# declare-lab/Emma-X

Hardware: AMD Instinct MI355X
Metric: actions/sec (higher is better)
Workload: dtype bf16; 1 GPU; BASELINE configs[1]: Emma-X-7B bf16, 1 frame(s)/GPU 224x224, 512-token prompt, greedy, 512 new tokens (EOS disabled), random-init weights; uint8 frames and prompt ids are resident in HBM when the timed region starts; the 7-vector is de-tokenised from the generated ids by the ids-level stand-in `actions_from_ids` (no LLaMA tokenizer offline: decode -> Solver text parse is host work of microseconds,; batch_per_gpu=1, global_batch=1, context=1280, parallelism=dp1, hipgraph=False, exact_numerics=False

## Files before the change

emma-x_amd/csrc/decode_ks.hip:

```cpp
#include <cstdlib>

#include "common.h"
#include "kernels.h"
#include "decode_epilogue.h"

#ifndef KS_W_AUX
#define KS_W_AUX 2
#endif
namespace {

constexpr int KS_WAVES = 8;
constexpr int KS_NT = KS_WAVES * 64;
constexpr int PSTRIDE = EMMAX_PSTRIDE;

__device__ __forceinline__ void ks_fold32(float& a, float& b) {
    asm volatile("s_nop 1\n\tv_permlane32_swap_b32 %0, %1" : "+v"(a), "+v"(b));
    a += b;
}
__device__ __forceinline__ void ks_fold16(float& a, float& b) {
    asm volatile("s_nop 1\n\tv_permlane16_swap_b32 %0, %1" : "+v"(a), "+v"(b));
    a += b;
}
template <int RB>
__device__ __forceinline__ float ks_reduce_rows(float (&v)[RB], int lane) {
    static_assert(RB == 1 || RB == 2 || RB == 4 || RB == 8 || RB == 16, "batch of rows");
    if constexpr (RB == 16) {
#pragma unroll
        for (int j = 0; j < 8; ++j) ks_fold32(v[j], v[j + 8]);
    }
    if constexpr (RB >= 8) {
        constexpr int H = 4;
#pragma unroll
        for (int j = 0; j < H; ++j) ks_fold16(v[j], v[j + H]);
    }
    if constexpr (RB >= 4) {
        const bool hi = (lane & 8) != 0;
#pragma unroll
        for (int j = 0; j < 2; ++j) {
            const float keep = hi ? v[j + 2] : v[j], give = hi ? v[j] : v[j + 2];
            v[j] = keep + dpp_move<0x128>(give);
        }
    }
    if constexpr (RB >= 2) {
        const bool hi = (lane & 4) != 0;
        const float keep = hi ? v[1] : v[0], give = hi ? v[0] : v[1];
        v[0] = keep + dpp_move<0x141>(give);
    }
    float t = v[0];
    t += dpp_move<0xB1>(t);
    t += dpp_move<0x4E>(t);
    if constexpr (RB < 2) t += dpp_move<0x141>(t);
    if constexpr (RB < 4) t += dpp_move<0x128>(t);
    if constexpr (RB < 8) { float a = t, b = t; ks_fold16(a, b); t = a; }
    if constexpr (RB < 16) { float a = t, b = t; ks_fold32(a, b); t = a; }
    return t;
}
template <int RB>
__device__ __forceinline__ int ks_row_of_lane(int lane) {
    int r = 0, bit = RB >> 1;
    if constexpr (RB == 16) { r += (lane >> 5) * bit; bit >>= 1; }
    if constexpr (RB >= 8) { r += ((lane >> 4) & 1) * bit; bit >>= 1; }
    if constexpr (RB >= 4) { r += ((lane >> 3) & 1) * bit; bit >>= 1; }
    if constexpr (RB >= 2) { r += ((lane >> 2) & 1) * bit; }
    return r;
}
template <int RB>
__device__ __forceinline__ bool ks_lane_stores(int lane) {
    int mask = 3;
    if constexpr (RB < 2) mask |= 4;
    if constexpr (RB < 4) mask |= 8;
    if constexpr (RB < 8) mask |= 16;
    if constexpr (RB < 16) mask |= 32;
    return (lane & mask) == 0;
}

template <int B, int CPL> struct KsShape { static constexpr int RB = (B == 1 ? 16 : 8) / (CPL == 1 ? 1 : CPL == 2 ? 2 : 4); };

template <int B> struct KsRegs { static constexpr int N = B == 1 ? 16 : 8; };

enum { XS_GLOBAL = 0, XS_ATTN = 1, XS_EMBED = 2 };
#ifdef DECODE_LAB_TRACE
__device__ unsigned long long g_ks_trace[512 * 2 * 4 * 6];
#define KS_STAMP(op, k, v) do { if ((threadIdx.x == 0 || threadIdx.x == 448) && blockIdx.x < 512 && (op) >= 0) \
    g_ks_trace[((blockIdx.x * 2 + (threadIdx.x ? 1 : 0)) * 4 + (op)) * 6 + (k)] = (v); } while (0)
#else
#define KS_STAMP(op, k, v) do { } while (0)
#endif
template <int MODE>
__device__ __forceinline__ void ks_pair_rows(const GemvParams& p, int g, int& r0, int& r1) {
    if (MODE == GEMV_QKV) {
        const int half = p.head_dim >> 1;
        const int hb = g >> p.ks_shift, d = g - hb * half;
        r0 = hb * p.head_dim + d;
        r1 = r0 + half;
    } else if (MODE == GEMV_GATEUP) {
        r0 = (g >> 4) * 32 + (g & 15);
        r1 = r0 + 16;
    } else {
        r0 = 2 * g;
        r1 = min(2 * g + 1, p.n_rows - 1);
    }
}
__device__ __forceinline__ void ks_share(const GemvParams& p, int& g_lo, int& npairs) {
    const int G = gridDim.x, bid = blockIdx.x;
    const int q = p.n_groups / G, r = p.n_groups % G;
    g_lo = bid * q + min(bid, r);
    npairs = min(q + (bid < r ? 1 : 0), max(p.n_groups - g_lo, 0));
}

template <int B, int MODE, int CPL>
__device__ __forceinline__ void ks_issue(const GemvParams& p, int g_lo, int nrows, int bb, const unsigned (&voff)[CPL], u32x4_t (&wr)[KsRegs<B>::N]) {
    constexpr int RB = KsShape<B, CPL>::RB;
    const __amdgpu_buffer_rsrc_t wrsrc = __builtin_amdgcn_make_buffer_rsrc((void*)p.W, 0, (int)((unsigned)p.n_rows * (unsigned)p.ldw * 2u), 0x00020000);
#pragma unroll
    for (int jj = 0; jj < RB; ++jj) {
        const int i = bb * RB + jj;
        int r0, r1;
        ks_pair_rows<MODE>(p, g_lo + (i >> 1), r0, r1);
        const int m = (i - nrows) >> 31;
        const int r = (((i & 1) ? r1 : r0) & m) | (p.n_rows & ~m);
        const unsigned so = (unsigned)r * (unsigned)p.ldw * 2u;
#pragma unroll
        for (int j = 0; j < CPL; ++j)
            wr[jj * CPL + j] = __builtin_bit_cast(u32x4_t, __builtin_amdgcn_raw_buffer_load_b128(wrsrc, voff[j], so, KS_W_AUX));
    }
}

template <int CPL>
__device__ __forceinline__ void ks_chunks(int K, int wave, int lane, int (&coff)[CPL], bool (&cok)[CPL], unsigned (&voff)[CPL]) {
    const int NCW = K >> 6;
#pragma unroll
    for (int j = 0; j < CPL; ++j) {
        const int c = j * 64 + lane;
        cok[j] = c < NCW;
        coff[j] = wave * NCW + min(c, NCW - 1);
        voff[j] = (unsigned)coff[j] * 16u;
    }
}

template <int B, int MODE, bool NORM, int XS, int CPL, bool R32, bool EX = false>
__device__ __forceinline__ void ks_run_op(const GemvParams& p, u32x4_t (&wr)[KsRegs<B>::N], float* part, float* sumsq, int rows_cap,
                                          int trace_op = -1) {
    constexpr int RB = KsShape<B, CPL>::RB;
    KS_STAMP(trace_op, 0, wall_clock64());
    const int tid = threadIdx.x, lane = tid & 63, wave = __builtin_amdgcn_readfirstlane(tid >> 6);
    const int K = p.K, bid = blockIdx.x;
    int g_lo, npairs;
    ks_share(p, g_lo, npairs);
    const int nrows = 2 * npairs;

    const bool epi = wave < B && lane < npairs;
    const int eb = wave < B ? wave : 0, epair = g_lo + min(lane, max(npairs - 1, 0));
    int er0, er1;
    ks_pair_rows<MODE>(p, epair, er0, er1);
    float pre_a = 0.f, pre_b = 0.f;
    int pre_pos = 0, pre_pg = 0;
    if (epi) {
        if (MODE == GEMV_RESID) {
            pre_a = resid_fetch(p, eb, er0, R32);
            pre_b = resid_fetch(p, eb, er1, R32);
        } else if (MODE == GEMV_QKV) {
            qkv_row_pos(p, eb, pre_pos, pre_pg);
            const int hb = epair >> p.ks_shift;
            qkv_rope_fetch(p, pre_pos, hb, epair - hb * (p.head_dim >> 1), pre_a, pre_b);
        }
    }

    int coff[CPL];
    bool cok[CPL];
    unsigned voff[CPL];
    ks_chunks<CPL>(K, wave, lane, coff, cok, voff);

    u32x4_t xr[B][CPL];
    u32x4_t xl[EX ? B : 1][EX ? CPL : 1];
    if constexpr (EX && XS == XS_GLOBAL && !NORM) {
        f32x8_t xq[B][CPL];
#pragma unroll
        for (int b = 0; b < B; ++b)
#pragma unroll
            for (int j = 0; j < CPL; ++j) xq[b][j] = ld_f32x8((const float*)p.x + (size_t)b * p.ldx + (size_t)coff[j] * 8);
        ks_issue<B, MODE, CPL>(p, g_lo, nrows, 0, voff, wr);
#pragma unroll
        for (int b = 0; b < B; ++b)
#pragma unroll
            for (int j = 0; j < CPL; ++j)
#pragma unroll
                for (int e = 0; e < 4; ++e) {
                    const hl2_t t = split_hl2(cok[j] ? f32x8_at(xq[b][j], 2 * e) : 0.f, cok[j] ? f32x8_at(xq[b][j], 2 * e + 1) : 0.f);
                    xr[b][j][e] = t.hi;
                    xl[b][j][e] = t.lo;
                }
    } else if constexpr (XS == XS_ATTN) {
#pragma unroll
        for (int b = 0; b < B; ++b)
#pragma unroll
            for (int j = 0; j < CPL; ++j) {
                const int cg = coff[j];
                const float* pp = p.attn_part + (size_t)(b * p.Hq + (cg >> 4)) * p.nsplit * PSTRIDE;
                if constexpr (EX) {
                    float m8[8];
                    (void)(p.nsplit == 8 ? attn_merge_chunk<8, 4>(pp, (cg & 15) * 8, m8) : attn_merge_chunk_loop(pp, (cg & 15) * 8, p.nsplit, m8));
#pragma unroll
                    for (int e = 0; e < 4; ++e) {
                        const hl2_t t = split_hl2(cok[j] ? m8[2 * e] : 0.f, cok[j] ? m8[2 * e + 1] : 0.f);
                        xr[b][j][e] = t.hi;
                        xl[b][j][e] = t.lo;
                    }
                } else {
                    const u32x4_t v = p.nsplit == 8 ? attn_merge_chunk<8, 4>(pp, (cg & 15) * 8) : attn_merge_chunk_loop(pp, (cg & 15) * 8, p.nsplit);
#pragma unroll
                    for (int e = 0; e < 4; ++e) xr[b][j][e] = cok[j] ? v[e] : 0u;
                }
            }
        __builtin_amdgcn_sched_barrier(0);
        ks_issue<B, MODE, CPL>(p, g_lo, nrows, 0, voff, wr);
    } else {
        u32x4_t nw[CPL];
        if constexpr (NORM) {
#pragma unroll
            for (int j = 0; j < CPL; ++j) nw[j] = *((const u32x4_t*)p.norm_w + coff[j]);
        }
        float ss[B];
        if constexpr (R32 && NORM && XS != XS_EMBED) {
            f32x8_t xq[B][CPL];
#pragma unroll
            for (int b = 0; b < B; ++b)
#pragma unroll
                for (int j = 0; j < CPL; ++j) xq[b][j] = ld_f32x8(p.h32 + (size_t)b * p.ldh + (size_t)coff[j] * 8);
            ks_issue<B, MODE, CPL>(p, g_lo, nrows, 0, voff, wr);
#pragma unroll
            for (int b = 0; b < B; ++b) {
                ss[b] = 0.f;
#pragma unroll
                for (int j = 0; j < CPL; ++j)
#pragma unroll
                    for (int e = 0; e < 4; ++e) {
                        const float a = cok[j] ? f32x8_at(xq[b][j], 2 * e) : 0.f, c = cok[j] ? f32x8_at(xq[b][j], 2 * e + 1) : 0.f;
                        ss[b] += a * a + c * c;
                        if constexpr (EX) {
                            const hl2_t t = split_hl2(a * bf_lo(nw[j][e]), c * bf_hi(nw[j][e]));
                            xr[b][j][e] = t.hi;
                            xl[b][j][e] = t.lo;
                        } else {
                            xr[b][j][e] = pack_bf16x2(a * bf_lo(nw[j][e]), c * bf_hi(nw[j][e]));
                        }
                    }
            }
        } else {
#pragma unroll
            for (int b = 0; b < B; ++b) {
                size_t row = (size_t)b;
                if constexpr (XS == XS_EMBED) row = (size_t)min(max(p.x_tok[b], 0), p.x_vocab - 1);
#pragma unroll
                for (int j = 0; j < CPL; ++j) {
                    xr[b][j] = *((const u32x4_t*)((const bf16_t*)p.x + row * p.ldx) + coff[j]);
                    if constexpr (XS == XS_EMBED) {
                        if (blockIdx.x == 0 && cok[j]) {
                            *((u32x4_t*)((bf16_t*)p.x_copy + (size_t)b * p.ldx) + coff[j]) = xr[b][j];
                            if constexpr (R32) {
                                const f32x8_t f = bf16x8_to_f32(xr[b][j]);
                                float* hp = p.h32 + (size_t)b * p.ldh + (size_t)coff[j] * 8;
                                *(f32x4_t*)hp = f.lo;
                                *(f32x4_t*)(hp + 4) = f.hi;
                            }
                        }
                    }
                }
            }
            ks_issue<B, MODE, CPL>(p, g_lo, nrows, 0, voff, wr);
#pragma unroll
            for (int b = 0; b < B; ++b) {
                ss[b] = 0.f;
#pragma unroll
                for (int j = 0; j < CPL; ++j)
#pragma unroll
                    for (int e = 0; e < 4; ++e) {
                        uint32_t v = cok[j] ? xr[b][j][e] : 0u;
                        if constexpr (NORM) {
                            const float a = bf_lo(v), c = bf_hi(v);
                            ss[b] += a * a + c * c;
                            if constexpr (EX) {
                                const hl2_t t = split_hl2(a * bf_lo(nw[j][e]), c * bf_hi(nw[j][e]));
                                v = t.hi;
                                xl[b][j][e] = t.lo;
                            } else {
                                v = pack_bf16x2(a * bf_lo(nw[j][e]), c * bf_hi(nw[j][e]));
                            }
                        }
                        xr[b][j][e] = v;
                    }
            }
        }
        if constexpr (NORM) {
#pragma unroll
            for (int b = 0; b < B; ++b) {
                const float t = wave_sum(ss[b]);
                if (lane == 0) sumsq[wave * B + b] = t;
            }
        }
    }

    KS_STAMP(trace_op, 1, wall_clock64());
    const int nbatch = (nrows + RB - 1) / RB;
    for (int bb = 0; bb < nbatch; ++bb) {
        float acc[B][RB];
#pragma unroll
        for (int jj = 0; jj < RB; ++jj)
#pragma unroll
            for (int b = 0; b < B; ++b) {
                float a = 0.f;
#pragma unroll
                for (int j = 0; j < CPL; ++j) {
                    a = dot2_bf16(wr[jj * CPL + j][0], xr[b][j][0], a);
                    a = dot2_bf16(wr[jj * CPL + j][1], xr[b][j][1], a);
                    a = dot2_bf16(wr[jj * CPL + j][2], xr[b][j][2], a);
                    a = dot2_bf16(wr[jj * CPL + j][3], xr[b][j][3], a);
                    if constexpr (EX) {
                        a = dot2_bf16(wr[jj * CPL + j][0], xl[b][j][0], a);
                        a = dot2_bf16(wr[jj * CPL + j][1], xl[b][j][1], a);
                        a = dot2_bf16(wr[jj * CPL + j][2], xl[b][j][2], a);
                        a = dot2_bf16(wr[jj * CPL + j][3], xl[b][j][3], a);
                    }
                }
                acc[b][jj] = a;
            }
        __builtin_amdgcn_sched_barrier(0);
        ks_issue<B, MODE, CPL>(p, g_lo, nrows, bb + 1, voff, wr);
        __builtin_amdgcn_sched_barrier(0);
#pragma unroll
        for (int b = 0; b < B; ++b) {
            const float t = ks_reduce_rows<RB>(acc[b], lane);
            if (ks_lane_stores<RB>(lane)) part[(wave * B + b) * rows_cap + bb * RB + ks_row_of_lane<RB>(lane)] = t;
        }
    }
    KS_STAMP(trace_op, 3, wall_clock64());
    __syncthreads();
    KS_STAMP(trace_op, 4, wall_clock64());

    float red0 = 0.f, red1 = 0.f;
    if (epi) {
#pragma unroll
        for (int w = 0; w < KS_WAVES; ++w) {
            red0 += part[(w * B + eb) * rows_cap + 2 * lane];
            red1 += part[(w * B + eb) * rows_cap + 2 * lane + 1];
        }
        if constexpr (NORM) {
            float t = 0.f;
#pragma unroll
            for (int w = 0; w < KS_WAVES; ++w) t += sumsq[w * B + eb];
            const float rstd = rsqrtf(t / (float)K + p.eps);
            red0 *= rstd;
            red1 *= rstd;
        }
    }
    const bool has1 = MODE == GEMV_QKV || MODE == GEMV_GATEUP || 2 * epair + 1 < p.n_rows;
    if (MODE == GEMV_PLAIN) {
        if (epi) {
            bf16_t* yp = (bf16_t*)p.y + (size_t)eb * p.ldy;
            yp[er0] = f2bf(red0);
            if (has1) yp[er1] = f2bf(red1);
        }
    } else if (MODE == GEMV_RESID) {
        if (epi) {
            if constexpr (R32) {
                float* hq = p.h32 + (size_t)eb * p.ldh;
                hq[er0] = pre_a + red0;
                if (has1) hq[er1] = pre_b + red1;
            }
            const uint32_t hv = pack_bf16x2(pre_a + red0, pre_b + red1);
            bf16_t* hp = (bf16_t*)p.y + (size_t)eb * p.ldy;
            hp[er0] = (bf16_t)(hv & 0xffffu);
            if (has1) hp[er1] = (bf16_t)(hv >> 16);
        }
    } else if (MODE == GEMV_GATEUP) {
        if (epi) swiglu_finish<EX>(p, eb, epair, red0, red1);
    } else if (MODE == GEMV_QKV && EX) {
        if (epi) {
            const int hd = p.head_dim, half = hd >> 1;
            const int hb = epair >> p.ks_shift, d = epair - hb * half;
            if (hb < p.Hq + p.Hkv) {
                const float y0 = __fadd_rn(__fmul_rn(red0, pre_a), -__fmul_rn(red1, pre_b)), y1 = __fadd_rn(__fmul_rn(red1, pre_a), __fmul_rn(red0, pre_b));
                if (hb < p.Hq) {
                    float* dst = (float*)p.y + (size_t)eb * p.ldy + hb * hd;
                    dst[d] = y0;
                    dst[d + half] = y1;
                } else {
                    gemv_kv_store_x(p, false, pre_pg, pre_pos, hb - p.Hq, d, y0);
                    gemv_kv_store_x(p, false, pre_pg, pre_pos, hb - p.Hq, d + half, y1);
                }
            } else {
                gemv_kv_store_x(p, true, pre_pg, pre_pos, hb - p.Hq - p.Hkv, d, red0);
                gemv_kv_store_x(p, true, pre_pg, pre_pos, hb - p.Hq - p.Hkv, d + half, red1);
            }
        }
    } else if (MODE == GEMV_QKV) {
        if (epi) {
            const int hd = p.head_dim, half = hd >> 1;
            const int hb = epair >> p.ks_shift, d = epair - hb * half;
            const float x0 = bf2f(f2bf(red0)), x1 = bf2f(f2bf(red1));
            if (hb < p.Hq + p.Hkv) {
                const bf16_t y0 = f2bf(x0 * pre_a - x1 * pre_b), y1 = f2bf(x1 * pre_a + x0 * pre_b);
                if (hb < p.Hq) {
                    bf16_t* q = (bf16_t*)p.y + (size_t)eb * p.ldy + hb * hd;
                    q[d] = y0;
                    q[d + half] = y1;
                } else {
                    bf16_t* kc = gemv_kv_row(p, false, eb, pre_pg, pre_pos, hb - p.Hq);
                    kc[d] = y0;
                    kc[d + half] = y1;
                }
            } else {
                bf16_t* vc = gemv_kv_row(p, true, eb, pre_pg, pre_pos, hb - p.Hq - p.Hkv);
                vc[d] = f2bf(x0);
                vc[d + half] = f2bf(x1);
            }
        }
    } else if (MODE == GEMV_LMHEAD) {
        if (wave < B) {
            float bv = -INFINITY;
            int bi = 0x7fffffff;
            if (epi) {
                bv = red0;
                bi = er0;
                if (has1) lmhead_take(red1, er1, bv, bi);
                if (p.logits_out) {
                    p.logits_out[(size_t)eb * p.n_rows + er0] = red0;
                    if (has1) p.logits_out[(size_t)eb * p.n_rows + er1] = red1;
                }
            }
            const float m = wave_max(bv);
            const float mi = wave_max((epi && bv == m) ? -(float)bi : -INFINITY);
            if (lane == 0) {
                p.part_val[(size_t)bid * B + eb] = m;
                p.part_idx[(size_t)bid * B + eb] = mi == -INFINITY ? 0x7fffffff : (int)(-mi);
            }
        }
    }
    KS_STAMP(trace_op, 5, wall_clock64());
}

template <int B, int MODE, bool NORM, int XS, int CPL, bool R32, bool EX = false>
__global__ __launch_bounds__(KS_NT, 4) void emmax_decode_ks_kernel(GemvParams p) {
    extern __shared__ __attribute__((aligned(16))) unsigned char ks_smem[];
    const int tid = threadIdx.x, lane = tid & 63, wave = __builtin_amdgcn_readfirstlane(tid >> 6);
    const int rows_cap = p.kc;
    float* part = (float*)ks_smem;
    float* sumsq = part + KS_WAVES * B * rows_cap;
    u32x4_t wr[KsRegs<B>::N];
    ks_run_op<B, MODE, NORM, XS, CPL, R32, EX>(p, wr, part, sumsq, rows_cap, 0);
}

template <int B, int MODE, bool NORM, int XS, int CPL, bool R32, bool EX = false>
int ks_launch_r(const GemvParams& p, const ProjGeom& g, hipStream_t stream) {
    hipLaunchKernelGGL((emmax_decode_ks_kernel<B, MODE, NORM, XS, CPL, R32, EX>), dim3(g.grid), dim3(KS_NT), g.smem, stream, p);
    return hipGetLastError() == hipSuccess ? 0 : -4;
}
template <int B, int MODE, bool NORM, bool XATTN, int CPL>
int ks_launch_t(const GemvParams& p, const ProjGeom& g, hipStream_t stream) {
    constexpr bool touches_h = NORM || MODE == GEMV_RESID;
    if (p.exact) {
        if constexpr (MODE == GEMV_PLAIN) return -2;
        else {
            if constexpr (MODE == GEMV_QKV) {
                if (p.x_tok) return ks_launch_r<B, MODE, NORM, XS_EMBED, CPL, true, true>(p, g, stream);
            }
            return ks_launch_r<B, MODE, NORM, XATTN ? XS_ATTN : XS_GLOBAL, CPL, true, true>(p, g, stream);
        }
    }
    if constexpr (MODE == GEMV_QKV) {
        if (p.x_tok) return p.h32 ? ks_launch_r<B, MODE, NORM, XS_EMBED, CPL, true>(p, g, stream) : ks_launch_r<B, MODE, NORM, XS_EMBED, CPL, false>(p, g, stream);
    }
    if constexpr (touches_h) {
        if (p.h32) return ks_launch_r<B, MODE, NORM, XATTN ? XS_ATTN : XS_GLOBAL, CPL, true>(p, g, stream);
    }
    return ks_launch_r<B, MODE, NORM, XATTN ? XS_ATTN : XS_GLOBAL, CPL, false>(p, g, stream);
}

template <int MODE, bool NORM, bool XATTN>
int ks_launch_mode(const GemvParams& p, int B, const ProjGeom& g, hipStream_t stream) {
#define KS_CASE(BB, CC) if (B == BB && g.cpl == CC) return ks_launch_t<BB, MODE, NORM, XATTN, CC>(p, g, stream)
    KS_CASE(1, 1); KS_CASE(1, 2); KS_CASE(1, 3); KS_CASE(2, 1); KS_CASE(2, 2); KS_CASE(2, 3);
#undef KS_CASE
    return -2;
}

}

bool decode_ks_enabled() { return emmax_tune().ks != 0; }

bool decode_ks_takes(const ProjShape& s, int B, ProjGeom* out) {
    if (B < 1 || B > 2 || s.wfmt != PW_BF16) return false;
    if (s.K % 64 || s.K > 64 * 64 * 3 || !s.ld_ok || s.K < 64) return false;
    if (s.mode < GEMV_QKV || s.mode > GEMV_PLAIN) return false;
    ProjGeom g = {};
    int max_grid = s.max_grid;
    if (s.mode == GEMV_RESID && s.attn_part) {
        if (s.K != s.Hq * 128) return false;
        if (!emmax_tune().ks_oproj) return false;
        max_grid = emmax_tune().ks_oproj_grid;
    }
    if (s.x_tok && s.mode != GEMV_QKV) return false;
    if (s.exact ? (s.mode == GEMV_PLAIN || !s.h32) : (s.mode == GEMV_PLAIN && s.h32)) return false;
    g.n_groups = (s.mode == GEMV_QKV || s.mode == GEMV_GATEUP) ? s.n_rows / 2 : (s.n_rows + 1) / 2;
    if (s.mode == GEMV_QKV) {
        while ((2 << g.shift) < s.head_dim) ++g.shift;
        if ((2 << g.shift) != s.head_dim) return false;
    }
    g.cpl = cdiv(s.K >> 6, 64);
    const int rb = B == 1 ? (g.cpl == 1 ? KsShape<1, 1>::RB : g.cpl == 2 ? KsShape<1, 2>::RB : KsShape<1, 3>::RB)
                          : (g.cpl == 1 ? KsShape<2, 1>::RB : g.cpl == 2 ? KsShape<2, 2>::RB : KsShape<2, 3>::RB);
    g.grid = min(512, g.n_groups);
    if (max_grid > 0) g.grid = min(g.grid, max_grid);
    if (s.mode == GEMV_LMHEAD) g.grid = min(g.grid, s.max_parts);
    if (g.grid < 1) return false;
    const int pairs_max = cdiv(g.n_groups, g.grid);
    if (pairs_max > 64) return false;
    g.kc = cdiv(2 * pairs_max, rb) * rb;
    g.smem = (size_t)(KS_WAVES * B * g.kc + KS_WAVES * B) * sizeof(float);
    if (out) *out = g;
    return true;
}

int launch_decode_ks(int mode, const GemvParams& p_in, int B, hipStream_t stream, int* grid_out, const ProjGeom* geom) {
    ProjGeom g;
    if (geom) g = *geom;
    else if (!decode_ks_takes(proj_shape(mode, p_in), B, &g)) return -2;
    GemvParams p = p_in;
    p.n_groups = p.n_pairs = g.n_groups; p.ks_shift = g.shift; p.kc = g.kc;
    if (grid_out) *grid_out = g.grid;
    switch (mode) {
        case GEMV_QKV: return ks_launch_mode<GEMV_QKV, true, false>(p, B, g, stream);
        case GEMV_RESID:
            return p.attn_part ? ks_launch_mode<GEMV_RESID, false, true>(p, B, g, stream) : ks_launch_mode<GEMV_RESID, false, false>(p, B, g, stream);
        case GEMV_GATEUP: return ks_launch_mode<GEMV_GATEUP, true, false>(p, B, g, stream);
        case GEMV_LMHEAD: return ks_launch_mode<GEMV_LMHEAD, true, false>(p, B, g, stream);
        default: return ks_launch_mode<GEMV_PLAIN, false, false>(p, B, g, stream);
    }
}

#ifdef DECODE_LAB_TRACE
extern "C" int emmax_debug_ks_trace(unsigned long long* host_out, int n_words) {
    return hipMemcpyFromSymbol(host_out, HIP_SYMBOL(g_ks_trace), (size_t)n_words * 8) == hipSuccess ? 0 : -1;
}
#endif
```

emma-x_amd/csrc/kernels.h:

```cpp
#pragma once

#include <hip/hip_runtime.h>
#include <stdint.h>

#include "common.h"

struct GemmParams {
    const void* A;
    const void* W;
    void* C;
    const void* bias;
    const void* scale;
    const void* residual;
    int M, N, K;
    int lda, ldw, ldc, ldr;
    int res_f32;
    int N_store;
    int act;
    int out_f32;
    float* ws;
    long long ws_bytes;
    int ksplit;
    const float* ln_stats;
    const float* ln_s;
// ... 63 lines not shown
};
int launch_prefill_state(const PrefillState& st, int32_t* cu, int32_t* ctx_len, int32_t* done, int32_t* n_out, int32_t* max_new,
                         int32_t* stop_m, int32_t* stop_after, hipStream_t stream);
struct CommitParams {
    int n, max_pages, max_out;
    int slot[EMMAX_MAX_DECODE_BATCH], src[EMMAX_MAX_DECODE_BATCH];
    int32_t *cur_tok, *ctx_len, *done, *n_out, *max_new, *stop_m, *stop_after, *out_ids, *page_table;
    float *temperature, *top_p, *logprob;
    int32_t* top_k;
    uint64_t* seed;
    uint32_t* subseq;
    float* penalty;
    int32_t *ngram, *min_new, *hist, *hist_len;
    int max_prompt;
    float* warp[4];
    uint32_t* rule_en;
};
int launch_slots_commit(const CommitParams& c, hipStream_t stream);
struct SlotForkParams {
    int n, rows, src, S, max_pages, max_prompt;
    int dst[EMMAX_MAX_DECODE_BATCH];
    int32_t *page_table, *hidden, *ctx_len, *done, *n_out, *max_new, *stop_m, *stop_after, *copy_src, *copy_dst, *copy_ntok;
    const float *in_t, *in_p;
    const int32_t* in_k;
    const uint64_t* in_seed;
    const uint32_t* in_sub;
    float *temperature, *top_p;
    int32_t* top_k;
    uint64_t* seed;
    uint32_t* subseq;
    float* penalty;
    int32_t *ngram, *min_new, *hist, *hist_len;
    float* warp[4];
    uint32_t* rule_en;
};
int launch_slots_fork(const SlotForkParams& p, hipStream_t stream);
int launch_slots_unhide(int32_t* table, int32_t* hidden, int n, hipStream_t stream);
int launch_set_int(int32_t* p, int32_t v, hipStream_t stream);
int launch_set_ints(int32_t* p, int n, int32_t v, hipStream_t stream);
int launch_slots_idle(int n, int32_t* cur_tok, int32_t* ctx_len, int32_t* done, int32_t* n_out, int32_t pad_id, hipStream_t stream);
int launch_embed_splice(const int32_t* ids, int P_max, const int32_t* cu, const void* E, const void* patches, void* h, int B,
                        int max_seqlen, int n_patches, int hidden, int vocab, hipStream_t stream, float* h32 = nullptr);
int launch_rope_kv_write(void* qkv, int ld, int q_off, int k_off, int v_off, const int32_t* cu, int B, int total_rows,
                         const float* cos_t, const float* sin_t, void* kcache, void* vcache, const int32_t* page_table,
                         int max_pages, int Hq, int Hkv, int hd, int page, hipStream_t stream);
int launch_kv_quant_rows(void* qkv , int ld, int k_off, int v_off, const int32_t* cu, int B, int total_rows, void* k8, void* v8, float* kscale,
                         float* vscale, const int32_t* page_table, int max_pages, int Hkv, int hd, int page, hipStream_t stream);
int launch_resize_bicubic_u8(const uint8_t* src, int B, int H, int W, uint8_t* dst, int OH, int OW, uint8_t* tmp, const int32_t* bounds_h,
                             const int32_t* kk_h, int ksize_h, const int32_t* bounds_v, const int32_t* kk_v, int ksize_v, hipStream_t stream);
int launch_gather_last_rows(const void* in, void* out, const int32_t* cu, int B, int D, hipStream_t stream, float* out32 = nullptr, const float* in32 = nullptr);

struct EmmaxTune {
    int graph;
    int ks;
    int ks_oproj;
    int ks_oproj_grid;
    int km;
    int km_down;
    int km_roll;
    int attn_deep;
    int attn_ksplit;
    int attn_lazy;
    int vis_streams;
    int attn_nw;
    int streamk;
    int fp8_gemv;
    int attn_group;
    int attn_nsplit;
    int attn_direct;
    int fold_embed;
    int mfma_xbar;
    int gemm_big;
    int gemm_splitk;
    int gemm_sk_big;
    int gemm_hybrid;
    int gemm_normfuse;
    int gemm_deep;
    int gemm_dbg;
    int gemm_lnfuse;
    int attn_resident;
    int kv_fp8;
    int resid32;
    int mx4_wide;
    int exact;
    int epoch;
};
const EmmaxTune& emmax_tune();

enum { GEMV_QKV = 0, GEMV_RESID = 1, GEMV_GATEUP = 2, GEMV_LMHEAD = 3, GEMV_PLAIN = 4 };
struct GemvParams {
    const void* x;
    const void* W;
    void* y;
    const void* norm_w;
    int K, ldw, ldx, ldy;
    int n_rows;
    int n_groups;
    int max_parts;
    int kc;
    int batch;
    float eps;
    int head_dim, Hq, Hkv, page, max_pages;
    const int32_t* ctx_len;
    const int32_t* page_table;
    const float* cos_t;
    const float* sin_t;
    void* kcache;
    void* vcache;
    float* part_val;
    int32_t* part_idx;
    float* logits_out;
    const float* attn_part;
    int nsplit;
    void* kv_stage;
    const float* wscale;
    int n_pairs;
    unsigned long long* sk_ws;
    int sk_kt8, sk_q, sk_r;
    unsigned int sk_magic;
    int qk_shift;
    int x_bar;
    int max_grid;
    int ks_shift;
    const int32_t* x_tok;
    void* x_copy;
    int x_vocab;
    float* h32;
    int ldh;
    int exact;
    long long kv24;
    const void* w4_scales;
};

enum { PW_BF16 = 0, PW_FP8 = 1, PW_MX4 = 2 };
struct ProjShape {
    int mode, K, n_rows, head_dim, Hq;
    int wfmt;
    bool exact, h32, attn_part, x_tok;
    int nsplit, max_parts, max_grid;
    bool ld_ok;
    bool mx4_wide;
};
static inline ProjShape proj_shape(int mode, const GemvParams& p) {
    return {mode, p.K, p.n_rows, p.head_dim, p.Hq, p.w4_scales ? PW_MX4 : p.wscale ? PW_FP8 : PW_BF16, p.exact != 0, p.h32 != nullptr,
            p.attn_part != nullptr, p.x_tok != nullptr, p.nsplit, p.max_parts, p.max_grid, p.ldw % 8 == 0 && p.ldx % 8 == 0};
}
struct ProjGeom {
    int grid, n_groups;
    int kc;
    size_t smem;
    int shift;
    int cpl, f8;
    int nb, phased, roll;
    int tmax, nph, nh;
};
bool decode_ks_takes(const ProjShape& s, int B, ProjGeom* g = nullptr);
bool decode_gemv_takes(const ProjShape& s, int B, ProjGeom* g = nullptr);
bool decode_km_takes(const ProjShape& s, int B, ProjGeom* g = nullptr);
bool decode_kmp_takes(const ProjShape& s, int B, ProjGeom* g = nullptr);
bool decode_mfma_takes(const ProjShape& s, int B, ProjGeom* g = nullptr);
int launch_decode_gemv(int mode, const GemvParams& p, int B, hipStream_t stream, int* grid_out = nullptr, int* staged_out = nullptr);
int launch_decode_gemv_staged(int mode, const GemvParams& p, int B, const ProjGeom& g, hipStream_t stream, int* grid_out = nullptr);
int launch_decode_ks(int mode, const GemvParams& p, int B, hipStream_t stream, int* grid_out = nullptr, const ProjGeom* geom = nullptr);
bool decode_ks_enabled();
int decode_gemv_init();
int launch_decode_embed(const int32_t* cur_tok, const void* E, void* h, int B, int hidden, int vocab, hipStream_t stream, float* h32 = nullptr);

struct DecodeAttnParams {
    const void* q;
    const void* kcache;
    const void* vcache;
    const int32_t* page_table;
    const int32_t* ctx_len;
    const int32_t* done;
    float* part;
    void* o_out;
    const void* kv_stage;
    float* kscale;
    float* vscale;
    int ldq, Hkv, page, max_pages;
    int page_shift;
    float scale;
    long long kv24;
    const int32_t* grp_shared;
    int grp_N, grp_nsplit, grp_Hq;
};
int decode_attn_nsplit(int B, int Hkv);
int launch_decode_attn(const DecodeAttnParams& p, int B, int Hq, int head_dim, int nsplit, hipStream_t stream);
enum { EMMAX_GROUP_ATTN_MAX_SPLITS = 8 };
bool group_attn_takes(int B, int N, int Hq, int Hkv);
int group_attn_nsplit(int B, int N, int Hq, int Hkv);
int launch_group_attn(const DecodeAttnParams& p, int B, int N, int Hq, int head_dim, hipStream_t stream);
int launch_x_decode_attn(const DecodeAttnParams& p, int B, int Hq, int head_dim, int nsplit, hipStream_t stream);

struct FinishParams {
    const float* part_val;
    const int32_t* part_idx;
    int n_part, B;
    int32_t* cur_tok;
    int32_t* ctx_len;
    int32_t* done;
    int32_t* n_out;
    int32_t* out_ids;
    const int32_t* max_new_p;
    const int32_t* stop_ids;
    const int32_t* stop_cfg;
    int32_t* stop_m;
    int32_t* stop_after;
    int max_out, max_ctx;
    int eos_id, pad_id;
    int is_prefill;
};
int launch_decode_finish(const FinishParams& p, hipStream_t stream);
__device__ __forceinline__ void emmax_finish_row(const FinishParams& p, int b, int tok, float* lp_row, float lp, bool stop_row) {
    int was_done = p.done[b];
    int n = p.n_out[b];
    const int budget_n = p.max_new_p[b];
    if (!p.is_prefill && !was_done && n >= budget_n) {
        was_done = 1;
        p.done[b] = 1;
    }
    if (!p.is_prefill && !was_done) p.ctx_len[b] += 1;
    if (p.is_prefill)
        for (int i = 0; i < p.max_out; ++i) {
            p.out_ids[(size_t)b * p.max_out + i] = p.pad_id;
            if (lp_row) lp_row[i] = 0.f;
        }
    if (was_done) {
        tok = p.pad_id;
    } else {
        if (n < p.max_out) {
            p.out_ids[(size_t)b * p.max_out + n] = tok;
            if (lp_row) lp_row[n] = lp;
        }
        n += 1;
        p.n_out[b] = n;
        const bool budget = !p.is_prefill && n >= budget_n;
        bool stop = false;
        const int n_trig = p.stop_cfg[0];
        if (n_trig > 0) {
            int aft = p.stop_after[b];
            if (aft >= 0) {
                aft += 1;
            } else {
                int mp = p.stop_m[b];
                mp = (tok == p.stop_ids[mp]) ? mp + 1 : ((tok == p.stop_ids[0]) ? 1 : 0);
                if (mp == n_trig) {
// ... 162 lines not shown
```

emma-x_amd/csrc/model.hip:

```cpp
#include <array>
#include <cctype>
#include <cstdarg>
#include <cstdlib>
#include <mutex>

#include "session.h"

thread_local std::string g_err;
int fail(int code, const char* fmt, ...) {
    char buf[1024];
    va_list ap;
    va_start(ap, fmt);
    vsnprintf(buf, sizeof(buf), fmt, ap);
    va_end(ap);
    g_err = buf;
    return code;
}

namespace {
struct TuneEntry { const char* name; int EmmaxTune::*field; int def; };
const TuneEntry kTune[] = {
    {"graph", &EmmaxTune::graph, 0},           {"ks", &EmmaxTune::ks, 1},
    {"ks_oproj", &EmmaxTune::ks_oproj, 1},     {"ks_oproj_grid", &EmmaxTune::ks_oproj_grid, 256},
    {"km", &EmmaxTune::km, 1},                 {"km_down", &EmmaxTune::km_down, 1},
    {"km_roll", &EmmaxTune::km_roll, 0},       {"attn_nw", &EmmaxTune::attn_nw, 4},
    {"attn_deep", &EmmaxTune::attn_deep, -1},  {"attn_ksplit", &EmmaxTune::attn_ksplit, -1},
    {"attn_lazy", &EmmaxTune::attn_lazy, 1},      {"vis_streams", &EmmaxTune::vis_streams, 1},
    {"streamk", &EmmaxTune::streamk, 1},       {"fp8_gemv", &EmmaxTune::fp8_gemv, -1},
    {"attn_nsplit", &EmmaxTune::attn_nsplit, 0}, {"attn_direct", &EmmaxTune::attn_direct, 1},
    {"fold_embed", &EmmaxTune::fold_embed, 1}, {"mfma_xbar", &EmmaxTune::mfma_xbar, 1},
    {"gemm_big", &EmmaxTune::gemm_big, -1},    {"gemm_splitk", &EmmaxTune::gemm_splitk, 1},
    {"gemm_sk_big", &EmmaxTune::gemm_sk_big, -1},
    {"gemm_deep", &EmmaxTune::gemm_deep, -1},       {"gemm_dbg", &EmmaxTune::gemm_dbg, 0},
    {"gemm_lnfuse", &EmmaxTune::gemm_lnfuse, 1}, {"attn_resident", &EmmaxTune::attn_resident, -1},
    {"gemm_hybrid", &EmmaxTune::gemm_hybrid, 1}, {"gemm_normfuse", &EmmaxTune::gemm_normfuse, 1},
    {"resid32", &EmmaxTune::resid32, 1},       {"kv_fp8", &EmmaxTune::kv_fp8, 0},
    {"exact", &EmmaxTune::exact, 0},           {"attn_group", &EmmaxTune::attn_group, -1},
    {"mx4_wide", &EmmaxTune::mx4_wide, 0},
};
EmmaxTune g_tune;
std::once_flag g_tune_once;
void tune_init() {
    g_tune.epoch = 0;
    for (const TuneEntry& e : kTune) {
        g_tune.*(e.field) = e.def;
        std::string env = "EMMAX_";
        for (const char* c = e.name; *c; ++c) env += (char)toupper((unsigned char)*c);
        if (const char* v = getenv(env.c_str())) g_tune.*(e.field) = atoi(v);
    }
}
}
const EmmaxTune& emmax_tune() {
    std::call_once(g_tune_once, tune_init);
    return g_tune;
}

__attribute__((constructor)) static void emmax_export_runtime_switches() { setenv("DEBUG_CLR_GRAPH_PACKET_CAPTURE", "0", 0); }

static int check_config(const emmax_config& c, bool format_rules = true) {
    for (int t = 0; t < 2; ++t) {
        const auto& w = c.tower[t];
        if (w.embed_dim <= 0 || w.num_heads <= 0 || w.embed_dim % w.num_heads) return fail(EMMAX_ERR_INVALID, "tower %d: bad embed_dim/num_heads", t);
        const int hd = w.embed_dim / w.num_heads;
        if (hd != 64 && hd != 72) return fail(EMMAX_ERR_INVALID, "tower %d: head_dim %d outside the hot path (64 or 72)", t, hd);
        if (w.embed_dim % 8 || w.mlp_hidden % 8) return fail(EMMAX_ERR_INVALID, "tower %d: dims must be multiples of 8", t);
        if (w.take_index < 0 || w.take_index >= w.depth) return fail(EMMAX_ERR_INVALID, "tower %d: take_index out of range", t);
        if (w.image_size % w.patch) return fail(EMMAX_ERR_INVALID, "tower %d: image_size %% patch != 0", t);
    }
    if (c.tower[0].image_size != c.tower[1].image_size || c.tower[0].patch != c.tower[1].patch)
        return fail(EMMAX_ERR_INVALID, "towers must share image size and patch size");
    if (c.head_dim != 128) return fail(EMMAX_ERR_INVALID, "LLM head_dim %d outside the hot path (128)", c.head_dim);
    if (c.hidden % 128) return fail(EMMAX_ERR_INVALID, "LLM hidden must be a multiple of 128");
    if (c.n_heads % c.n_kv_heads) return fail(EMMAX_ERR_INVALID, "n_heads %% n_kv_heads != 0");
    const int G = c.n_heads / c.n_kv_heads;
    if (G != 1 && G != 2 && G != 4 && G != 8) return fail(EMMAX_ERR_INVALID, "GQA group %d unsupported (1,2,4,8)", G);
    if (c.inter % 16) return fail(EMMAX_ERR_INVALID, "LLM intermediate size must be a multiple of 16");
    if (c.vocab % 8) return fail(EMMAX_ERR_INVALID, "vocab must be a multiple of 8");
    if (c.decode_fp8 < 0 || c.decode_fp8 > 2) return fail(EMMAX_ERR_INVALID, "decode_fp8 %d: 0 (bf16), 1 (fp8-e4m3) or 2 (MXFP4)", c.decode_fp8);
    if (c.decode_fp8 == 1 && (c.hidden % 64 || (c.n_heads * c.head_dim) % 64)) return fail(EMMAX_ERR_INVALID, "fp8 decode needs K % 64 == 0");
    if (c.decode_fp8 == 2 && format_rules) {
        const int q_dim = c.n_heads * c.head_dim, qkv_dim = (c.n_heads + 2 * c.n_kv_heads) * c.head_dim;
        if (c.hidden % 1024 || c.hidden > 4096 || q_dim % 1024 || q_dim > 4096)
            return fail(EMMAX_ERR_INVALID, "MXFP4 decode weights need hidden (%d) and n_heads * head_dim (%d) in multiples of 1024 up to 4096", c.hidden, q_dim);
        if (c.inter % 128 || c.inter <= 4096 || c.inter > 12288)
            return fail(EMMAX_ERR_INVALID, "MXFP4 decode weights need an intermediate size (%d) that is a multiple of 128, above 4096 and at most 12288", c.inter);
        if (qkv_dim > 32768 || 2 * c.inter > 32768 || pad_to(c.vocab, 128) > 32768)
            return fail(EMMAX_ERR_INVALID, "MXFP4 decode weights need at most 32768 rows per projection (qkv %d, gate/up %d, vocab %d)", qkv_dim, 2 * c.inter, c.vocab);
    }
    return 0;
}

struct ProjDim { int stage; int64_t N, K; int perm, perm_hd, gemv_mode, f8bit; };
static std::array<ProjDim, 4> layer_projs(const emmax_model* m) {
    return {{{STAGE_QKV, m->qkv_dim, m->H, 1, m->cfg.head_dim, GEMV_QKV, F8_QKV}, {STAGE_OPROJ, m->H, m->q_dim, 0, 0, GEMV_RESID, F8_OPROJ},
             {STAGE_GATEUP, 2 * (int64_t)m->inter_p, m->H, 2, 0, GEMV_GATEUP, F8_GATEUP}, {STAGE_DOWN, m->H, m->inter_p, 0, 0, GEMV_RESID, F8_DOWN}}};
}

static void derive(emmax_model* m) {
    const auto& c = m->cfg;
    m->H = c.hidden;
    m->inter = c.inter;
    m->inter_p = pad_to(c.inter, 64);
    m->q_dim = c.n_heads * c.head_dim;
    m->kv_dim = c.n_kv_heads * c.head_dim;
    m->qkv_dim = m->q_dim + 2 * m->kv_dim;
    m->vocab = c.vocab;
    m->vocab_p = pad_to(c.vocab, 128);
    m->V = c.tower[0].embed_dim + c.tower[1].embed_dim;
    m->Vp = pad_to(m->V, 128);
    m->P1 = 4 * m->V;
    m->P1p = pad_to(m->P1, 128);
    for (int t = 0; t < 2; ++t) {
        const auto& w = c.tower[t];
        TowerW& T = m->tw[t];
        T.D = w.embed_dim;
        T.Dp = pad_to(T.D, 128);
        T.D3p = pad_to(3 * T.D, 128);
        T.M = w.mlp_hidden;
        T.Mp = pad_to(T.M, 128);
        T.n_prefix = (w.has_cls ? 1 : 0) + w.n_reg;
        T.n_patches = (w.image_size / w.patch) * (w.image_size / w.patch);
        T.N = T.n_prefix + T.n_patches;
        T.hd = T.D / w.num_heads;
        T.Kpe = pad_to(3 * w.patch * w.patch, 64);
        T.n_blocks = w.take_index + 1;
        T.blk.resize(T.n_blocks);
    }
    m->layers.resize(c.n_layers);
    for (auto& L : m->layers) {
        memset(&L, 0, sizeof(L));
        for (const ProjDim& d : layer_projs(m)) { L.proj[d.stage].gemv_mode = d.gemv_mode; L.proj[d.stage].f8bit = d.f8bit; }
    }
    m->lm_head_w = ProjW{};
    m->lm_head_w.gemv_mode = GEMV_LMHEAD; m->lm_head_w.f8bit = F8_LMHEAD;
    m->fp8 = c.decode_fp8 == 1;
    m->mx4 = c.decode_fp8 == 2;
    m->mx4_wide = m->mx4 && emmax_tune().mx4_wide != 0;
    for (auto& L : m->layers)
        for (const ProjDim& d : layer_projs(m)) L.proj[d.stage].q4w = m->mx4_wide;
    m->lm_head_w.q4w = m->mx4_wide;
}

static void plan_arena(emmax_model* m, Bump& b) {
    for (int t = 0; t < 2; ++t) {
        TowerW& T = m->tw[t];
        T.patch_w = b.take((int64_t)T.Dp * T.Kpe);
        T.patch_b = b.take(T.Dp);
        T.pos = b.take((int64_t)T.n_patches * T.D);
        T.cls = b.take(T.D);
        T.reg = b.take((int64_t)std::max(1, m->cfg.tower[t].n_reg) * T.D);
        for (auto& k : T.blk) {
            k.n1w = b.take(T.D); k.n1b = b.take(T.D);
            k.qkv_w = b.take((int64_t)T.D3p * T.Dp); k.qkv_b = b.take(T.D3p);
            k.proj_w = b.take((int64_t)T.Dp * T.Dp); k.proj_b = b.take(T.Dp);
            k.ls1 = b.take(T.Dp);
            k.n2w = b.take(T.D); k.n2b = b.take(T.D);
            k.fc1_w = b.take((int64_t)T.Mp * T.Dp); k.fc1_b = b.take(T.Mp);
            k.fc2_w = b.take((int64_t)T.Dp * T.Mp); k.fc2_b = b.take(T.Dp);
            k.ls2 = b.take(T.Dp);
            k.ln1_s = (float*)b.take(2 * (int64_t)T.D3p); k.ln1_c = (float*)b.take(2 * (int64_t)T.D3p);
            k.ln2_s = (float*)b.take(2 * (int64_t)T.Mp); k.ln2_c = (float*)b.take(2 * (int64_t)T.Mp);
        }
    }
    m->pj1_w = b.take((int64_t)m->P1p * m->Vp); m->pj1_b = b.take(m->P1p);
    m->pj2_w = b.take((int64_t)m->H * m->P1p); m->pj2_b = b.take(m->H);
    m->pj3_w = b.take((int64_t)m->H * m->H); m->pj3_b = b.take(m->H);
    m->embed = b.take((int64_t)m->vocab * m->H);
    for (auto& L : m->layers) {
        const auto dims = layer_projs(m);
        ProjW *const q = &L.proj[STAGE_QKV], *const o = &L.proj[STAGE_OPROJ], *const g = &L.proj[STAGE_GATEUP], *const d = &L.proj[STAGE_DOWN];
        L.ln1 = b.take(m->H);
        q->rm = b.take(dims[0].N * dims[0].K);
        o->rm = b.take(dims[1].N * dims[1].K);
        L.ln2 = b.take(m->H);
        g->rm = b.take(dims[2].N * dims[2].K);
        d->rm = b.take(dims[3].N * dims[3].K);
        for (const ProjDim& p : dims) { ProjW& w = L.proj[p.stage]; w.r8 = nullptr; w.sc = w.km_sc = nullptr; w.q4 = w.q4s = nullptr; }
        if (m->mx4)
            for (const ProjDim& p : dims) { ProjW& w = L.proj[p.stage]; w.q4 = b.bytes(p.N * p.K / 2); w.q4s = b.bytes(p.N * p.K / 32); }
        if (m->fp8) {
            for (const ProjDim& p : dims) L.proj[p.stage].fm = b.take(p.N * p.K / 2);
            q->km = b.take(dims[0].N * dims[0].K / 2);
            g->km = b.take(dims[2].N * dims[2].K / 2);
            for (const ProjDim& p : dims) L.proj[p.stage].r8 = b.take(p.N * p.K / 2);
            for (const ProjDim& p : dims) L.proj[p.stage].sc = (float*)b.take(2 * p.N);
            q->km_sc = (float*)b.take(2 * dims[0].N);
            g->km_sc = (float*)b.take(2 * dims[2].N);
            o->km = o->fm; o->km_sc = o->sc;
            d->km = d->fm; d->km_sc = d->sc;
        }
    }
    m->final_norm = b.take(m->H);
    ProjW& lm = m->lm_head_w;
    lm.rm = b.take((int64_t)m->vocab_p * m->H);
    if (m->fp8) {
        lm.km = lm.fm = b.take((int64_t)m->vocab_p * m->H / 2);
        lm.km_sc = lm.sc = (float*)b.take(2 * (int64_t)m->vocab_p);
        lm.r8 = b.take((int64_t)m->vocab_p * m->H / 2);
    }
    if (m->mx4) { lm.q4 = b.bytes((int64_t)m->vocab_p * m->H / 2); lm.q4s = b.bytes((int64_t)m->vocab_p * m->H / 32); }
}

static void plan_aux(emmax_model* m, Bump& b, bool with_ab_partner) {
    for (auto& L : m->layers) {
        const auto dims = layer_projs(m);
        ProjW *const q = &L.proj[STAGE_QKV], *const o = &L.proj[STAGE_OPROJ], *const g = &L.proj[STAGE_GATEUP], *const d = &L.proj[STAGE_DOWN];
        q->km = b.take(dims[0].N * dims[0].K);
        g->km = b.take(dims[2].N * dims[2].K);
        o->km = o->fm = b.take(dims[1].N * dims[1].K);
        d->km = d->fm = b.take(dims[3].N * dims[3].K);
        q->fm = with_ab_partner ? b.take(dims[0].N * dims[0].K) : nullptr;
        g->fm = with_ab_partner ? b.take(dims[2].N * dims[2].K) : nullptr;
    }
    m->lm_head_w.km = m->lm_head_w.fm = b.take((int64_t)m->vocab_p * m->H);
}

static int put2d(emmax_model* m, const std::string& key, int rows, int cols, bf16* dst, int dst_ld, int row0, hipStream_t st) {
    auto it = m->bound.find(key);
    if (it == m->bound.end()) return fail(EMMAX_ERR_MISSING, "finalize: weight `%s` was never bound", key.c_str());
    const Bound& w = it->second;
    if (w.dtype != EMMAX_BF16) return fail(EMMAX_ERR_INVALID, "weight `%s` must be bf16", key.c_str());
    if (w.numel() != (int64_t)rows * cols)
        return fail(EMMAX_ERR_INVALID, "weight `%s`: expected %d x %d = %lld elements, got %lld", key.c_str(), rows, cols,
// ... 81 lines not shown
        TowerW& T = m->tw[t];
        const emmax_tower_config& tc = m->cfg.tower[t];
        const std::string P = pre[t];
        PUT2(P + "patch_embed.proj.weight", T.D, 3 * tc.patch * tc.patch, T.patch_w, T.Kpe, 0);
        PUT1(P + "patch_embed.proj.bias", T.D, T.patch_b);
        PUT1(P + "pos_embed", T.n_patches * T.D, T.pos);
        if (tc.has_cls) PUT1(P + "cls_token", T.D, T.cls);
        if (tc.n_reg) PUT1(P + "reg_token", tc.n_reg * T.D, T.reg);
        for (int i = 0; i < T.n_blocks; ++i) {
            BlockW& k = T.blk[i];
            const std::string Bp = P + "blocks." + std::to_string(i) + ".";
            PUT1(Bp + "norm1.weight", T.D, k.n1w); PUT1(Bp + "norm1.bias", T.D, k.n1b);
            PUT2(Bp + "attn.qkv.weight", 3 * T.D, T.D, k.qkv_w, T.Dp, 0); PUT1(Bp + "attn.qkv.bias", 3 * T.D, k.qkv_b);
            PUT2(Bp + "attn.proj.weight", T.D, T.D, k.proj_w, T.Dp, 0); PUT1(Bp + "attn.proj.bias", T.D, k.proj_b);
            PUT1(Bp + "norm2.weight", T.D, k.n2w); PUT1(Bp + "norm2.bias", T.D, k.n2b);
            PUT2(Bp + "mlp.fc1.weight", T.M, T.D, k.fc1_w, T.Dp, 0); PUT1(Bp + "mlp.fc1.bias", T.M, k.fc1_b);
            PUT2(Bp + "mlp.fc2.weight", T.D, T.M, k.fc2_w, T.Mp, 0); PUT1(Bp + "mlp.fc2.bias", T.D, k.fc2_b);
            if (tc.layerscale) { PUT1(Bp + "ls1.scale_factor", T.D, k.ls1); PUT1(Bp + "ls2.scale_factor", T.D, k.ls2); }
            if (fold_ln) {
                KCHK(launch_ln_fold(k.qkv_w, T.Dp, 3 * T.D, T.D, k.n1w, k.n1b, k.qkv_b, k.ln1_s, k.ln1_c, st));
                KCHK(launch_ln_fold(k.fc1_w, T.Dp, T.M, T.D, k.n2w, k.n2b, k.fc1_b, k.ln2_s, k.ln2_c, st));
            }
        }
    }
    PUT2("projector.fc1.weight", m->P1, m->V, m->pj1_w, m->Vp, 0); PUT1("projector.fc1.bias", m->P1, m->pj1_b);
    PUT2("projector.fc2.weight", m->H, m->P1, m->pj2_w, m->P1p, 0); PUT1("projector.fc2.bias", m->H, m->pj2_b);
    PUT2("projector.fc3.weight", m->H, m->H, m->pj3_w, m->H, 0); PUT1("projector.fc3.bias", m->H, m->pj3_b);
    PUT2("language_model.model.embed_tokens.weight", m->vocab, m->H, m->embed, m->H, 0);
    for (int li = 0; li < m->cfg.n_layers; ++li) {
        LayerW& L = m->layers[li];
        const std::string P = "language_model.model.layers." + std::to_string(li) + ".";
        PUT1(P + "input_layernorm.weight", m->H, L.ln1);
        PUT2(P + "self_attn.q_proj.weight", m->q_dim, m->H, L.proj[STAGE_QKV].rm, m->H, 0);
        PUT2(P + "self_attn.k_proj.weight", m->kv_dim, m->H, L.proj[STAGE_QKV].rm, m->H, m->q_dim);
        PUT2(P + "self_attn.v_proj.weight", m->kv_dim, m->H, L.proj[STAGE_QKV].rm, m->H, m->q_dim + m->kv_dim);
        PUT2(P + "self_attn.o_proj.weight", m->H, m->q_dim, L.proj[STAGE_OPROJ].rm, m->q_dim, 0);
        PUT1(P + "post_attention_layernorm.weight", m->H, L.ln2);
        {
            auto ig = m->bound.find(P + "mlp.gate_proj.weight");
            auto iu = m->bound.find(P + "mlp.up_proj.weight");
            if (ig == m->bound.end() || iu == m->bound.end()) return fail(EMMAX_ERR_MISSING, "finalize: gate/up of layer %d not bound", li);
            if (ig->second.numel() != (int64_t)m->inter * m->H || iu->second.numel() != (int64_t)m->inter * m->H)
                return fail(EMMAX_ERR_INVALID, "gate/up of layer %d have the wrong size", li);
            const size_t grp = (size_t)16 * m->H * 2;
            HIPCHK(hipMemcpy2DAsync(L.proj[STAGE_GATEUP].rm, 2 * grp, ig->second.ptr, grp, grp, m->inter / 16, hipMemcpyDeviceToDevice, st));
            HIPCHK(hipMemcpy2DAsync((char*)L.proj[STAGE_GATEUP].rm + grp, 2 * grp, iu->second.ptr, grp, grp, m->inter / 16, hipMemcpyDeviceToDevice, st));
        }
        PUT2(P + "mlp.down_proj.weight", m->H, m->inter, L.proj[STAGE_DOWN].rm, m->inter_p, 0);
        if (m->fp8) {
            const auto dims = layer_projs(m);
            for (const ProjDim& d : dims) KCHK(launch_quant_fm8(L.proj[d.stage].rm, (int)d.K, L.proj[d.stage].fm, L.proj[d.stage].sc, (int)d.N, (int)d.K, st));
            for (const ProjDim& d : dims)
                KCHK(launch_quant_rm8(L.proj[d.stage].rm, (int)d.K, L.proj[d.stage].r8, L.proj[d.stage].sc, (int)d.N, (int)d.K, st));
            for (const ProjDim& d : dims)
                if (d.perm) KCHK(launch_quant_fm8(L.proj[d.stage].rm, (int)d.K, L.proj[d.stage].km, L.proj[d.stage].km_sc, (int)d.N, (int)d.K, st, d.perm, d.perm_hd));
        }
        if (m->mx4)
            for (const ProjDim& d : layer_projs(m)) {
                ProjW& w = L.proj[d.stage];
                KCHK(launch_quant_mx4(w.rm, (int)d.K, w.q4, w.q4s, (int)d.N, (int)d.K, d.perm, d.perm_hd, st));
                KCHK(launch_dequant_mx4(w.q4, w.q4s, w.rm, (int)d.K, (int)d.N, (int)d.K, d.perm, d.perm_hd, st));
            }
    }
    PUT1("language_model.model.norm.weight", m->H, m->final_norm);
    PUT2("language_model.lm_head.weight", m->vocab, m->H, m->lm_head_w.rm, m->H, 0);
    if (m->fp8) {
        KCHK(launch_quant_fm8(m->lm_head_w.rm, m->H, m->lm_head_w.fm, m->lm_head_w.sc, m->vocab_p, m->H, st));
        KCHK(launch_quant_rm8(m->lm_head_w.rm, m->H, m->lm_head_w.r8, m->lm_head_w.sc, m->vocab_p, m->H, st));
    }
    if (m->mx4) {
        KCHK(launch_quant_mx4(m->lm_head_w.rm, m->H, m->lm_head_w.q4, m->lm_head_w.q4s, m->vocab_p, m->H, 0, 0, st));
        KCHK(launch_dequant_mx4(m->lm_head_w.q4, m->lm_head_w.q4s, m->lm_head_w.rm, m->H, m->vocab_p, m->H, 0, 0, st));
    }
#undef PUT2
#undef PUT1
    HIPCHK(hipStreamSynchronize(st));
    m->finalized = true;
    m->ln_folded = fold_ln;
    m->aux_built = m->fp8 || m->mx4;
    m->bound.clear();
    return 0;
}

int emmax_model_max_decode_batch(const emmax_model* m) { return m ? model_max_decode_batch(m) : -1; }
int emmax_model_max_decode_batch_exact(const emmax_model* m) { return m ? model_max_decode_batch(m, true) : -1; }
int emmax_model_mxfp4_wide(const emmax_model* m) { return m ? (m->mx4_wide ? 1 : 0) : -1; }
int emmax_config_max_decode_batch(const emmax_config* cfg, int exact) {
    if (!cfg) return fail(EMMAX_ERR_INVALID, "null argument");
    if (int r = check_config(*cfg, false)) return r;
    emmax_model tmp;
    tmp.cfg = *cfg;
    derive(&tmp);
    return model_max_decode_batch(&tmp, exact != 0);
}

int64_t emmax_model_aux_bytes(const emmax_model* m) {
    if (!m) return -1;
    if (m->fp8 || m->mx4) return 0;
    emmax_model tmp = *m;
    Bump b{nullptr};
    plan_aux(&tmp, b, emmax_tune().km == 0);
    return b.off + 256;
}

int emmax_model_build_aux(emmax_model* m, void* aux, int64_t aux_bytes, emmax_stream stream) {
    if (!m) return fail(EMMAX_ERR_INVALID, "null argument");
    if (!m->finalized) return fail(EMMAX_ERR_STATE, "emmax_model_build_aux before emmax_model_finalize");
    if (m->fp8 || m->mx4) return 0;
    if (!aux) return fail(EMMAX_ERR_INVALID, "null argument");
    hipStream_t st = (hipStream_t)stream;
    const bool ab = emmax_tune().km == 0;
    const int64_t need = emmax_model_aux_bytes(m);
    if (aux_bytes < need) return fail(EMMAX_ERR_NOMEM, "aux arena too small: %lld < %lld", (long long)aux_bytes, (long long)need);
    if ((uintptr_t)aux % 256) return fail(EMMAX_ERR_INVALID, "aux arena must be 256-byte aligned");
    Bump b{(char*)aux};
    plan_aux(m, b, ab);
    for (auto& L : m->layers) {
        const auto dims = layer_projs(m);
        for (const ProjDim& d : dims)
            if (d.perm) KCHK(launch_repack_km(L.proj[d.stage].rm, (int)d.K, L.proj[d.stage].km, (int)d.N, (int)d.K, d.perm, d.perm_hd, st));
        for (const ProjDim& d : dims)
            if (!d.perm) KCHK(launch_repack_fm(L.proj[d.stage].rm, (int)d.K, L.proj[d.stage].fm, (int)d.N, (int)d.K, st));
        for (const ProjDim& d : dims)
            if (d.perm && ab) KCHK(launch_repack_fm(L.proj[d.stage].rm, (int)d.K, L.proj[d.stage].fm, (int)d.N, (int)d.K, st));
    }
    KCHK(launch_repack_fm(m->lm_head_w.rm, m->H, m->lm_head_w.fm, m->vocab_p, m->H, st));
    HIPCHK(hipStreamSynchronize(st));
    m->aux_built = true;
    m->aux_ab = ab;
    return 0;
}

}
```

emma-x_amd/csrc/ops.hip:

```cpp
#include "session.h"

static GemvParams plain_gemv(const void* x, const void* W, void* y, int N, int K, const float* wscale = nullptr) {
    GemvParams p;
    memset(&p, 0, sizeof(p));
    p.x = x; p.ldx = K; p.W = W; p.ldw = K; p.K = K; p.y = y; p.ldy = N; p.n_rows = N; p.wscale = wscale;
    return p;
}

extern "C" {

int emmax_profile_decode_stage(emmax_session* s, int stage, int reps, float* avg_us, emmax_stream stream) {
    if (!s || !avg_us || reps < 1) return fail(EMMAX_ERR_INVALID, "bad argument");
    if (!s->prefilled) return fail(EMMAX_ERR_STATE, "profile needs an active (prefilled) session");
    hipStream_t st = (hipStream_t)stream;
    emmax_model* m = s->m;
    const int B = s->cur_B, nl = m->cfg.n_layers;
    hipEvent_t e0, e1;
    HIPCHK(hipEventCreate(&e0));
    HIPCHK(hipEventCreate(&e1));
    int launches = 0, r = 0;
    for (int pass = 0; pass < 2 && r == 0; ++pass) {
        if (pass == 1) HIPCHK(hipEventRecord(e0, st));
        const int n = pass == 0 ? 1 : reps;
        for (int i = 0; i < n && r == 0; ++i) {
// ... 590 lines not shown
    if (ksplit != 0 && (ksplit < 2 || ksplit > K / 64)) return fail(EMMAX_ERR_INVALID, "emmax_op_gemm_stream: ksplit %d (0 = the launch plan, else 2..K / 64 = %d)", ksplit, K / 64);
    if (ws && (ws_bytes < 0 || ((uintptr_t)ws & 15))) return fail(EMMAX_ERR_INVALID, "emmax_op_gemm_stream: the workspace must be 16-byte aligned");
    if (ksplit >= 2 && (!ws || (long long)ksplit * M * N * 4 > ws_bytes))
        return fail(EMMAX_ERR_NOMEM, "emmax_op_gemm_stream: %d slices need a workspace of %lld bytes (%lld given)", ksplit, (long long)ksplit * M * N * 4, (long long)(ws ? ws_bytes : 0));
    if ((norm_w == nullptr) != (norm_out == nullptr)) return fail(EMMAX_ERR_INVALID, "emmax_op_gemm_stream: norm_w and norm_out go together");
    GemmParams p = gp(A, lda, W, ldw, C32, ldc, M, N, K);
    p.bias = bias; p.act = act; p.scale = scale; p.out_f32 = 1; p.res_f32 = 1; p.N_store = n_store;
    p.residual = residual32 ? residual32 : C32;
    p.ldr = residual32 ? ldr : ldc;
    if (ws) { p.ws = (float*)ws; p.ws_bytes = ws_bytes; }
    if (norm_out) {
        p.norm_w = norm_w; p.norm_out = norm_out; p.ld_norm = ld_norm; p.norm_eps = eps;
        if (ld_norm < N) return fail(EMMAX_ERR_INVALID, "emmax_op_gemm_stream: ld_norm %d < N %d", ld_norm, N);
        if (ksplit == 0 ? !gemm_fuses_norm(p) : !gemm_splitk_fuses_norm(p))
            return fail(EMMAX_ERR_INVALID, "emmax_op_gemm_stream: this path does not fuse the RMSNorm (act 0, N = 4096 whole rows, 16-byte aligned rows of ld %% 8, %s)",
                        ksplit == 0 ? "and a launch plan that splits K with the given workspace" : "explicit slices");
    }
    const int r = ksplit == 0 ? launch_gemm(p, (hipStream_t)stream) : launch_gemm_splitk(p, ksplit, (hipStream_t)stream, emmax_tune().gemm_sk_big > 0 ? 1 : 0);
    if (r) return fail(r == -4 ? EMMAX_ERR_HIP : EMMAX_ERR_INVALID, "emmax_op_gemm_stream: unsupported shape or launch failure");
    return 0;
}
int emmax_op_rmsnorm_f32(const float* x, int ldx, void* y, int ldy, const void* w, int rows, int D, float eps, emmax_stream stream) {
    if (!x || !y || !w) return fail(EMMAX_ERR_INVALID, "emmax_op_rmsnorm_f32: null argument");
    if (rows < 1 || D < 8 || ldx < D || ldy < D || (((uintptr_t)x | (uintptr_t)y | (uintptr_t)w) & 15))
        return fail(EMMAX_ERR_INVALID, "emmax_op_rmsnorm_f32: rows %d, D %d, ldx %d / ldy %d (>= D), 16-byte aligned pointers", rows, D, ldx, ldy);
    const int r = launch_rmsnorm_f32(x, y, w, rows, D, ldx, ldy, eps, (hipStream_t)stream);
    if (r) return fail(r == -4 ? EMMAX_ERR_HIP : EMMAX_ERR_INVALID, "emmax_op_rmsnorm_f32: unsupported shape (D %% 8, D <= 8192, ldx %% 4, ldy %% 8)");
    return 0;
}
int emmax_op_rope_kv_write(void* qkv, int ld, int q_off, int k_off, int v_off, const int32_t* cu, int B, int total_rows, const float* cos_t, const float* sin_t,
                           void* kcache, void* vcache, const int32_t* page_table, int max_pages, int Hq, int Hkv, int head_dim, int page, emmax_stream stream) {
    if (!qkv || !cu || !cos_t || !sin_t || !page_table) return fail(EMMAX_ERR_INVALID, "emmax_op_rope_kv_write: null argument");
    if ((kcache == nullptr) != (vcache == nullptr)) return fail(EMMAX_ERR_INVALID, "emmax_op_rope_kv_write: kcache and vcache go together (both null: rotate only)");
    if (B < 1 || B > EMMAX_MAX_DECODE_BATCH || total_rows < 1 || Hq < 1 || Hkv < 1 || page < 1 || max_pages < 1)
        return fail(EMMAX_ERR_INVALID, "emmax_op_rope_kv_write: B %d (1..%d), total_rows %d, heads %d / %d, page %d, max_pages %d", B, EMMAX_MAX_DECODE_BATCH, total_rows, Hq, Hkv, page, max_pages);
    if (head_dim < 8 || head_dim % 8 || (ld | q_off | k_off | v_off) % 8 || q_off < 0 || k_off < 0 || v_off < 0 || q_off + Hq * head_dim > ld || k_off + Hkv * head_dim > ld ||
        v_off + Hkv * head_dim > ld)
        return fail(EMMAX_ERR_INVALID, "emmax_op_rope_kv_write: head_dim %d, ld %d and the offsets %d / %d / %d in multiples of 8, the heads inside a row", head_dim, ld, q_off, k_off, v_off);
    if ((((uintptr_t)qkv | (uintptr_t)kcache | (uintptr_t)vcache) & 15) || (((uintptr_t)cos_t | (uintptr_t)sin_t | (uintptr_t)cu | (uintptr_t)page_table) & 3))
        return fail(EMMAX_ERR_INVALID, "emmax_op_rope_kv_write: qkv and the caches must be 16-byte aligned, the tables 4-byte aligned");
    const int r = launch_rope_kv_write(qkv, ld, q_off, k_off, v_off, cu, B, total_rows, cos_t, sin_t, kcache, vcache, page_table, max_pages, Hq, Hkv, head_dim, page,
                                       (hipStream_t)stream);
    if (r) return fail(r == -4 ? EMMAX_ERR_HIP : EMMAX_ERR_INVALID, "emmax_op_rope_kv_write: launch failure");
    return 0;
}
int emmax_op_kv_quant_rows(void* qkv, int ld, int k_off, int v_off, const int32_t* cu, int B, int total_rows, void* k8, void* v8, float* kscale, float* vscale,
                           const int32_t* page_table, int max_pages, int Hkv, int head_dim, int page, emmax_stream stream) {
    if (!qkv || !cu || !k8 || !v8 || !kscale || !vscale || !page_table) return fail(EMMAX_ERR_INVALID, "emmax_op_kv_quant_rows: null argument");
    if (head_dim != 128) return fail(EMMAX_ERR_INVALID, "emmax_op_kv_quant_rows: head_dim %d (the fp8 KV cache holds rows of 128)", head_dim);
    if (B < 1 || B > EMMAX_MAX_DECODE_BATCH || total_rows < 1 || Hkv < 1 || page < 1 || max_pages < 1)
        return fail(EMMAX_ERR_INVALID, "emmax_op_kv_quant_rows: B %d (1..%d), total_rows %d, Hkv %d, page %d, max_pages %d", B, EMMAX_MAX_DECODE_BATCH, total_rows, Hkv, page, max_pages);
    if ((ld | k_off | v_off) % 8 || k_off < 0 || v_off < 0 || k_off + Hkv * 128 > ld || v_off + Hkv * 128 > ld)
        return fail(EMMAX_ERR_INVALID, "emmax_op_kv_quant_rows: ld %d and the offsets %d / %d in multiples of 8, the heads inside a row", ld, k_off, v_off);
    if (((uintptr_t)qkv & 15) || (((uintptr_t)k8 | (uintptr_t)v8) & 7) || (((uintptr_t)kscale | (uintptr_t)vscale | (uintptr_t)cu | (uintptr_t)page_table) & 3))
        return fail(EMMAX_ERR_INVALID, "emmax_op_kv_quant_rows: qkv must be 16-byte aligned, the e4m3 pages 8-byte, scales and tables 4-byte");
    const int r = launch_kv_quant_rows(qkv, ld, k_off, v_off, cu, B, total_rows, k8, v8, kscale, vscale, page_table, max_pages, Hkv, head_dim, page, (hipStream_t)stream);
    if (r) return fail(r == -4 ? EMMAX_ERR_HIP : EMMAX_ERR_INVALID, "emmax_op_kv_quant_rows: launch failure");
    return 0;
}
int emmax_op_embed_splice(const int32_t* ids, int P_max, const int32_t* cu, const void* E, const void* patches, void* h, float* h32, int B, int max_seqlen,
                          int n_patches, int hidden, int vocab, emmax_stream stream) {
    if (!ids || !cu || !E || !h) return fail(EMMAX_ERR_INVALID, "emmax_op_embed_splice: null argument");
    if (n_patches < 0 || (n_patches > 0 && !patches)) return fail(EMMAX_ERR_INVALID, "emmax_op_embed_splice: n_patches %d needs the patch rows (0: text only)", n_patches);
    if (B < 1 || B > EMMAX_MAX_DECODE_BATCH || P_max < 1 || max_seqlen < 1 || max_seqlen > n_patches + P_max || vocab < 1 || hidden < 8 || hidden % 8)
        return fail(EMMAX_ERR_INVALID, "emmax_op_embed_splice: B %d (1..%d), P_max %d, max_seqlen %d (1..n_patches + P_max), vocab %d, hidden %d (%% 8)", B, EMMAX_MAX_DECODE_BATCH, P_max,
                    max_seqlen, vocab, hidden);
    if ((((uintptr_t)E | (uintptr_t)patches | (uintptr_t)h | (uintptr_t)h32) & 15) || (((uintptr_t)ids | (uintptr_t)cu) & 3))
        return fail(EMMAX_ERR_INVALID, "emmax_op_embed_splice: rows must be 16-byte aligned, ids and cu 4-byte aligned");
    const int r = launch_embed_splice(ids, P_max, cu, E, patches, h, B, max_seqlen, n_patches, hidden, vocab, (hipStream_t)stream, h32);
    if (r) return fail(r == -4 ? EMMAX_ERR_HIP : EMMAX_ERR_INVALID, "emmax_op_embed_splice: launch failure");
    return 0;
}
int emmax_op_gather_last_rows(const void* in, const float* in32, void* out, float* out32, const int32_t* cu, int B, int D, emmax_stream stream) {
    if ((!in && !in32) || !out || !cu) return fail(EMMAX_ERR_INVALID, "emmax_op_gather_last_rows: null argument (source rows as bf16 or as fp32, bf16 out, cu)");
    if (in && in32) return fail(EMMAX_ERR_INVALID, "emmax_op_gather_last_rows: one source, bf16 or fp32");
    if (B < 1 || B > EMMAX_MAX_DECODE_BATCH || D < 8 || D % 8) return fail(EMMAX_ERR_INVALID, "emmax_op_gather_last_rows: B %d (1..%d), D %d (%% 8)", B, EMMAX_MAX_DECODE_BATCH, D);
    if ((((uintptr_t)in | (uintptr_t)in32 | (uintptr_t)out | (uintptr_t)out32) & 15) || ((uintptr_t)cu & 3))
        return fail(EMMAX_ERR_INVALID, "emmax_op_gather_last_rows: rows must be 16-byte aligned, cu 4-byte aligned");
    const int r = launch_gather_last_rows(in, out, cu, B, D, (hipStream_t)stream, out32, in32);
    if (r) return fail(r == -4 ? EMMAX_ERR_HIP : EMMAX_ERR_INVALID, "emmax_op_gather_last_rows: launch failure");
    return 0;
}


}
```

emma-x_amd/csrc/session.h:

```cpp
#pragma once
#include <hip/hip_runtime.h>

#include <algorithm>
#include <cmath>
#include <cstdio>
#include <cstring>
#include <string>
#include <unordered_map>
#include <vector>

#include "../../include/emmax.h"
#include "common.h"
#include "kernels.h"

#pragma GCC visibility push(hidden)
extern thread_local std::string g_err;
int fail(int code, const char* fmt, ...);
#pragma GCC visibility pop
#define HIPCHK(x)                                                                                                   \
    do {                                                                                                            \
        hipError_t e_ = (x);                                                                                        \
        if (e_ != hipSuccess) return fail(EMMAX_ERR_HIP, "%s failed: %s (%s:%d)", #x, hipGetErrorString(e_), __FILE__, __LINE__); \
    } while (0)
#define KCHK(x)                                                                                                     \
    do {                                                                                                            \
        int r_ = (x);                                                                                               \
        if (r_ != 0) return fail(r_ == -4 ? EMMAX_ERR_HIP : EMMAX_ERR_INVALID, "%s failed (%d) (%s:%d)", #x, r_, __FILE__, __LINE__); \
    } while (0)

static inline int pad_to(int x, int m) { return (x + m - 1) / m * m; }
static const int PAGE = 64;
static const int EMMAX_LM_BLOCKS = 512;

typedef uint16_t bf16;

struct Bump {
    char* base;
    int64_t off = 0;
    void* bytes(int64_t n) {
        off = (off + 255) / 256 * 256;
        void* p = base ? (void*)(base + off) : nullptr;
        off += n;
        return p;
    }
    bf16* take(int64_t elems) { return (bf16*)bytes(elems * 2); }
};

struct Bound {
    const void* ptr;
    int dtype;
    std::vector<int64_t> shape;
    int64_t numel() const {
        int64_t n = 1;
        for (auto s : shape) n *= s;
        return n;
    }
};

struct BlockW {
    bf16 *n1w, *n1b, *qkv_w, *qkv_b, *proj_w, *proj_b, *ls1, *n2w, *n2b, *fc1_w, *fc1_b, *fc2_w, *fc2_b, *ls2;
    float *ln1_s, *ln1_c, *ln2_s, *ln2_c;
};
struct TowerW {
    int D, Dp, D3p, M, Mp, N, n_prefix, n_patches, hd, Kpe, n_blocks;
    bf16 *patch_w, *patch_b, *pos, *cls, *reg;
    std::vector<BlockW> blk;
};

enum { STAGE_QKV = 0, STAGE_ATTN = 1, STAGE_OPROJ = 2, STAGE_GATEUP = 3, STAGE_DOWN = 4, STAGE_LMHEAD = 5 };
enum { F8_QKV = 1, F8_OPROJ = 2, F8_GATEUP = 4, F8_DOWN = 8, F8_LMHEAD = 16 };

struct ProjW {
    bf16 *rm, *fm;
    bf16* km;
    bf16* r8;
    float *sc, *km_sc;
    void *q4, *q4s;
    int gemv_mode, f8bit;
    bool q4w;
};
struct LayerW {
    bf16 *ln1, *ln2;
    ProjW proj[STAGE_DOWN + 1];
};

struct emmax_model {
    emmax_config cfg;
    std::unordered_map<std::string, Bound> bound;
    bool finalized = false;
    int H, inter, inter_p, q_dim, kv_dim, qkv_dim, vocab, vocab_p, V, Vp, P1, P1p;
    TowerW tw[2];
    bf16 *pj1_w, *pj1_b, *pj2_w, *pj2_b, *pj3_w, *pj3_b;
    bf16 *embed, *final_norm;
    ProjW lm_head_w = {};
    bool fp8 = false;
    bool mx4 = false;
    bool mx4_wide = false;
    bool ln_folded = false;
    bool aux_built = false;
    bool aux_ab = false;
    std::vector<LayerW> layers;
};

enum { UPLOAD_ROWS = 256, PINNED_BYTES = 4096 * 4 };
struct Pinned {
    int32_t done[EMMAX_MAX_DECODE_BATCH];
    alignas(8) char upload[UPLOAD_ROWS * (4 * 4 + 8)];
};
static_assert(sizeof(Pinned) <= PINNED_BYTES, "the pinned buffer's layout outgrew its allocation");

struct Sampling {
    bool on = false;
    float *t, *p, *logprob ;
    int32_t* k;
    uint64_t* seed;
    uint32_t* sub;
};
struct Processing {
    bool on = false;
    float* pen;
    int32_t *ng, *mn, *hist , *hist_len;
};
struct Warpers {
    bool on = false;
    float *minp, *typ, *eps, *eta;
};
struct TokenRules {
    bool on = false;
    bool implied_proc = false;
    int32_t *n , *off , *ids , *flags;
    float* bias;
    uint32_t* en;
};
struct Scores {
    bool on = false, has_scores = false;
    int rows = 0;
    uint64_t* words;
};
struct Beams {
    int K = 0, G = 0, es = 0, lp_pos = 0, eos = -1, max_new = 0;
    bool forked = false, ready = false;
    float *cand_acc, *row_lse, *run, *fin_score, *pw, *tr_score, *tr_lse, *tc_acc, *res_score;
    int32_t *cand_tok, *fin_flag, *fin_t, *fin_par, *fin_tok, *grp, *spare, *csrc, *cdst, *cntok, *tr_tok, *tr_par, *tc_idx, *res_bidx, *res_len;
};

struct emmax_session {
    emmax_model* m;
    int max_batch, max_prompt, max_ctx, max_pages, max_rows , max_out;
    int rows_total, stg0, n_stg;
    bf16 *vA, *vpe, *vtok, *vln, *vqkv, *vatt, *vmlp, *feats, *pj1, *pj2, *patch_embeds;
    float* vstats;
    int32_t* cu_vit[2];
    bf16 *v2A, *v2pe, *v2tok, *v2ln, *v2qkv, *v2att, *v2mlp;
    float *v2stats, *v2splitk_ws;
    int64_t v2splitk_bytes;
    int vis2_B = 0;
    hipStream_t vis_stream = nullptr;
    hipEvent_t ev_vfork = nullptr, ev_vjoin = nullptr;
    bf16 *ph, *pxn, *pqkv, *patt, *pact;
    float* ph32;
    bool p32 = false;
    int32_t* cu;
    bf16 *dh, *dq, *datt, *dact;
    float* dh32;
    float *part, *part_val, *part_val2 ;
    float* logits;
    Sampling samp;
    Processing proc;
    Warpers warp;
    TokenRules rules;
    Scores scores;
    Beams beam;
    int grp_N = 0;
    int32_t* grp_shared = nullptr;
    int32_t* hidden = nullptr;
    float *fork_t = nullptr, *fork_p = nullptr;
    int32_t* fork_k = nullptr;
    uint64_t* fork_seed = nullptr;
    uint32_t* fork_sub = nullptr;
    std::vector<int> sg_gid, sg_own, sg_nfull, slot_fresh, slot_stg_idx, slot_stg_epoch;
// ... 17 lines not shown
    int n_lm_blocks;
    bf16* kv;
    int64_t kv_layer_stride;
    bool kv8 = false;
    bf16* kv_stage = nullptr;
    int cur_B = 0, total_rows = 0, max_seqlen = 0, vision_B = 0;
    int dec_steps = 0;
    bool prefilled = false;
    std::vector<int> S;
    Pinned* pinned = nullptr;
    hipGraph_t graph = nullptr;
    hipGraphExec_t graph_exec = nullptr;
    hipStream_t graph_stream_cap = nullptr;
    int graph_B = 0;
    int graph_failed = 0;
    int last_step_graph = 0;
    int last_via = 0;
    int op_rows = 0;
    int32_t *op_state = nullptr, *op_out = nullptr;
    hipEvent_t ev = nullptr;
    int graph_epoch = -1;
    int graph_grp = 0;
    int graph_mode = 0;
    hipStream_t own_stream = nullptr;
    hipEvent_t ev_in = nullptr, ev_out = nullptr;
    std::string graph_err;
};

enum { KV_BF16 = 0, KV_FP8 = 1, KV_F32 = 2, KV_X24 = 3 };
static inline int kv_elem_bytes(int fmt) { return fmt == KV_F32 ? 4 : fmt == KV_X24 ? 3 : fmt == KV_FP8 ? 1 : 2; }
static inline int64_t kv_rows_per_layer(const emmax_model* m, int rows, int max_pages) { return (int64_t)rows * max_pages * m->cfg.n_kv_heads * PAGE; }
static inline char* kv_layer(emmax_session* s, int layer) { return (char*)s->kv + (size_t)layer * s->kv_layer_stride; }
static inline int64_t kv_rows(emmax_session* s) { return kv_rows_per_layer(s->m, s->rows_total, s->max_pages); }
static inline bf16* kcache_of(emmax_session* s, int layer) { return (bf16*)kv_layer(s, layer); }
static inline bf16* vcache_of(emmax_session* s, int layer) { return (bf16*)(kv_layer(s, layer) + kv_rows(s) * s->m->cfg.head_dim * kv_elem_bytes(s->kv_fmt)); }
static inline float* kscale_of(emmax_session* s, int layer) { return (float*)(kv_layer(s, layer) + 2 * kv_rows(s) * s->m->cfg.head_dim); }
static inline float* vscale_of(emmax_session* s, int layer) { return kscale_of(s, layer) + kv_rows(s); }
static inline float* h32_of(emmax_session* s, int slot0 = 0) { return emmax_tune().resid32 ? s->dh32 + (size_t)slot0 * s->m->H : nullptr; }

#pragma GCC visibility push(hidden)
class StreamScope {
public:
    StreamScope(emmax_session* s, emmax_stream user) : s_(s), user_((hipStream_t)user), st_(user_) { err_ = enter(); }
    StreamScope(const StreamScope&) = delete;
    ~StreamScope() { if (st_ != user_ && hipEventRecord(s_->ev_out, st_) == hipSuccess) (void)hipStreamWaitEvent(user_, s_->ev_out, 0); }
    int error() const { return err_; }
    hipStream_t stream() const { return st_; }
    int leave() {
        const hipStream_t st = st_;
        st_ = user_;
        if (st != user_) {
            HIPCHK(hipEventRecord(s_->ev_out, st));
            HIPCHK(hipStreamWaitEvent(user_, s_->ev_out, 0));
        }
        return 0;
    }

private:
    int enter() {
        if ((uintptr_t)user_ > 2) return 0;
        HIPCHK(hipEventRecord(s_->ev_in, user_));
        HIPCHK(hipStreamWaitEvent(s_->own_stream, s_->ev_in, 0));
        st_ = s_->own_stream;
        return 0;
    }
    emmax_session* s_;
    hipStream_t user_, st_;
    int err_;
};

int check_sampling_values(const emmax_session* s, const int32_t* rows, int n, const float* T, const int32_t* top_k, const float* top_p);
int upload_fork_sampling(emmax_session* s, int n, const float* T, const int32_t* top_k, const float* top_p, const uint64_t* seed, const uint32_t* subseq,
                         hipStream_t st);
int slots_restore_pages(emmax_session* s, hipStream_t st);
GemmParams gp(const void* A, int lda, const void* W, int ldw, void* C, int ldc, int M, int N, int K);
GemmParams gps(emmax_session* s, const void* A, int lda, const void* W, int ldw, void* C, int ldc, int M, int N, int K);
GemmParams gpx(emmax_session* s, const void* A_hl, int Kp, const void* W, int ldw, float* C, int ldc, int M, int N);
int run_prefill(emmax_session* s, const int32_t* ids, const int32_t* lens, int B, int P_max, const void* patches, hipStream_t st, int slot0 = -1);
int model_max_decode_batch(const emmax_model* m, bool exact = false, int* first_stage = nullptr, int* first_B = nullptr);
int session_max_rows(const emmax_session* s);
int decode_stage_route(const emmax_model* m, int stage, int B, bool exact);
bool decode_batch_served(const emmax_model* m, int B, bool exact);
const char* decode_stage_name(int stage);
int stage_chunk(int stage, bool exact);
bool beam_pages_fit(const emmax_session* s, int S, int max_new);
int launch_beam_finish(emmax_session* s, bool is_prefill, hipStream_t st);
int run_group_fork(emmax_session* s, int G, hipStream_t st);
int run_slots_fork(emmax_session* s, int src, int logit_row, const int32_t* dst, int n, hipStream_t st);
int run_lm_head_step(emmax_session* s, int B, bool is_prefill, float* logits_out, bool do_finish, hipStream_t st, int slot0 = 0);
int run_decode_stage(emmax_session* s, int B, int li, int stage, hipStream_t st);
int decode_oproj_form(const emmax_model* m, bool exact, int B, int* nsplit);
int attn_group_rows(const emmax_session* s, int B);
int run_decode_step(emmax_session* s, int B, hipStream_t st);
int ensure_graph(emmax_session* s, int B, hipStream_t st);
int launch_graph_step(emmax_session* s, int B, hipStream_t st);
void drop_graph(emmax_session* s);

#pragma GCC visibility pop
```

emma-x_amd/csrc/step.hip:

```cpp
#include "session.h"

static bool streamk_on() { return emmax_tune().streamk != 0; }

static int fp8_gemv_mask(int B) {
    const int mask = emmax_tune().fp8_gemv;
    if (mask >= 0) return mask & 31;
    return B == 1 ? (F8_OPROJ | F8_LMHEAD) : F8_OPROJ;
}

struct ProjCopies { bool rm, r8, sc, km, fm, q4; int f8bit; bool q4w; };
static ProjCopies copies_of(const ProjW& w) { return {w.rm != nullptr, w.r8 != nullptr, w.sc != nullptr, w.km != nullptr, w.fm != nullptr, w.q4 != nullptr, w.f8bit, w.q4 != nullptr && w.q4w}; }
static ProjCopies copies_planned(const emmax_model* m, int stage) {
    const bool pair = stage == STAGE_QKV || stage == STAGE_GATEUP;
    const bool fm = m->fp8 || (!m->mx4 && (!pair || (m->aux_built ? m->aux_ab : emmax_tune().km == 0)));
    const int bit = stage == STAGE_QKV ? F8_QKV : stage == STAGE_OPROJ ? F8_OPROJ : stage == STAGE_GATEUP ? F8_GATEUP : stage == STAGE_DOWN ? F8_DOWN : F8_LMHEAD;
    return {true, m->fp8, m->fp8, !m->mx4, fm, m->mx4, bit, m->mx4 && m->mx4_wide};
}

enum { ROUTE_NO_FM = -1 };
static int proj_route(const ProjCopies& c, ProjShape s, int B, ProjGeom* g) {
    if (s.exact) {
        s.wfmt = PW_BF16;
        if (c.sc || c.q4) return EMMAX_VIA_NONE;
        if (B < EMMAX_MFMA_MIN_BATCH) return decode_ks_takes(s, B, g) ? EMMAX_VIA_KS : EMMAX_VIA_NONE;
        return c.km && decode_km_enabled() && decode_km_takes(s, B, g) ? EMMAX_VIA_KM : EMMAX_VIA_NONE;
    }
    if (c.q4) {
        s.wfmt = PW_MX4;
        if (c.f8bit == F8_DOWN && s.K <= 4096) return EMMAX_VIA_NONE;
        s.mx4_wide = c.q4w;
        if (!decode_km_takes(s, B, g)) return EMMAX_VIA_NONE;
        return B > 16 ? EMMAX_VIA_KMP : EMMAX_VIA_KM;
    }
    s.wfmt = c.sc ? PW_FP8 : PW_BF16;
    if (B < EMMAX_MFMA_MIN_BATCH && c.sc && c.r8 && (fp8_gemv_mask(B) & c.f8bit) && decode_gemv_takes(s, B, g)) return EMMAX_VIA_GEMV_FP8;
    if (B >= EMMAX_MFMA_MIN_BATCH || c.sc) {
        if (c.km && decode_km_enabled() && decode_km_takes(s, B, g)) return B > 16 ? EMMAX_VIA_KMP : EMMAX_VIA_KM;
        if (!c.fm) return ROUTE_NO_FM;
        return decode_mfma_takes(s, B, g) ? EMMAX_VIA_MFMA : EMMAX_VIA_NONE;
    }
    if (decode_ks_enabled() && decode_ks_takes(s, B, g)) return EMMAX_VIA_KS;
    return decode_gemv_takes(s, B, g) ? EMMAX_VIA_GEMV : EMMAX_VIA_NONE;
}

static int launch_proj(const ProjW& w, GemvParams& p, int B, hipStream_t st, int* grid_out, int* via = nullptr) {
    const int mode = w.gemv_mode;
    ProjGeom g;
    const int route = proj_route(copies_of(w), proj_shape(mode, p), B, &g);
    if (via) *via = route > 0 ? route : EMMAX_VIA_NONE;
    switch (route) {
        case EMMAX_VIA_KS:
            p.W = w.rm;
            return launch_decode_ks(mode, p, B, st, grid_out, &g);
        case EMMAX_VIA_GEMV:
            p.W = w.rm;
            return launch_decode_gemv_staged(mode, p, B, g, st, grid_out);
        case EMMAX_VIA_GEMV_FP8:
            p.W = w.r8; p.wscale = w.sc;
            p.ldw = p.K;
            return launch_decode_gemv_staged(mode, p, B, g, st, grid_out);
        case EMMAX_VIA_KM:
        case EMMAX_VIA_KMP:
            if (w.q4) { p.W = w.q4; p.w4_scales = w.q4s; }
            else { p.W = w.km; p.wscale = w.sc ? w.km_sc : nullptr; }
            return launch_decode_km(mode, p, B, st, grid_out, &g);
        case EMMAX_VIA_MFMA:
            p.W = w.fm; p.wscale = w.sc;
            return launch_decode_mfma(mode, p, B, st, grid_out, &g);
        case ROUTE_NO_FM:
            return fail(EMMAX_ERR_STATE, "decode_mfma.hip's copy of this matrix was not built (tuning switch km was 1 at emmax_model_build_aux)");
        default: break;
    }
    if (p.exact) return fail(EMMAX_ERR_INVALID, "exact numerics: no two-term kernel for this projection (batch %d, K %d)", B, p.K);
    if (w.q4) return fail(EMMAX_ERR_INVALID, "MXFP4 decode weights: no kernel for this projection (batch %d of 1-%d, K %d)", B, w.q4w ? EMMAX_MAX_DECODE_BATCH : 16, p.K);
    return -1;
}

int stage_chunk(int stage, bool exact) {
    return exact ? 8 : (stage == STAGE_DOWN || stage == STAGE_LMHEAD) ? EMMAX_KMP_ROWS : EMMAX_MAX_DECODE_BATCH;
}

static bool attn_direct_on(const emmax_model* m, bool exact, int B) {
    if (exact && B < EMMAX_MFMA_MIN_BATCH) return false;
    return decode_attn_nsplit(B, m->cfg.n_kv_heads) == 1 && emmax_tune().attn_direct != 0;
}
static bool attn_direct_on(const emmax_session* s, int B) { return attn_direct_on(s->m, s->exact, B); }

int attn_group_rows(const emmax_session* s, int B) {
    const int N = s->grp_N > 0 ? s->grp_N : (s->beam.K >= 2 && s->beam.forked) ? s->beam.K : 0;
    const int sw = emmax_tune().attn_group;
    if (N < 2 || s->exact || sw == 0 || !attn_direct_on(s, B)) return 0;
    if (sw < 0 && !(s->grp_N >= 4 && s->grp_N <= 16 && (B == 32 || B == 48 || B == 64))) return 0;
    return group_attn_takes(B, N, s->m->cfg.n_heads, s->m->cfg.n_kv_heads) ? N : 0;
}

int decode_oproj_form(const emmax_model* m, bool exact, int B, int* nsplit) {
    const bool direct = attn_direct_on(m, exact, B);
    if (nsplit) *nsplit = direct ? 1 : decode_attn_nsplit(B, m->cfg.n_kv_heads);
    return !direct ? 1 : (exact ? 2 : 0);
}

static ProjShape stage_shape(const emmax_model* m, int stage, int B, bool exact) {
    ProjShape s = {};
    s.exact = exact; s.h32 = exact || emmax_tune().resid32 != 0; s.ld_ok = true;
    switch (stage) {
        case STAGE_QKV: s.mode = GEMV_QKV; s.K = m->H; s.n_rows = m->qkv_dim; s.head_dim = m->cfg.head_dim; s.Hq = m->cfg.n_heads; break;
        case STAGE_OPROJ:
            s.mode = GEMV_RESID; s.K = m->q_dim; s.n_rows = m->H;
            if (decode_oproj_form(m, exact, B, &s.nsplit) == 1) { s.attn_part = true; s.Hq = m->cfg.n_heads; }
            break;
        case STAGE_GATEUP: s.mode = GEMV_GATEUP; s.K = m->H; s.n_rows = 2 * m->inter_p; break;
        case STAGE_DOWN: s.mode = GEMV_RESID; s.K = m->inter_p; s.n_rows = m->H; break;
        default: s.mode = GEMV_LMHEAD; s.K = m->H; s.n_rows = m->vocab; s.max_parts = EMMAX_LM_BLOCKS;
    }
    return s;
}

bool decode_batch_served(const emmax_model* m, int B, bool exact) {
    if (exact || B <= 8) return true;
    return emmax_tune().attn_direct != 0 && decode_attn_nsplit(9, m->cfg.n_kv_heads) == 1 && m->inter_p > 4096;
}

int decode_stage_route(const emmax_model* m, int stage, int B, bool exact) {
    if (!decode_batch_served(m, B, exact)) return EMMAX_VIA_NONE;
    const ProjShape s = stage_shape(m, stage, B, exact);
    const ProjCopies c = copies_planned(m, stage);
    const int chunk = stage_chunk(stage, exact);
    int via = EMMAX_VIA_NONE, n_prev = 0;
    for (int r = 0; r < B && via >= 0; r += chunk) {
        const int n = std::min(chunk, B - r);
        ProjGeom g;
        if (n != n_prev && (via = proj_route(c, s, n, &g)) == EMMAX_VIA_NONE) break;
        n_prev = n;
    }
    return via;
}

static const int kProjStages[] = {STAGE_QKV, STAGE_OPROJ, STAGE_GATEUP, STAGE_DOWN, STAGE_LMHEAD};
const char* decode_stage_name(int stage) {
    return stage == STAGE_QKV ? "qkv" : stage == STAGE_OPROJ ? "o-proj" : stage == STAGE_GATEUP ? "gate/up" : stage == STAGE_DOWN ? "down" : "lm-head";
}

int model_max_decode_batch(const emmax_model* m, bool exact, int* first_stage, int* first_B) {
    for (int B = 1; B <= EMMAX_MAX_DECODE_BATCH; ++B)
        for (int stage : kProjStages)
            if (decode_stage_route(m, stage, B, exact) <= 0) {
                if (first_stage) *first_stage = stage;
                if (first_B) *first_B = B;
                return B - 1;
            }
    return EMMAX_MAX_DECODE_BATCH;
}
int session_max_rows(const emmax_session* s) { return model_max_decode_batch(s->m, s->exact); }

static void stage_params(emmax_session* s, int B, int li, int stage, GemvParams& p) {
    emmax_model* m = s->m;
    const auto& c = m->cfg;
    const LayerW& L = m->layers[li];
    memset(&p, 0, sizeof(p));
    p.sk_ws = streamk_on() ? s->sk_ws : nullptr;
    if (stage != STAGE_ATTN) { p.h32 = h32_of(s); p.ldh = m->H; }
    if (s->exact) { p.exact = 1; p.h32 = s->dh32; p.ldh = m->H; }
    switch (stage) {
        case STAGE_QKV:
            p.x = s->dh; p.ldx = m->H; p.ldw = m->H; p.K = m->H; p.norm_w = L.ln1; p.eps = c.rms_eps;
            p.y = s->dq; p.ldy = m->q_dim; p.n_rows = m->qkv_dim;
            p.head_dim = c.head_dim; p.Hq = c.n_heads; p.Hkv = c.n_kv_heads; p.page = PAGE; p.max_pages = s->max_pages;
            p.ctx_len = s->ctx_len; p.page_table = s->page_table; p.cos_t = s->cos_t; p.sin_t = s->sin_t;
            p.kcache = kcache_of(s, li); p.vcache = vcache_of(s, li);
            p.kv_stage = s->kv8 ? s->kv_stage : nullptr;
            if (s->exact) { p.y = s->dq32; p.kv24 = s->kv24; }
            break;
        case STAGE_OPROJ:
            p.x = s->datt; p.ldx = m->q_dim; p.ldw = m->q_dim; p.K = m->q_dim; p.y = s->dh; p.ldy = m->H; p.n_rows = m->H;
            if (!attn_direct_on(s, B)) {
                p.attn_part = s->part; p.nsplit = decode_attn_nsplit(B, c.n_kv_heads); p.Hq = c.n_heads;
            } else if (s->exact) {
                p.x = s->dq32;
            }
            break;
        case STAGE_GATEUP:
            p.x = s->dh; p.ldx = m->H; p.ldw = m->H; p.K = m->H; p.norm_w = L.ln2; p.eps = c.rms_eps;
            p.y = s->dact; p.ldy = m->inter_p; p.n_rows = 2 * m->inter_p;
            if (s->exact) p.y = s->dact32;
            break;
        case STAGE_DOWN:
            p.x = s->dact; p.ldx = m->inter_p; p.ldw = m->inter_p; p.K = m->inter_p; p.y = s->dh; p.ldy = m->H; p.n_rows = m->H;
            if (s->exact) p.x = s->dact32;
            break;
        default: break;
    }
}
static void lmhead_params(emmax_session* s, int slot0, float* logits_out, GemvParams& p) {
    emmax_model* m = s->m;
    memset(&p, 0, sizeof(p));
    p.sk_ws = streamk_on() ? (slot0 >= s->stg0 ? s->sk_ws2 : s->sk_ws) : nullptr;
    p.x = s->dh + (size_t)slot0 * m->H; p.ldx = m->H; p.ldw = m->H; p.K = m->H; p.norm_w = m->final_norm; p.eps = m->cfg.rms_eps;
    p.h32 = h32_of(s, slot0); p.ldh = m->H;
    if (s->exact) { p.exact = 1; p.h32 = s->dh32 + (size_t)slot0 * m->H; }
    const bool stg = slot0 >= s->stg0;
    p.n_rows = m->vocab; p.max_parts = s->n_lm_blocks; p.part_val = stg ? s->part_val2 : s->part_val; p.part_idx = stg ? s->part_idx2 : s->part_idx;
    p.logits_out = logits_out;
}

enum { FINISH_WARP = 1 << 13, FINISH_RULES = 1 << 14, FINISH_EXT = FINISH_WARP | FINISH_RULES, FINISH_ROWS = 6 | FINISH_EXT  };
static int finish_mode(const emmax_session* s) {
    return (s->samp.on ? 1 : 0) | (s->proc.on ? 2 : 0) | (s->scores.on ? 4 : 0) |
           (s->beam.K ? (8 | (s->beam.eos >= 0 ? 16 : 0) | (s->beam.K << 5) | (s->beam.es << 10) | (s->beam.lp_pos << 12)) : 0) |
           (s->warp.on ? FINISH_WARP : 0) | (s->rules.on ? FINISH_RULES : 0);
}

static void finish_rows(emmax_session* s, int B, bool is_prefill, int slot0, FinishParams& f) {
    emmax_model* m = s->m;
    f.B = B;
    f.cur_tok = s->cur_tok + slot0; f.ctx_len = s->ctx_len + slot0; f.done = s->done + slot0; f.n_out = s->n_out + slot0;
    f.out_ids = s->out_ids + (size_t)slot0 * s->max_out;
    f.max_new_p = s->max_new_d + slot0; f.max_out = s->max_out; f.max_ctx = s->max_ctx;
    f.stop_ids = s->stop_ids; f.stop_cfg = s->stop_cfg; f.stop_m = s->stop_m + slot0; f.stop_after = s->stop_after + slot0;
// ... 347 lines not shown
```

emma-x_amd/emmax/_lib.py:

```python

from __future__ import annotations

import ctypes as C
import os
from typing import Optional

_HERE = os.path.dirname(os.path.abspath(__file__))
LIB_PATH = os.path.join(_HERE, "libemmax_hip.so")

_c_i32p = C.POINTER(C.c_int32)
_c_i64p = C.POINTER(C.c_int64)
_c_f32p = C.POINTER(C.c_float)
_vp = C.c_void_p


class EmmaxError(RuntimeError):
    pass


class TowerConfigC(C.Structure):
    _fields_ = [
        ("embed_dim", C.c_int32), ("depth", C.c_int32), ("num_heads", C.c_int32), ("mlp_hidden", C.c_int32),
        ("has_cls", C.c_int32), ("n_reg", C.c_int32), ("layerscale", C.c_int32),
        ("patch", C.c_int32), ("image_size", C.c_int32), ("take_index", C.c_int32),
        ("ln_eps", C.c_float), ("mean", C.c_float * 3), ("std", C.c_float * 3),
    ]


class ConfigC(C.Structure):
    _fields_ = [
        ("tower", TowerConfigC * 2),
        ("hidden", C.c_int32), ("inter", C.c_int32), ("n_layers", C.c_int32), ("n_heads", C.c_int32),
        ("n_kv_heads", C.c_int32), ("head_dim", C.c_int32), ("vocab", C.c_int32),
        ("rms_eps", C.c_float), ("rope_theta", C.c_float),
        ("bos_id", C.c_int32), ("eos_id", C.c_int32), ("pad_id", C.c_int32), ("decode_fp8", C.c_int32),
    ]


ABI_VERSION = 12

SIGNATURES = {
    "emmax_version": (C.c_char_p, []),
    "emmax_last_error": (C.c_char_p, []),
    "emmax_abi_version": (C.c_int, []),
    "emmax_config_size": (C.c_int, []),
    "emmax_tuning_set": (C.c_int, [C.c_char_p, C.c_int]),
    "emmax_tuning_get": (C.c_int, [C.c_char_p, C.POINTER(C.c_int)]),
    "emmax_model_create": (C.c_int, [C.POINTER(ConfigC), C.POINTER(_vp)]),
    "emmax_model_destroy": (None, [_vp]),
    "emmax_model_bind_weight": (C.c_int, [_vp, C.c_char_p, _vp, C.c_int, _c_i64p, C.c_int]),
    "emmax_model_arena_bytes": (C.c_int64, [_vp]),
    "emmax_model_max_decode_batch": (C.c_int, [_vp]),
    "emmax_model_max_decode_batch_exact": (C.c_int, [_vp]),
    "emmax_model_mxfp4_wide": (C.c_int, [_vp]),
    "emmax_config_max_decode_batch": (C.c_int, [C.POINTER(ConfigC), C.c_int]),
    "emmax_model_finalize": (C.c_int, [_vp, _vp, C.c_int64, _vp]),
    "emmax_model_aux_bytes": (C.c_int64, [_vp]),
    "emmax_model_build_aux": (C.c_int, [_vp, _vp, C.c_int64, _vp]),
    "emmax_session_bytes": (C.c_int, [_vp, C.c_int, C.c_int, C.c_int, _c_i64p, _c_i64p]),
    "emmax_session_create": (C.c_int, [_vp, C.c_int, C.c_int, C.c_int, _vp, C.c_int64, _vp, C.c_int64, C.POINTER(_vp)]),
    "emmax_session_bytes_ex": (C.c_int, [_vp, C.c_int, C.c_int, C.c_int, C.c_int, _c_i64p, _c_i64p]),
    "emmax_session_create_ex": (C.c_int, [_vp, C.c_int, C.c_int, C.c_int, C.c_int, _vp, C.c_int64, _vp, C.c_int64, C.POINTER(_vp)]),
    "emmax_session_stage_rows": (C.c_int, [_vp]),
    "emmax_session_destroy": (None, [_vp]),
    "emmax_vision_encode": (C.c_int, [_vp, _vp, C.c_int, _vp, _vp]),
    "emmax_vision_encode_pixels": (C.c_int, [_vp, _vp, C.c_int, _vp, _vp]),
    "emmax_vision_features": (C.c_int, [_vp, C.c_int, _vp, _vp]),
    "emmax_prefill": (C.c_int, [_vp, _vp, _c_i32p, C.c_int, C.c_int, _vp, _vp]),
    "emmax_prefill_text": (C.c_int, [_vp, _vp, _c_i32p, C.c_int, C.c_int, _vp]),
    "emmax_prefill_logits": (C.c_int, [_vp, _vp, _vp]),
    "emmax_last_logits": (C.c_int, [_vp, _vp, _vp]),
    "emmax_decode_step": (C.c_int, [_vp, _vp]),
    "emmax_set_current_tokens": (C.c_int, [_vp, _vp, _vp]),
    "emmax_generate": (C.c_int, [_vp, C.c_int, C.c_int, _vp, _vp, _vp]),
    "emmax_session_graph_active": (C.c_int, [_vp]),
    "emmax_profile_decode_stage": (C.c_int, [_vp, C.c_int, C.c_int, _c_f32p, _vp]),
    "emmax_session_set_stop": (C.c_int, [_vp, _vp, C.c_int, C.c_int, _vp]),
    "emmax_slots_open": (C.c_int, [_vp, C.c_int, _vp]),
    "emmax_slot_prefill": (C.c_int, [_vp, C.c_int, _vp, C.c_int, _vp, C.c_int, _vp]),
    "emmax_slots_prefill": (C.c_int, [_vp, C.c_int, C.c_int, _vp, C.c_int, _vp, _vp, _vp, _vp]),
    "emmax_slots_prefill_staged": (C.c_int, [_vp, C.c_int, _vp, C.c_int, _vp, _vp, _vp, _vp]),
    "emmax_slots_commit": (C.c_int, [_vp, _vp, _vp, C.c_int, _vp]),
    "emmax_slots_step": (C.c_int, [_vp, C.c_int, _vp]),
    "emmax_slots_state": (C.c_int, [_vp, _vp, _vp, _vp]),
    "emmax_slot_output": (C.c_int, [_vp, C.c_int, _vp, C.c_int, _vp]),
    "emmax_slot_release": (C.c_int, [_vp, C.c_int, _vp]),
    "emmax_slots_fork": (C.c_int, [_vp, C.c_int, C.c_int, _vp, C.c_int, _vp, _vp, _vp, _vp, _vp, _vp]),
    "emmax_slots_page_state": (C.c_int, [_vp, _vp, _vp, _vp]),
    "emmax_op_gemm": (C.c_int, [_vp, C.c_int, _vp, C.c_int, _vp, C.c_int, C.c_int, C.c_int, C.c_int, _vp, C.c_int, _vp, _vp,
                                C.c_int, C.c_int, _vp]),
    "emmax_op_gemm_splitk": (C.c_int, [_vp, C.c_int, _vp, C.c_int, _vp, C.c_int, C.c_int, C.c_int, C.c_int, _vp, C.c_int, _vp, _vp,
                                       C.c_int, C.c_int, C.c_int, _vp, C.c_int64, _vp]),
    "emmax_gemm_plan": (C.c_int, [C.c_int, C.c_int, C.c_int, C.c_int, C.c_int, C.c_int, C.c_int, C.c_int, C.c_int64, C.c_char_p, C.c_int]),
    "emmax_op_gemm_ln": (C.c_int, [_vp, C.c_int, _vp, C.c_int, _vp, C.c_int, C.c_int, C.c_int, C.c_int, _vp, _vp, _vp, C.c_float, C.c_int, _vp, _vp, _vp, _vp]),
    "emmax_op_layernorm": (C.c_int, [_vp, _vp, _vp, _vp, C.c_int, C.c_int, C.c_float, _vp]),
    "emmax_op_rmsnorm": (C.c_int, [_vp, _vp, _vp, C.c_int, C.c_int, C.c_float, _vp]),
    "emmax_op_attention": (C.c_int, [_vp, C.c_int, C.c_int, C.c_int, C.c_int, _vp, C.c_int, _vp, C.c_int, C.c_int, C.c_int,
                                     C.c_int, C.c_int, C.c_float, C.c_int, _vp]),
    "emmax_op_decode_attention": (C.c_int, [_vp, _vp, _vp, _vp, _vp, _vp, _vp, C.c_int, C.c_int, C.c_int, C.c_int, C.c_int, C.c_int,
                                            C.c_float, C.POINTER(C.c_int), _vp]),
    "emmax_op_decode_attention_direct": (C.c_int, [_vp, _vp, _vp, _vp, _vp, _vp, _vp, C.c_int, C.c_int, C.c_int, C.c_int, C.c_int, C.c_float, _vp]),
    "emmax_op_decode_attention_kv8": (C.c_int, [_vp, _vp, _vp, _vp, _vp, _vp, _vp, _vp, _vp, _vp, _vp, C.c_int, C.c_int, C.c_int, C.c_int, C.c_int, C.c_int,
                                                C.c_float, _vp]),
    "emmax_op_decode_attention_group": (C.c_int, [_vp, _vp, _vp, _vp, _vp, _vp, _vp, C.c_int, C.c_int, C.c_int, C.c_int, C.c_int, C.c_float, C.c_int, _vp, _vp, _vp]),
    "emmax_op_decode_attention_group_kv8": (C.c_int, [_vp, _vp, _vp, _vp, _vp, _vp, _vp, _vp, _vp, _vp, _vp, C.c_int, C.c_int, C.c_int, C.c_int, C.c_int, C.c_int,
                                                      _vp, C.c_float, _vp]),
    "emmax_op_gemv": (C.c_int, [_vp, _vp, _vp, C.c_int, C.c_int, C.c_int, _vp]),
    "emmax_op_resize_bicubic_u8": (C.c_int, [_vp, C.c_int, C.c_int, C.c_int, _vp, C.c_int, C.c_int, _vp, _vp, _vp, C.c_int, _vp, _vp, C.c_int, _vp]),
    "emmax_op_quant_fm8": (C.c_int, [_vp, C.c_int, _vp, _vp, C.c_int, C.c_int, _vp]),
    "emmax_op_quant_mxfp4": (C.c_int, [_vp, C.c_int, _vp, _vp, C.c_int, C.c_int, C.c_int, C.c_int, _vp]),
    "emmax_op_dequant_mxfp4": (C.c_int, [_vp, _vp, _vp, C.c_int, C.c_int, C.c_int, C.c_int, C.c_int, _vp]),
    "emmax_op_gemm_small_mxfp4": (C.c_int, [_vp, _vp, _vp, _vp, C.c_int, C.c_int, C.c_int, _vp]),
    "emmax_op_gemm_wide_mxfp4": (C.c_int, [_vp, _vp, _vp, _vp, C.c_int, C.c_int, C.c_int, _vp]),
    "emmax_op_gemm_small_fp8": (C.c_int, [_vp, _vp, _vp, _vp, C.c_int, C.c_int, C.c_int, _vp]),
    "emmax_op_quant_rm8": (C.c_int, [_vp, C.c_int, _vp, _vp, C.c_int, C.c_int, _vp]),
    "emmax_op_gemv_fp8": (C.c_int, [_vp, _vp, _vp, _vp, C.c_int, C.c_int, C.c_int, _vp]),
    "emmax_op_repack_fm": (C.c_int, [_vp, C.c_int, _vp, C.c_int, C.c_int, _vp]),
    "emmax_op_gemm_small": (C.c_int, [_vp, _vp, _vp, C.c_int, C.c_int, C.c_int, _vp]),
    "emmax_op_repack_km": (C.c_int, [_vp, C.c_int, _vp, C.c_int, C.c_int, C.c_int, C.c_int, _vp]),
    "emmax_op_gemm_small_km": (C.c_int, [_vp, _vp, _vp, C.c_int, C.c_int, C.c_int, _vp]),
    "emmax_session_exact": (C.c_int, [_vp]),
    "emmax_op_x_gemm": (C.c_int, [_vp, C.c_int, _vp, C.c_int, _vp, C.c_int, C.c_int, C.c_int, C.c_int, _vp, C.c_int, _vp, C.c_int, _vp, _vp, C.c_int64, _vp]),
    "emmax_op_x_rownorm": (C.c_int, [C.c_int, _vp, _vp, _vp, _vp, C.c_int, C.c_int, C.c_float, _vp, _vp]),
    "emmax_op_x_attention": (C.c_int, [_vp, C.c_int, C.c_int, C.c_int, C.c_int, _vp, C.c_int, C.c_int, C.c_int, C.c_int, C.c_int, C.c_float, C.c_int, _vp, _vp]),
    "emmax_op_x_join": (C.c_int, [_vp, _vp, C.c_int, C.c_int, _vp]),
    "emmax_op_x_decode_attention": (C.c_int, [_vp, _vp, _vp, C.c_int64, _vp, _vp, _vp, _vp, C.c_int, C.c_int, C.c_int, C.c_int, C.c_int, C.c_int, C.c_float, _vp]),
    "emmax_op_sample": (C.c_int, [_vp, C.c_int, C.c_int, C.c_int, _vp, _vp, _vp, _vp, _vp, _vp, _vp, _vp, _vp]),
    "emmax_session_set_sampling": (C.c_int, [_vp, C.c_int, C.c_int, _vp, _vp, _vp, _vp, _vp, _vp]),
    "emmax_slots_set_sampling_staged": (C.c_int, [_vp, C.c_int, _vp, _vp, _vp, _vp, _vp, _vp]),
    "emmax_session_clear_sampling": (C.c_int, [_vp, _vp]),
    "emmax_session_sampling": (C.c_int, [_vp]),
    "emmax_session_logprobs": (C.c_int, [_vp, C.c_int, _vp, _vp]),
    "emmax_slot_logprobs": (C.c_int, [_vp, C.c_int, _vp, C.c_int, _vp]),
    "emmax_session_set_processing": (C.c_int, [_vp, C.c_int, C.c_int, _vp, _vp, _vp, _vp]),
    "emmax_slots_set_processing_staged": (C.c_int, [_vp, C.c_int, _vp, _vp, _vp, _vp]),
    "emmax_session_clear_processing": (C.c_int, [_vp, _vp]),
    "emmax_session_processing": (C.c_int, [_vp]),
    "emmax_session_set_scores": (C.c_int, [_vp, _vp, _vp, C.c_int, _vp]),
    "emmax_session_set_warpers": (C.c_int, [_vp, C.c_int, C.c_int, _vp, _vp, _vp, _vp, _vp]),
    "emmax_slots_set_warpers_staged": (C.c_int, [_vp, C.c_int, _vp, _vp, _vp, _vp, _vp]),
    "emmax_session_clear_warpers": (C.c_int, [_vp, _vp]),
    "emmax_session_warpers": (C.c_int, [_vp]),
    "emmax_session_set_token_rules": (C.c_int, [_vp, C.c_int, _vp, _vp, _vp, _vp, _vp]),
    "emmax_session_set_rule_enables": (C.c_int, [_vp, C.c_int, C.c_int, _vp, _vp]),
    "emmax_slots_set_rule_enables_staged": (C.c_int, [_vp, C.c_int, _vp, _vp]),
    "emmax_session_clear_token_rules": (C.c_int, [_vp, _vp]),
    "emmax_session_token_rules": (C.c_int, [_vp]),
    "emmax_op_sample_ext": (C.c_int, [_vp, C.c_int, C.c_int, C.c_int, _vp, _vp, _vp, _vp, _vp, _vp, _vp, _vp, _vp, _vp, _vp, _vp, _vp, _vp, _vp, C.c_int, C.c_int,
                                      _vp, _vp, _vp, _vp, _vp, C.c_int, C.c_int, _vp, _vp, _vp, _vp]),
    "emmax_session_set_beams": (C.c_int, [_vp, C.c_int, C.c_double, C.c_int, _vp]),
    "emmax_session_clear_beams": (C.c_int, [_vp, _vp]),
    "emmax_session_beams": (C.c_int, [_vp]),
    "emmax_session_beam_result": (C.c_int, [_vp, C.c_int, _vp, _vp, _vp, _vp, _vp]),
    "emmax_session_beam_trace": (C.c_int, [_vp, C.c_int, _vp, _vp, _vp, _vp, _vp, _vp, _vp]),
    "emmax_session_set_sample_groups": (C.c_int, [_vp, C.c_int, _vp]),
    "emmax_session_clear_sample_groups": (C.c_int, [_vp, _vp]),
    "emmax_session_sample_groups": (C.c_int, [_vp]),
    "emmax_session_attn_grouped": (C.c_int, [_vp, C.c_int]),
    "emmax_op_decode_stage": (C.c_int, [_vp, C.c_int, C.c_int, C.c_int, _vp, _vp, _c_i32p, _c_i32p, _vp, _vp, _vp, _vp, _vp, C.POINTER(C.c_int),
                                        C.POINTER(C.c_int), C.POINTER(C.c_int), _vp]),
    "emmax_op_decode_route": (C.c_int, [_vp, C.c_int, C.c_int, C.c_int, C.POINTER(C.c_int)]),
    "emmax_op_decode_kv_read": (C.c_int, [_vp, C.c_int, C.c_int, C.c_int, C.c_int, _c_i32p, C.c_int, _c_f32p, _c_f32p, _vp]),
    "emmax_op_gemm_stream": (C.c_int, [_vp, C.c_int, _vp, C.c_int, _vp, C.c_int, _vp, C.c_int, C.c_int, C.c_int, C.c_int, _vp, C.c_int, _vp, C.c_int, C.c_int, _vp, C.c_int64,
                                       _vp, _vp, C.c_int, C.c_float, _vp]),
    "emmax_op_rmsnorm_f32": (C.c_int, [_vp, C.c_int, _vp, C.c_int, _vp, C.c_int, C.c_int, C.c_float, _vp]),
    "emmax_op_rope_kv_write": (C.c_int, [_vp, C.c_int, C.c_int, C.c_int, C.c_int, _vp, C.c_int, C.c_int, _vp, _vp, _vp, _vp, _vp, C.c_int, C.c_int, C.c_int, C.c_int,
                                         C.c_int, _vp]),
    "emmax_op_kv_quant_rows": (C.c_int, [_vp, C.c_int, C.c_int, C.c_int, _vp, C.c_int, C.c_int, _vp, _vp, _vp, _vp, _vp, C.c_int, C.c_int, C.c_int, C.c_int, _vp]),
    "emmax_op_embed_splice": (C.c_int, [_vp, C.c_int, _vp, _vp, _vp, _vp, _vp, C.c_int, C.c_int, C.c_int, C.c_int, C.c_int, _vp]),
    "emmax_op_gather_last_rows": (C.c_int, [_vp, _vp, _vp, _vp, _vp, C.c_int, C.c_int, _vp]),
}

_lib: Optional[C.CDLL] = None


def load() -> C.CDLL:
    global _lib
    if _lib is not None:
        return _lib
    if not os.path.isfile(LIB_PATH):
        raise EmmaxError(
            f"{LIB_PATH} not found: the HIP extension is not built. Run `python -c 'import __graft_entry__ as g; g.build()'` "
            "or `make -C emma-x_amd/csrc`. There is no CPU fallback for the product path.")
    lib = C.CDLL(LIB_PATH)
    for name, (res, args) in SIGNATURES.items():
        fn = getattr(lib, name)
        fn.restype = res
        fn.argtypes = args
    if lib.emmax_abi_version() != ABI_VERSION:
        raise EmmaxError(f"ABI mismatch: library reports {lib.emmax_abi_version()}, host expects {ABI_VERSION}")
    if lib.emmax_config_size() != C.sizeof(ConfigC):
        raise EmmaxError(f"emmax_config is {lib.emmax_config_size()} bytes in the library, {C.sizeof(ConfigC)} in this binding")
    _lib = lib
    return lib
# ... 55 lines not shown
```

emma-x_amd/emmax/engine.py:

```python

from __future__ import annotations

import ctypes as C
import os
from typing import Dict, List, Optional, Sequence, Tuple

import torch

from . import _lib
from .config import DECODE_WEIGHT_DTYPES, EmmaXConfig, check_decode_weight_dtype
from .weights import param_shapes, validate_state_dict


def _config_c(cfg: EmmaXConfig) -> _lib.ConfigC:
    c = _lib.ConfigC()
    for i, tw in enumerate(cfg.towers):
        t = c.tower[i]
        t.embed_dim, t.depth, t.num_heads, t.mlp_hidden = tw.embed_dim, tw.depth, tw.num_heads, tw.mlp_hidden
        t.has_cls, t.n_reg, t.layerscale = int(tw.has_cls), tw.n_reg, int(tw.layerscale)
        t.patch, t.image_size, t.take_index = tw.patch, tw.image_size, tw.take_index
        t.ln_eps = tw.ln_eps
        for j in range(3):
            t.mean[j] = tw.mean[j]
            t.std[j] = tw.std[j]
    L = cfg.llm
    c.hidden, c.inter, c.n_layers, c.n_heads, c.n_kv_heads, c.head_dim, c.vocab = (
        L.hidden_size, L.intermediate_size, L.num_layers, L.num_heads, L.num_kv_heads, L.head_dim, L.vocab_size)
    c.rms_eps, c.rope_theta = L.rms_eps, L.rope_theta
    c.bos_id, c.eos_id, c.pad_id = cfg.bos_token_id, cfg.eos_token_id, cfg.pad_token_id
    c.decode_fp8 = DECODE_WEIGHT_DTYPES[check_decode_weight_dtype(getattr(cfg, "decode_weight_dtype", "bf16"))]
    return c


class _Staged:

    def __init__(self, n, event, keep):
        self.n, self.event, self.keep, self.committed = n, event, keep, 0

    def ready(self) -> bool:
        return self.event.query()

    def wait(self) -> None:
        self.event.synchronize()


def _device_bytes(nbytes: int, device, what: str):
    return torch.empty(nbytes, dtype=torch.uint8, device=device)


class EmmaxEngine:

    def __init__(self, cfg: EmmaXConfig, state_dict: Dict[str, torch.Tensor], device: str = "cuda:0",
                 max_batch: int = 1, max_prompt: int = 512, max_ctx: Optional[int] = None, free_state_dict: bool = False,
                 exact: Optional[bool] = None, mxfp4_wide: Optional[bool] = None):
        if mxfp4_wide and cfg.decode_weight_dtype != "mxfp4":
            raise ValueError(f"mxfp4_wide serves MXFP4 decode weights at 17-64 rows: this config has decode_weight_dtype={cfg.decode_weight_dtype!r}")
        self.lib = _lib.load()
        self.exact = int(_lib.tuning_get("exact")) if exact is None else int(exact)
        self.cfg = cfg
        self.device = torch.device(device)
        if self.device.type != "cuda":
            raise _lib.EmmaxError("EmmaxEngine needs a HIP device (cuda:N); the product path has no CPU fallback")
        validate_state_dict(state_dict, cfg)
        torch.cuda.set_device(self.device)
        self._model = C.c_void_p()
        self._session = C.c_void_p()
        cc = _config_c(cfg)
        with _lib.tuning(**({} if mxfp4_wide is None else {"mx4_wide": int(bool(mxfp4_wide))})):
            _lib.check(self.lib.emmax_model_create(C.byref(cc), C.byref(self._model)), "emmax_model_create")
        self.mxfp4_wide = bool(self.lib.emmax_model_mxfp4_wide(self._model) == 1)
        keep: List[torch.Tensor] = []
        for key, shape, _ in param_shapes(cfg):
            t = state_dict[key]
            if t.device != self.device or t.dtype != torch.bfloat16 or not t.is_contiguous():
                t = t.to(device=self.device, dtype=torch.bfloat16).contiguous()
            keep.append(t)
            shp = (C.c_int64 * t.ndim)(*t.shape)
            _lib.check(self.lib.emmax_model_bind_weight(self._model, key.encode(), t.data_ptr(), 0, shp, t.ndim),
                       f"bind {key}")
            if free_state_dict:
                state_dict[key] = None
        nbytes = self.lib.emmax_model_arena_bytes(self._model)
        self.arena = _device_bytes(nbytes, self.device, "ARENA")
        stream = _lib.current_stream()
        import time

        t0 = time.perf_counter()
        with _lib.tuning(exact=int(self.exact)):
            _lib.check(self.lib.emmax_model_finalize(self._model, self.arena.data_ptr(), nbytes, stream), "emmax_model_finalize")
        self.finalize_s = time.perf_counter() - t0
        self.aux_build_s = 0.0
        del keep
        self.aux_arena: Optional[torch.Tensor] = None
        self.max_batch = self.max_prompt = self.max_ctx = 0
        self._resize_tables: Dict[Tuple[int, int, int], tuple] = {}
        self._adm_stream = None
        self._commit_event = None
        self.new_session(max_batch, max_prompt, max_ctx)

    def new_session(self, max_batch: int, max_prompt: int, max_ctx: Optional[int] = None, stage_rows: int = 0) -> None:
        if self._session:
            self.lib.emmax_session_destroy(self._session)
            self._session = C.c_void_p()
        np_ = self.cfg.n_patches
        if max_ctx is None:
            max_ctx = np_ + max_prompt + 512 + 1
        ws, kv = C.c_int64(), C.c_int64()
        with _lib.tuning(exact=int(self.exact)):
            _lib.check(self.lib.emmax_session_bytes_ex(self._model, max_batch, max_prompt, max_ctx, int(stage_rows), C.byref(ws), C.byref(kv)),
                       "emmax_session_bytes_ex")
            self.workspace = torch.empty(ws.value, dtype=torch.uint8, device=self.device)
            self.kv = _device_bytes(kv.value, self.device, "KV")
            _lib.check(self.lib.emmax_session_create_ex(self._model, max_batch, max_prompt, max_ctx, int(stage_rows), self.workspace.data_ptr(),
                                                        ws.value, self.kv.data_ptr(), kv.value, C.byref(self._session)),
                       "emmax_session_create_ex")
        assert bool(self.lib.emmax_session_exact(self._session)) == bool(self.exact)
        self._score_bufs = None
        self._beam_K = 0
        self._group_N = 0
        self.max_batch, self.max_prompt, self.max_ctx, self.stage_rows = max_batch, max_prompt, max_ctx, int(stage_rows)

    def ensure_stage_rows(self, n: int) -> None:
        if n > self.stage_rows:
            self.new_session(max(self.max_batch, int(n)), self.max_prompt, self.max_ctx, stage_rows=int(n))

    def ensure_decode_batch(self, batch: int) -> None:
        if batch < 3 or self.aux_arena is not None:
            return
        n = int(self.lib.emmax_model_aux_bytes(self._model))
        import time

        t0 = time.perf_counter()
        self.aux_arena = _device_bytes(max(n, 256), self.device, "AUX")
        _lib.check(self.lib.emmax_model_build_aux(self._model, self.aux_arena.data_ptr(), n, _lib.current_stream()), "emmax_model_build_aux")
        self.aux_build_s = time.perf_counter() - t0

    @property
    def patch_dtype(self) -> torch.dtype:
        return torch.float32 if self.exact else torch.bfloat16

    def max_decode_batch(self) -> int:
        if self.exact:
            return int(self.lib.emmax_model_max_decode_batch_exact(self._model))
        return int(self.lib.emmax_model_max_decode_batch(self._model))

    def weight_bytes(self) -> int:
        return int(self.arena.numel()) + (int(self.aux_arena.numel()) if self.aux_arena is not None else 0)

    def ensure_capacity(self, batch: int, prompt: int, max_new: int) -> None:
        need_ctx = self.cfg.n_patches + prompt + max_new + 1
        if batch > self.max_batch or prompt > self.max_prompt or need_ctx > self.max_ctx:
            self.new_session(max(batch, self.max_batch), max(prompt, self.max_prompt), max(need_ctx, self.max_ctx),
                             stage_rows=self.stage_rows)

    def close(self) -> None:
        if getattr(self, "_session", None):
            self.lib.emmax_session_destroy(self._session)
            self._session = C.c_void_p()
        if getattr(self, "_model", None):
            self.lib.emmax_model_destroy(self._model)
            self._model = C.c_void_p()

    def __del__(self):
        try:
            self.close()
        except Exception:
            pass

    def vision_encode(self, frames_u8: torch.Tensor) -> torch.Tensor:
        assert frames_u8.dtype == torch.uint8 and frames_u8.is_cuda and frames_u8.is_contiguous()
        frames_u8 = self.resize_frames(frames_u8)
        B = frames_u8.shape[0]
        out = torch.empty(B, self.cfg.n_patches, self.cfg.llm.hidden_size, dtype=self.patch_dtype, device=self.device)
        _lib.check(self.lib.emmax_vision_encode(self._session, frames_u8.data_ptr(), B, out.data_ptr(), _lib.current_stream()),
                   "emmax_vision_encode")
        return out

    def resize_frames(self, frames_u8: torch.Tensor, size: Optional[int] = None) -> torch.Tensor:
        from .resize import bicubic_coeffs

        size = size or self.cfg.towers[0].image_size
        B, H, W, _ = frames_u8.shape
        if H == size and W == size:
            return frames_u8
        assert frames_u8.dtype == torch.uint8 and frames_u8.is_cuda and frames_u8.is_contiguous()
        key = (H, W, size)
        if key not in self._resize_tables:
            bh, kh, nh = bicubic_coeffs(W, size)
            bv, kv, nv = bicubic_coeffs(H, size)
            self._resize_tables[key] = tuple(torch.from_numpy(a.copy()).to(self.device) for a in (bh, kh, bv, kv)) + (nh, nv)
        bh, kh, bv, kv, nh, nv = self._resize_tables[key]
        out = torch.empty(B, size, size, 3, dtype=torch.uint8, device=self.device)
        tmp = torch.empty(B, H, size, 3, dtype=torch.uint8, device=self.device)
        _lib.check(self.lib.emmax_op_resize_bicubic_u8(frames_u8.data_ptr(), B, H, W, out.data_ptr(), size, size, tmp.data_ptr(),
                                                       bh.data_ptr(), kh.data_ptr(), nh, bv.data_ptr(), kv.data_ptr(), nv,
                                                       _lib.current_stream()), "emmax_op_resize_bicubic_u8")
        return out

    def vision_encode_pixels(self, pixel_values: torch.Tensor) -> torch.Tensor:
        pv = pixel_values.to(device=self.device, dtype=torch.bfloat16).contiguous()
        B = pv.shape[0]
        out = torch.empty(B, self.cfg.n_patches, self.cfg.llm.hidden_size, dtype=self.patch_dtype, device=self.device)
        _lib.check(self.lib.emmax_vision_encode_pixels(self._session, pv.data_ptr(), B, out.data_ptr(), _lib.current_stream()),
                   "emmax_vision_encode_pixels")
        return out

    def vision_features(self, B: int) -> torch.Tensor:
        out = torch.empty(B, self.cfg.n_patches, self.cfg.vision_dim, dtype=torch.bfloat16, device=self.device)
        _lib.check(self.lib.emmax_vision_features(self._session, B, out.data_ptr(), _lib.current_stream()), "emmax_vision_features")
        return out

    def _pack_prompts(self, who: str, prompts: Sequence[Sequence[int]], pad: int, patch_embeds: Optional[Sequence[torch.Tensor]] = None):
        lens = [len(p) for p in prompts]
        P_max = max(lens)
        ids = torch.full((len(prompts), P_max), pad, dtype=torch.int32)
        for i, p in enumerate(prompts):
            ids[i, : lens[i]] = torch.as_tensor(list(p), dtype=torch.int32)
        pe = None
        if patch_embeds is not None:
            if len(patch_embeds) != len(prompts):
                raise ValueError(f"{who}: one patch-embedding tensor per prompt")
            pe = torch.stack([t.reshape(self.cfg.n_patches, self.cfg.llm.hidden_size) for t in patch_embeds]).contiguous()
            assert pe.dtype == self.patch_dtype
        return ids.to(self.device), lens, P_max, pe

    def prefill(self, input_ids: Sequence[Sequence[int]], patch_embeds: torch.Tensor) -> List[int]:
        B = len(input_ids)
        K = self._beam_K
        N = self._group_N or 1
        self.ensure_decode_batch(B * (K or N))
# ... 358 lines not shown
```

include/emmax.h:

```cpp
#ifndef EMMAX_H
#define EMMAX_H

#include <stdint.h>

#ifdef __cplusplus
extern "C" {
#endif

#define EMMAX_ABI_VERSION 12

typedef enum emmax_status {
    EMMAX_OK = 0,
    EMMAX_ERR_INVALID = -1,
    EMMAX_ERR_MISSING = -2,
    EMMAX_ERR_NOMEM = -3,
    EMMAX_ERR_HIP = -4,
    EMMAX_ERR_STATE = -5
} emmax_status;

typedef enum emmax_dtype { EMMAX_BF16 = 0, EMMAX_F32 = 1, EMMAX_U8 = 2, EMMAX_I32 = 3 } emmax_dtype;

typedef void* emmax_stream;
typedef struct emmax_model emmax_model;
typedef struct emmax_session emmax_session;

typedef struct emmax_tower_config {
    int32_t embed_dim, depth, num_heads, mlp_hidden;
    int32_t has_cls, n_reg, layerscale;
    int32_t patch, image_size;
    int32_t take_index;
    float ln_eps;
    float mean[3], std[3];
} emmax_tower_config;

typedef struct emmax_config {
    emmax_tower_config tower[2];
    int32_t hidden, inter, n_layers, n_heads, n_kv_heads, head_dim, vocab;
    float rms_eps, rope_theta;
    int32_t bos_id, eos_id, pad_id;
    int32_t decode_fp8;
} emmax_config;

const char* emmax_version(void);
const char* emmax_last_error(void);
int emmax_abi_version(void);
int emmax_config_size(void);

int emmax_tuning_set(const char* name, int value);
int emmax_tuning_get(const char* name, int* value_out);

int emmax_model_create(const emmax_config* cfg, emmax_model** out);
void emmax_model_destroy(emmax_model* m);
int emmax_model_bind_weight(emmax_model* m, const char* hf_key, const void* ptr_dev, int dtype,
                            const int64_t* shape, int ndim);
int64_t emmax_model_arena_bytes(const emmax_model* m);
int emmax_model_max_decode_batch(const emmax_model* m);
int emmax_model_max_decode_batch_exact(const emmax_model* m);
int emmax_model_mxfp4_wide(const emmax_model* m);
int emmax_config_max_decode_batch(const emmax_config* cfg, int exact);
int emmax_model_finalize(emmax_model* m, void* arena_dev, int64_t arena_bytes, emmax_stream stream);
int64_t emmax_model_aux_bytes(const emmax_model* m);
int emmax_model_build_aux(emmax_model* m, void* aux_arena_dev, int64_t aux_bytes, emmax_stream stream);

int emmax_session_bytes(const emmax_model* m, int max_batch, int max_prompt, int max_ctx,
                        int64_t* workspace_bytes, int64_t* kv_bytes);
int emmax_session_create(emmax_model* m, int max_batch, int max_prompt, int max_ctx,
                         void* workspace_dev, int64_t workspace_bytes, void* kv_dev, int64_t kv_bytes,
                         emmax_session** out);
int emmax_session_bytes_ex(const emmax_model* m, int max_batch, int max_prompt, int max_ctx, int stage_rows,
                           int64_t* workspace_bytes, int64_t* kv_bytes);
int emmax_session_create_ex(emmax_model* m, int max_batch, int max_prompt, int max_ctx, int stage_rows,
                            void* workspace_dev, int64_t workspace_bytes, void* kv_dev, int64_t kv_bytes,
                            emmax_session** out);
int emmax_session_stage_rows(const emmax_session* s);
int emmax_session_exact(const emmax_session* s);
void emmax_session_destroy(emmax_session* s);

int emmax_vision_encode(emmax_session* s, const uint8_t* frames_u8_dev, int B, void* patch_embeds_out_dev,
                        emmax_stream stream);
int emmax_vision_encode_pixels(emmax_session* s, const void* pixel_values_bf16_dev, int B, void* patch_embeds_out_dev,
                               emmax_stream stream);
int emmax_vision_features(emmax_session* s, int B, void* feats_out_dev, emmax_stream stream);

int emmax_prefill(emmax_session* s, const int32_t* ids_dev, const int32_t* lens_host, int B, int P_max,
                  const void* patch_embeds_dev, emmax_stream stream);
int emmax_prefill_text(emmax_session* s, const int32_t* ids_dev, const int32_t* lens_host, int B, int P_max, emmax_stream stream);
int emmax_prefill_logits(emmax_session* s, float* logits_out_dev, emmax_stream stream);
int emmax_last_logits(emmax_session* s, float* logits_out_dev, emmax_stream stream);

int emmax_decode_step(emmax_session* s, emmax_stream stream);
int emmax_set_current_tokens(emmax_session* s, const int32_t* tokens_dev, emmax_stream stream);
int emmax_generate(emmax_session* s, int max_new_tokens, int stop_on_eos, int32_t* out_ids_dev, int32_t* out_lens_dev,
                   emmax_stream stream);

int emmax_session_graph_active(emmax_session* s);
int emmax_profile_decode_stage(emmax_session* s, int stage, int reps, float* avg_us_out, emmax_stream stream);

int emmax_session_set_stop(emmax_session* s, const int32_t* trigger_ids_host, int n_trigger, int n_after, emmax_stream stream);
int emmax_slots_open(emmax_session* s, int n_slots, emmax_stream stream);
int emmax_slot_prefill(emmax_session* s, int slot, const int32_t* ids_dev, int len, const void* patch_embeds_dev, int max_new,
                       emmax_stream stream);
int emmax_slots_prefill(emmax_session* s, int slot0, int n, const int32_t* ids_dev, int P_max, const int32_t* lens_host,
                        const void* patch_embeds_dev, const int32_t* max_new_host, emmax_stream stream);
int emmax_slots_prefill_staged(emmax_session* s, int n, const int32_t* ids_dev, int P_max, const int32_t* lens_host,
                               const void* patch_embeds_dev, const int32_t* max_new_host, emmax_stream stream);
int emmax_slots_commit(emmax_session* s, const int32_t* staged_idx_host, const int32_t* slots_host, int n, emmax_stream stream);
int emmax_slots_step(emmax_session* s, int n_steps, emmax_stream stream);
int emmax_slots_state(emmax_session* s, int32_t* done_dev, int32_t* n_out_dev, emmax_stream stream);
int emmax_slot_output(emmax_session* s, int slot, int32_t* ids_dev, int n, emmax_stream stream);
int emmax_slot_release(emmax_session* s, int slot, emmax_stream stream);

int emmax_op_sample(const float* logits_dev, int ld, int B, int V, const float* temperature_dev, const int32_t* top_k_dev, const float* top_p_dev,
                    const uint64_t* seed_dev, const uint32_t* subseq_dev, const int32_t* step_dev, int32_t* tok_out_dev, float* logprob_out_dev,
                    emmax_stream stream);

int emmax_session_set_sampling(emmax_session* s, int row0, int n, const float* temperature_host, const int32_t* top_k_host, const float* top_p_host,
                               const uint64_t* seed_host, const uint32_t* subseq_host, emmax_stream stream);
int emmax_slots_set_sampling_staged(emmax_session* s, int n, const float* temperature_host, const int32_t* top_k_host, const float* top_p_host,
                                    const uint64_t* seed_host, const uint32_t* subseq_host, emmax_stream stream);
int emmax_session_clear_sampling(emmax_session* s, emmax_stream stream);
int emmax_session_sampling(const emmax_session* s);
int emmax_session_logprobs(emmax_session* s, int max_new, float* out_dev, emmax_stream stream);
int emmax_slot_logprobs(emmax_session* s, int slot, float* out_dev, int n, emmax_stream stream);

int emmax_session_set_processing(emmax_session* s, int row0, int n, const float* penalty_host, const int32_t* ngram_host, const int32_t* min_new_host,
                                 emmax_stream stream);
int emmax_slots_set_processing_staged(emmax_session* s, int n, const float* penalty_host, const int32_t* ngram_host, const int32_t* min_new_host,
                                      emmax_stream stream);
int emmax_session_clear_processing(emmax_session* s, emmax_stream stream);
int emmax_session_processing(const emmax_session* s);
int emmax_session_set_scores(emmax_session* s, float* scores_dev, float* logits_dev, int max_new, emmax_stream stream);

int emmax_session_set_warpers(emmax_session* s, int row0, int n, const float* min_p_host, const float* typical_p_host, const float* epsilon_cutoff_host,
                              const float* eta_cutoff_host, emmax_stream stream);
int emmax_slots_set_warpers_staged(emmax_session* s, int n, const float* min_p_host, const float* typical_p_host, const float* epsilon_cutoff_host,
                                   const float* eta_cutoff_host, emmax_stream stream);
int emmax_session_clear_warpers(emmax_session* s, emmax_stream stream);
int emmax_session_warpers(const emmax_session* s);
int emmax_session_set_token_rules(emmax_session* s, int n_rules, const int32_t* offsets_host, const int32_t* ids_host, const int32_t* flags_host,
                                  const float* bias_host, emmax_stream stream);
int emmax_session_set_rule_enables(emmax_session* s, int row0, int n, const uint32_t* enable_host, emmax_stream stream);
int emmax_slots_set_rule_enables_staged(emmax_session* s, int n, const uint32_t* enable_host, emmax_stream stream);
int emmax_session_clear_token_rules(emmax_session* s, emmax_stream stream);
int emmax_session_token_rules(const emmax_session* s);
int emmax_op_sample_ext(const float* logits_dev, int ld, int B, int V, const float* temperature_dev, const int32_t* top_k_dev, const float* top_p_dev,
                        const uint64_t* seed_dev, const uint32_t* subseq_dev, const int32_t* n_out_dev, const float* min_p_dev, const float* typical_p_dev,
                        const float* epsilon_cutoff_dev, const float* eta_cutoff_dev, const float* penalty_dev, const int32_t* ngram_dev,
                        const int32_t* min_new_dev, const int32_t* hist_dev, const int32_t* hist_len_dev, int max_hist, int n_rules,
                        const int32_t* rule_off_dev, const int32_t* rule_ids_dev, const int32_t* rule_flags_dev, const float* rule_bias_dev,
                        const uint32_t* rule_enable_dev, int eos_id, int pad_id, int32_t* tok_out_dev, float* logprob_out_dev, float* scores_out_dev,
                        emmax_stream stream);

#define EMMAX_MAX_BEAMS 8
int emmax_session_set_beams(emmax_session* s, int num_beams, double length_penalty, int early_stopping, emmax_stream stream);
int emmax_session_clear_beams(emmax_session* s, emmax_stream stream);
int emmax_session_beams(const emmax_session* s);
int emmax_session_beam_result(emmax_session* s, int max_new, int32_t* seq_dev, int32_t* len_dev, float* score_dev, int32_t* beam_indices_dev,
                              emmax_stream stream);
int emmax_session_beam_trace(emmax_session* s, int max_new, int32_t* tok_dev, int32_t* parent_dev, float* score_dev, float* lse_dev,
                             int32_t* cand_idx_dev, float* cand_acc_dev, emmax_stream stream);

int emmax_session_set_sample_groups(emmax_session* s, int n, emmax_stream stream);
int emmax_session_clear_sample_groups(emmax_session* s, emmax_stream stream);
int emmax_session_sample_groups(const emmax_session* s);
int emmax_session_attn_grouped(const emmax_session* s, int B);

int emmax_slots_fork(emmax_session* s, int src_slot, int staged_idx, const int32_t* dst_slots_host, int n, const float* temperature_host,
                     const int32_t* top_k_host, const float* top_p_host, const uint64_t* seed_host, const uint32_t* subseq_host, emmax_stream stream);
int emmax_slots_page_state(emmax_session* s, int32_t* table_out_dev, int32_t* hidden_out_dev, emmax_stream stream);

int emmax_op_gemm(const void* A_dev, int lda, const void* W_dev, int ldw, void* C_dev, int ldc, int M, int N, int K,
                  const void* bias_dev, int act, const void* scale_dev, const void* residual_dev, int ldr, int out_f32,
                  emmax_stream stream);
int emmax_op_gemm_splitk(const void* A_dev, int lda, const void* W_dev, int ldw, void* C_dev, int ldc, int M, int N, int K,
                         const void* bias_dev, int act, const void* scale_dev, const void* residual_dev, int ldr, int out_f32,
                         int ksplit, void* ws_dev, int64_t ws_bytes, emmax_stream stream);
int emmax_gemm_plan(int M, int N, int K, int act, int out_f32, int has_ln, int has_residual, int with_norm, int64_t ws_bytes, char* text_out,
                    int text_len);
int emmax_op_gemm_ln(const void* X_dev, int ldx, void* W_dev, int ldw, void* C_dev, int ldc, int M, int N, int K, const void* gamma_dev,
                     const void* beta_dev, const void* bias_dev, float eps, int act, float* stats_ws_dev, float* ln_s_ws_dev,
                     float* ln_c_ws_dev, emmax_stream stream);
int emmax_op_layernorm(const void* x_dev, void* y_dev, const void* w_dev, const void* b_dev, int rows, int D, float eps,
                       emmax_stream stream);
int emmax_op_rmsnorm(const void* x_dev, void* y_dev, const void* w_dev, int rows, int D, float eps, emmax_stream stream);
int emmax_op_attention(const void* qkv_dev, int ld_qkv, int q_off, int k_off, int v_off, void* out_dev, int ld_out,
                       const int32_t* cu_seqlens_dev, int B, int max_seqlen, int Hq, int Hkv, int head_dim, float scale,
                       int causal, emmax_stream stream);
int emmax_op_decode_attention(const void* q_dev, const void* kcache_dev, const void* vcache_dev, const int32_t* page_table_dev,
                              const int32_t* ctx_len_dev, const int32_t* done_dev, float* part_out_dev, int B, int Hq, int Hkv,
                              int page, int max_pages, int nsplit, float scale, int* nsplit_out, emmax_stream stream);
int emmax_op_decode_attention_direct(const void* q_dev, const void* kcache_dev, const void* vcache_dev, const int32_t* page_table_dev,
                                     const int32_t* ctx_len_dev, const int32_t* done_dev, void* o_out_dev, int B, int Hq, int Hkv,
                                     int page, int max_pages, float scale, emmax_stream stream);
int emmax_op_decode_attention_kv8(const void* q_dev, void* kcache8_dev, void* vcache8_dev, float* kscale_dev, float* vscale_dev,
                                  const void* kv_stage_dev, const int32_t* page_table_dev, const int32_t* ctx_len_dev, const int32_t* done_dev,
                                  float* partials_out_dev, void* o_out_dev, int B, int Hq, int Hkv, int page, int max_pages, int nsplit,
                                  float scale, emmax_stream stream);
int emmax_op_decode_attention_group(const void* q_dev, const void* kcache_dev, const void* vcache_dev, const int32_t* page_table_dev,
                                    const int32_t* ctx_len_dev, const int32_t* done_dev, void* o_out_dev, int B, int Hq, int Hkv, int page,
                                    int max_pages, float scale, int N, const int32_t* shared_pages_dev, float* part_ws_dev, emmax_stream stream);
int emmax_op_decode_attention_group_kv8(const void* q_dev, void* kcache8_dev, void* vcache8_dev, float* kscale_dev, float* vscale_dev,
                                        const void* kv_stage_dev, const int32_t* page_table_dev, const int32_t* ctx_len_dev,
                                        const int32_t* done_dev, float* part_ws_dev, void* o_out_dev, int B, int Hq, int Hkv, int page,
                                        int max_pages, int N, const int32_t* shared_pages_dev, float scale, emmax_stream stream);
int emmax_op_gemv(const void* x_dev, const void* W_dev, void* y_dev, int B, int N, int K, emmax_stream stream);

int emmax_op_resize_bicubic_u8(const uint8_t* src_dev, int B, int H, int W, uint8_t* dst_dev, int OH, int OW, uint8_t* tmp_dev,
                               const int32_t* bounds_h_dev, const int32_t* kk_h_dev, int ksize_h, const int32_t* bounds_v_dev,
                               const int32_t* kk_v_dev, int ksize_v, emmax_stream stream);

int emmax_op_quant_fm8(const void* W_dev, int ld, void* W8_fm_out_dev, float* scales_out_dev, int N, int K, emmax_stream stream);
int emmax_op_quant_mxfp4(const void* W_dev, int ld, void* tiles_out_dev, void* scales_out_dev, int N, int K, int perm, int perm_hd, emmax_stream stream);
int emmax_op_dequant_mxfp4(const void* tiles_dev, const void* scales_dev, void* W_out_dev, int ld, int N, int K, int perm, int perm_hd, emmax_stream stream);
int emmax_op_gemm_small_mxfp4(const void* x_dev, const void* tiles_dev, const void* scales_dev, void* y_dev, int B, int N, int K, emmax_stream stream);
int emmax_op_gemm_wide_mxfp4(const void* x_dev, const void* tiles_dev, const void* scales_dev, void* y_dev, int B, int N, int K, emmax_stream stream);
int emmax_op_gemm_small_fp8(const void* x_dev, const void* W8_fm_dev, const float* scales_dev, void* y_dev, int B, int N, int K,
                            emmax_stream stream);
int emmax_op_repack_km(const void* W_dev, int ld, void* W_km_dev, int N, int K, int perm, int head_dim, emmax_stream stream);
int emmax_op_gemm_small_km(const void* x_dev, const void* W_km_dev, void* y_dev, int B, int N, int K, emmax_stream stream);
int emmax_op_quant_rm8(const void* W_dev, int ld, void* W8_rows_out_dev, float* scales_out_dev, int N, int K, emmax_stream stream);
int emmax_op_gemv_fp8(const void* x_dev, const void* W8_rows_dev, const float* scales_dev, void* y_dev, int B, int N, int K,
                      emmax_stream stream);
int emmax_op_repack_fm(const void* W_dev, int ld, void* W_fm_out_dev, int N, int K, emmax_stream stream);
int emmax_op_gemm_small(const void* x_dev, const void* W_fm_dev, void* y_dev, int B, int N, int K, emmax_stream stream);

enum { EMMAX_VIA_NONE = 0, EMMAX_VIA_KS = 1, EMMAX_VIA_GEMV = 2, EMMAX_VIA_GEMV_FP8 = 3, EMMAX_VIA_KM = 4, EMMAX_VIA_KMP = 5, EMMAX_VIA_MFMA = 6 };
int emmax_op_decode_stage(emmax_session* s, int layer, int stage, int B, const void* h_in_dev, const float* h32_in_dev, const int32_t* ctx_len_host,
                          const int32_t* page_table_host, const void* x_in_dev, void* h_out_dev, float* h32_out_dev, void* y_out_dev,
                          int32_t* tok_out_dev, int* via_out, int* oproj_form_out, int* nsplit_out, emmax_stream stream);
int emmax_op_decode_route(const emmax_model* m, int stage, int B, int exact, int* via_out);
int emmax_op_decode_kv_read(emmax_session* s, int layer, int row, int p0, int n, const int32_t* page_row_host, int from_stage, float* k_out_host,
                            float* v_out_host, emmax_stream stream);

int emmax_op_gemm_stream(const void* A_dev, int lda, const void* W_dev, int ldw, float* C32_dev, int ldc, const float* residual32_dev, int ldr, int M, int N,
                         int K, const void* bias_dev, int act, const void* scale_dev, int n_store, int ksplit, void* ws_dev, int64_t ws_bytes,
                         const void* norm_w_dev, void* norm_out_dev, int ld_norm, float eps, emmax_stream stream);
int emmax_op_rmsnorm_f32(const float* x_dev, int ldx, void* y_dev, int ldy, const void* w_dev, int rows, int D, float eps, emmax_stream stream);
int emmax_op_rope_kv_write(void* qkv_dev, int ld, int q_off, int k_off, int v_off, const int32_t* cu_seqlens_dev, int B, int total_rows, const float* cos_dev,
                           const float* sin_dev, void* kcache_dev, void* vcache_dev, const int32_t* page_table_dev, int max_pages, int Hq, int Hkv, int head_dim,
                           int page, emmax_stream stream);
int emmax_op_kv_quant_rows(void* qkv_dev, int ld, int k_off, int v_off, const int32_t* cu_seqlens_dev, int B, int total_rows, void* k8_dev, void* v8_dev,
                           float* kscale_dev, float* vscale_dev, const int32_t* page_table_dev, int max_pages, int Hkv, int head_dim, int page, emmax_stream stream);
int emmax_op_embed_splice(const int32_t* ids_dev, int P_max, const int32_t* cu_seqlens_dev, const void* embed_dev, const void* patches_dev, void* h_dev,
                          float* h32_dev, int B, int max_seqlen, int n_patches, int hidden, int vocab, emmax_stream stream);
int emmax_op_gather_last_rows(const void* in_dev, const float* in32_dev, void* out_dev, float* out32_dev, const int32_t* cu_seqlens_dev, int B, int D,
                              emmax_stream stream);

int emmax_op_x_gemm(const float* A32_dev, int lda, const void* W_dev, int ldw, float* C32_dev, int ldc, int M, int N, int K, const void* bias_dev, int act,
                    const float* residual32_dev, int ldr, void* hl_ws_dev, void* ws_dev, int64_t ws_bytes, emmax_stream stream);
int emmax_op_x_rownorm(int mode, const float* x_dev, float* y32_dev, const void* w_dev, const void* b_dev, int rows, int D, float eps, void* hl_ws_dev,
                       emmax_stream stream);
int emmax_op_x_attention(const float* qkv32_dev, int ld_qkv, int q_off, int k_off, int v_off, const int32_t* cu_seqlens_dev, int B, int max_seqlen, int Hq,
                         int Hkv, int head_dim, float scale, int causal, void* hl_ws_dev, emmax_stream stream);
int emmax_op_x_join(const void* hl_dev, float* out32_dev, int rows, int D, emmax_stream stream);
int emmax_op_x_decode_attention(const float* q32_dev, const void* kcache_dev, const void* vcache_dev, int64_t kv24_elems, const int32_t* page_table_dev,
                                const int32_t* ctx_len_dev, const int32_t* done_dev, float* part_out_dev, int B, int Hq, int Hkv, int page, int max_pages,
                                int nsplit, float scale, emmax_stream stream);

#ifdef __cplusplus
}
#endif
#endif
```

Measured before the change: 0.7505 actions/s.

## Stream batch-1 decode projection weights from a lossless packed 13-slot format

Adds a packed weight layout for batch-1 split-K decode GEMVs. Each 16-row batch is stored in 13 slots plus a per-region header byte per row, with an overflow area holding raw rows for regions that cannot be packed. The kernel expands rows in registers, prefetches the next region's header through scalar loads, and interleaves the next batch's loads with the current dot products. The aim is to cut weight bytes read from HBM in memory-bound decode. In exchange it costs an extra packed weight arena, a build pass at setup, and extra unpack ALU work per row.

```diff
diff --git a/emma-x_amd/csrc/decode_ks.hip b/emma-x_amd/csrc/decode_ks.hip
--- a/emma-x_amd/csrc/decode_ks.hip
+++ b/emma-x_amd/csrc/decode_ks.hip
@@ -3,6 +3,7 @@
 #include "common.h"
 #include "kernels.h"
 #include "decode_epilogue.h"
+#include "pk13.h"
 
 #ifndef KS_W_AUX
 #define KS_W_AUX 2
@@ -86,27 +87,79 @@
 #else
 #define KS_STAMP(op, k, v) do { } while (0)
 #endif
-template <int MODE>
-__device__ __forceinline__ void ks_pair_rows(const GemvParams& p, int g, int& r0, int& r1) {
-    if (MODE == GEMV_QKV) {
-        const int half = p.head_dim >> 1;
-        const int hb = g >> p.ks_shift, d = g - hb * half;
-        r0 = hb * p.head_dim + d;
+__device__ __forceinline__ void ks_pair_rows_of(int mode, int head_dim, int shift, int n_rows, int g, int& r0, int& r1) {
+    if (mode == GEMV_QKV) {
+        const int half = head_dim >> 1;
+        const int hb = g >> shift, d = g - hb * half;
+        r0 = hb * head_dim + d;
         r1 = r0 + half;
-    } else if (MODE == GEMV_GATEUP) {
+    } else if (mode == GEMV_GATEUP) {
         r0 = (g >> 4) * 32 + (g & 15);
         r1 = r0 + 16;
     } else {
         r0 = 2 * g;
-        r1 = min(2 * g + 1, p.n_rows - 1);
-    }
-}
-__device__ __forceinline__ void ks_share(const GemvParams& p, int& g_lo, int& npairs) {
-    const int G = gridDim.x, bid = blockIdx.x;
-    const int q = p.n_groups / G, r = p.n_groups % G;
+        r1 = min(2 * g + 1, n_rows - 1);
+    }
+}
+template <int MODE>
+__device__ __forceinline__ void ks_pair_rows(const GemvParams& p, int g, int& r0, int& r1) {
+    ks_pair_rows_of(MODE, p.head_dim, p.ks_shift, p.n_rows, g, r0, r1);
+}
+__device__ __forceinline__ void ks_share_of(int n_groups, int G, int bid, int& g_lo, int& npairs) {
+    const int q = n_groups / G, r = n_groups % G;
     g_lo = bid * q + min(bid, r);
-    npairs = min(q + (bid < r ? 1 : 0), max(p.n_groups - g_lo, 0));
-}
+    npairs = min(q + (bid < r ? 1 : 0), max(n_groups - g_lo, 0));
+}
+__device__ __forceinline__ void ks_share(const GemvParams& p, int& g_lo, int& npairs) { ks_share_of(p.n_groups, gridDim.x, blockIdx.x, g_lo, npairs); }
+
+__host__ __device__ inline int ks_pk_batches(int npairs) { return (2 * npairs + PK13_ROWS - 1) / PK13_ROWS; }
+__host__ __device__ inline int ks_pk_first_batch(int n_groups, int G, int bid) {
+    const int q = n_groups / G, r = n_groups % G;
+    return bid * ks_pk_batches(q) + (bid < r ? bid : r) * (ks_pk_batches(q + 1) - ks_pk_batches(q));
+}
+__host__ __device__ inline unsigned ks_pk_block_bytes(int npairs) {
+    const int rows = 2 * npairs, rem = rows % PK13_ROWS;
+    return (unsigned)(rows / PK13_ROWS + (rem > 8 ? 1 : 0)) * (unsigned)PK13_REGION + (rem > 0 && rem <= 8 ? (unsigned)PK13_HALF : 0u);
+}
+__host__ __device__ inline unsigned ks_pk_first_byte(int n_groups, int G, int bid) {
+    const int q = n_groups / G, r = n_groups % G;
+    return (unsigned)bid * ks_pk_block_bytes(q) + (unsigned)(bid < r ? bid : r) * (ks_pk_block_bytes(q + 1) - ks_pk_block_bytes(q));
+}
+struct KsPkHdr { u32x4_t a, b; };
+__device__ __forceinline__ KsPkHdr ks_pk_hdr(const void* hdr, int region) {
+    typedef const __attribute__((address_space(4))) u32x4_t* cptr_t;
+    const cptr_t h = (cptr_t)((uintptr_t)hdr + (size_t)region * PK13_HDR);
+    return {h[0], h[2]};
+}
+__device__ __forceinline__ KsPkHdr ks_pk_hdr_request(const void* hdr, int region) {
+    const uint64_t addr = (uint64_t)(uintptr_t)hdr + (uint64_t)region * PK13_HDR;
+    KsPkHdr h;
+    asm volatile("s_load_dwordx4 %0, %2, 0x0\n\ts_load_dwordx4 %1, %2, 0x20" : "=&s"(h.a), "=&s"(h.b) : "s"(addr));
+    return h;
+}
+__device__ __forceinline__ void ks_pk_hdr_wait(KsPkHdr& h) { asm volatile("s_waitcnt lgkmcnt(0)" : "+s"(h.a), "+s"(h.b)); }
+template <int JJ>
+__device__ __forceinline__ uint32_t ks_pk_bb(const KsPkHdr& h) {
+    const uint32_t w = (JJ >> 3) ? h.b[(JJ & 7) >> 2] : h.a[(JJ & 7) >> 2];
+    return ((w >> (8 * (JJ & 3))) & 0xffu) * 0x10001u;
+}
+__device__ __forceinline__ void ks_issue_pk(__amdgpu_buffer_rsrc_t rs, unsigned so, unsigned so_b, unsigned lane16, u32x4_t (&wr)[16]) {
+#pragma unroll
+    for (int L = 0; L < PK13_SLOTS; ++L)
+        wr[L] = __builtin_bit_cast(u32x4_t, __builtin_amdgcn_raw_buffer_load_b128(rs, lane16, (L < PK13_HALF / 1024 ? so : so_b) + L * 1024u, KS_W_AUX));
+}
+template <int L>
+__device__ __forceinline__ void ks_load_pk(__amdgpu_buffer_rsrc_t rs, unsigned so, unsigned so_b, unsigned lane16, u32x4_t (&wr)[16]) {
+    wr[L] = __builtin_bit_cast(u32x4_t, __builtin_amdgcn_raw_buffer_load_b128(rs, lane16, (L < PK13_HALF / 1024 ? so : so_b) + L * 1024u, KS_W_AUX));
+}
+__device__ __forceinline__ void ks_issue_ovf(__amdgpu_buffer_rsrc_t rs, unsigned so, unsigned lane16, u32x4_t (&wr)[16]) {
+#pragma unroll
+    for (int L = 0; L < PK13_ROWS; ++L) wr[L] = __builtin_bit_cast(u32x4_t, __builtin_amdgcn_raw_buffer_load_b128(rs, lane16, so + L * 1024u, KS_W_AUX));
+}
+template <int N> struct KsUnroll {
+    template <class F> static __device__ __forceinline__ void run(F&& f) { KsUnroll<N - 1>::run(f); f(std::integral_constant<int, N - 1>{}); }
+};
+template <> struct KsUnroll<0> { template <class F> static __device__ __forceinline__ void run(F&&) {} };
 
 template <int B, int MODE, int CPL>
 __device__ __forceinline__ void ks_issue(const GemvParams& p, int g_lo, int nrows, int bb, const unsigned (&voff)[CPL], u32x4_t (&wr)[KsRegs<B>::N]) {
@@ -126,6 +179,19 @@
     }
 }
 
+template <int B, int MODE, int CPL, bool PK>
+__device__ __forceinline__ void ks_issue_first(const GemvParams& p, int g_lo, int nrows, const unsigned (&voff)[CPL], u32x4_t (&wr)[KsRegs<B>::N]) {
+    if constexpr (PK) {
+        const int wave = __builtin_amdgcn_readfirstlane(threadIdx.x >> 6);
+        __builtin_amdgcn_sched_barrier(0);
+        const unsigned piece = nrows <= 8 ? (unsigned)PK13_HALF : (unsigned)PK13_REGION;
+        const unsigned so = ks_pk_first_byte(p.n_groups, gridDim.x, blockIdx.x) * KS_WAVES + (unsigned)wave * piece;
+        ks_issue_pk(__builtin_amdgcn_make_buffer_rsrc((void*)p.W, 0, (int)p.pk_bytes, 0x00020000), so, nrows <= 8 ? p.pk_bytes : so, (threadIdx.x & 63) * 16u, wr);
+    } else {
+        ks_issue<B, MODE, CPL>(p, g_lo, nrows, 0, voff, wr);
+    }
+}
+
 template <int CPL>
 __device__ __forceinline__ void ks_chunks(int K, int wave, int lane, int (&coff)[CPL], bool (&cok)[CPL], unsigned (&voff)[CPL]) {
     const int NCW = K >> 6;
@@ -138,10 +204,11 @@
     }
 }
 
-template <int B, int MODE, bool NORM, int XS, int CPL, bool R32, bool EX = false>
+template <int B, int MODE, bool NORM, int XS, int CPL, bool R32, bool EX = false, bool PK = false>
 __device__ __forceinline__ void ks_run_op(const GemvParams& p, u32x4_t (&wr)[KsRegs<B>::N], float* part, float* sumsq, int rows_cap,
                                           int trace_op = -1) {
     constexpr int RB = KsShape<B, CPL>::RB;
+    static_assert(!PK || (B == 1 && CPL == 1 && !EX && RB == PK13_ROWS), "the pk13 regions are batch-1 batches of one chunk per lane");
     KS_STAMP(trace_op, 0, wall_clock64());
     const int tid = threadIdx.x, lane = tid & 63, wave = __builtin_amdgcn_readfirstlane(tid >> 6);
     const int K = p.K, bid = blockIdx.x;
@@ -179,7 +246,7 @@
         for (int b = 0; b < B; ++b)
 #pragma unroll
             for (int j = 0; j < CPL; ++j) xq[b][j] = ld_f32x8((const float*)p.x + (size_t)b * p.ldx + (size_t)coff[j] * 8);
-        ks_issue<B, MODE, CPL>(p, g_lo, nrows, 0, voff, wr);
+        ks_issue_first<B, MODE, CPL, PK>(p, g_lo, nrows, voff, wr);
 #pragma unroll
         for (int b = 0; b < B; ++b)
 #pragma unroll
@@ -213,7 +280,7 @@
                 }
             }
         __builtin_amdgcn_sched_barrier(0);
-        ks_issue<B, MODE, CPL>(p, g_lo, nrows, 0, voff, wr);
+        ks_issue_first<B, MODE, CPL, PK>(p, g_lo, nrows, voff, wr);
     } else {
         u32x4_t nw[CPL];
         if constexpr (NORM) {
@@ -227,7 +294,7 @@
             for (int b = 0; b < B; ++b)
 #pragma unroll
                 for (int j = 0; j < CPL; ++j) xq[b][j] = ld_f32x8(p.h32 + (size_t)b * p.ldh + (size_t)coff[j] * 8);
-            ks_issue<B, MODE, CPL>(p, g_lo, nrows, 0, voff, wr);
+            ks_issue_first<B, MODE, CPL, PK>(p, g_lo, nrows, voff, wr);
 #pragma unroll
             for (int b = 0; b < B; ++b) {
                 ss[b] = 0.f;
@@ -267,7 +334,7 @@
                     }
                 }
             }
-            ks_issue<B, MODE, CPL>(p, g_lo, nrows, 0, voff, wr);
+            ks_issue_first<B, MODE, CPL, PK>(p, g_lo, nrows, voff, wr);
 #pragma unroll
             for (int b = 0; b < B; ++b) {
                 ss[b] = 0.f;
@@ -302,6 +369,64 @@
 
     KS_STAMP(trace_op, 1, wall_clock64());
     const int nbatch = (nrows + RB - 1) / RB;
+    if constexpr (PK) {
+        const __amdgpu_buffer_rsrc_t prs = __builtin_amdgcn_make_buffer_rsrc((void*)p.W, 0, (int)p.pk_bytes, 0x00020000);
+        const __amdgpu_buffer_rsrc_t ors = __builtin_amdgcn_make_buffer_rsrc((void*)p.pk_ovf, 0, (int)p.pk_ovf_bytes, 0x00020000);
+        const int reg0 = ks_pk_first_batch(p.n_groups, gridDim.x, bid) * KS_WAVES + wave;
+        const unsigned lane16 = (unsigned)lane * 16u, byte0 = ks_pk_first_byte(p.n_groups, gridDim.x, bid) * KS_WAVES;
+        KsPkHdr cur = ks_pk_hdr_request(p.pk_hdr, reg0);
+        ks_pk_hdr_wait(cur);
+        for (int bb = 0; bb < nbatch; ++bb) {
+            KsPkHdr nxt = ks_pk_hdr_request(p.pk_hdr, reg0 + KS_WAVES * min(bb + 1, nbatch - 1));
+            const bool more = bb + 1 < nbatch, half = nrows - (bb + 1) * RB <= 8;
+            const unsigned so = more ? byte0 + (unsigned)(bb + 1) * (unsigned)(KS_WAVES * PK13_REGION) + (unsigned)wave * (half ? (unsigned)PK13_HALF : (unsigned)PK13_REGION) : p.pk_bytes;
+            const unsigned so_b = half ? p.pk_bytes : so;
+            const int oi = (int)cur.a[2];
+            float acc[1][RB];
+            if (oi >= 0) {
+                ks_issue_ovf(ors, (unsigned)oi * (unsigned)PK13_OVF, lane16, wr);
+#pragma unroll
+                for (int jj = 0; jj < RB; ++jj) {
+                    float a = 0.f;
+                    a = dot2_bf16(wr[jj][0], xr[0][0][0], a);
+                    a = dot2_bf16(wr[jj][1], xr[0][0][1], a);
+                    a = dot2_bf16(wr[jj][2], xr[0][0][2], a);
+                    a = dot2_bf16(wr[jj][3], xr[0][0][3], a);
+                    acc[0][jj] = a;
+                }
+                __builtin_amdgcn_sched_barrier(0);
+                ks_issue_pk(prs, so, so_b, lane16, wr);
+                __builtin_amdgcn_sched_barrier(0);
+            } else {
+                uint32_t s6a = 0u, s6b = 0u;
+                KsUnroll<RB>::run([&](auto J) {
+                    constexpr int jj = decltype(J)::value;
+                    const u32x4_t w = pk13_expand<jj>(wr, ks_pk_bb<jj>(cur), s6a, s6b);
+                    float a = 0.f;
+                    a = dot2_bf16(w[0], xr[0][0][0], a);
+                    a = dot2_bf16(w[1], xr[0][0][1], a);
+                    a = dot2_bf16(w[2], xr[0][0][2], a);
+                    a = dot2_bf16(w[3], xr[0][0][3], a);
+                    acc[0][jj] = a;
+                    if constexpr ((jj & 3) == 3) {
+                        __builtin_amdgcn_sched_barrier(0);
+                        if constexpr (jj == 3) { ks_load_pk<0>(prs, so, so_b, lane16, wr); ks_load_pk<1>(prs, so, so_b, lane16, wr); ks_load_pk<3>(prs, so, so_b, lane16, wr); }
+                        if constexpr (jj == 7) {
+                            asm volatile("v_mov_b32 %0, %2\n\tv_mov_b32 %1, %3" : "=&v"(s6a), "=&v"(s6b) : "v"(wr[6][2]), "v"(wr[6][3]));
+                            ks_load_pk<2>(prs, so, so_b, lane16, wr); ks_load_pk<4>(prs, so, so_b, lane16, wr); ks_load_pk<5>(prs, so, so_b, lane16, wr); ks_load_pk<6>(prs, so, so_b, lane16, wr); }
+                        if constexpr (jj == 11) { ks_load_pk<7>(prs, so, so_b, lane16, wr); ks_load_pk<8>(prs, so, so_b, lane16, wr); ks_load_pk<10>(prs, so, so_b, lane16, wr); }
+                        if constexpr (jj == 15) { ks_load_pk<9>(prs, so, so_b, lane16, wr); ks_load_pk<11>(prs, so, so_b, lane16, wr); ks_load_pk<12>(prs, so, so_b, lane16, wr); }
+                        __builtin_amdgcn_sched_barrier(0);
+                    }
+                });
+            }
+            ks_pk_hdr_wait(nxt);
+            cur = nxt;
+            __builtin_amdgcn_sched_barrier(0);
+            const float t = ks_reduce_rows<RB>(acc[0], lane);
+            if (ks_lane_stores<RB>(lane)) part[wave * rows_cap + bb * RB + ks_row_of_lane<RB>(lane)] = t;
+        }
+    } else
     for (int bb = 0; bb < nbatch; ++bb) {
         float acc[B][RB];
 #pragma unroll
@@ -439,7 +564,7 @@
     KS_STAMP(trace_op, 5, wall_clock64());
 }
 
-template <int B, int MODE, bool NORM, int XS, int CPL, bool R32, bool EX = false>
+template <int B, int MODE, bool NORM, int XS, int CPL, bool R32, bool EX = false, bool PK = false>
 __global__ __launch_bounds__(KS_NT, 4) void emmax_decode_ks_kernel(GemvParams p) {
     extern __shared__ __attribute__((aligned(16))) unsigned char ks_smem[];
     const int tid = threadIdx.x, lane = tid & 63, wave = __builtin_amdgcn_readfirstlane(tid >> 6);
@@ -447,19 +572,19 @@
     float* part = (float*)ks_smem;
     float* sumsq = part + KS_WAVES * B * rows_cap;
     u32x4_t wr[KsRegs<B>::N];
-    ks_run_op<B, MODE, NORM, XS, CPL, R32, EX>(p, wr, part, sumsq, rows_cap, 0);
-}
-
-template <int B, int MODE, bool NORM, int XS, int CPL, bool R32, bool EX = false>
+    ks_run_op<B, MODE, NORM, XS, CPL, R32, EX, PK>(p, wr, part, sumsq, rows_cap, 0);
+}
+
+template <int B, int MODE, bool NORM, int XS, int CPL, bool R32, bool EX = false, bool PK = false>
 int ks_launch_r(const GemvParams& p, const ProjGeom& g, hipStream_t stream) {
-    hipLaunchKernelGGL((emmax_decode_ks_kernel<B, MODE, NORM, XS, CPL, R32, EX>), dim3(g.grid), dim3(KS_NT), g.smem, stream, p);
+    hipLaunchKernelGGL((emmax_decode_ks_kernel<B, MODE, NORM, XS, CPL, R32, EX, PK>), dim3(g.grid), dim3(KS_NT), g.smem, stream, p);
     return hipGetLastError() == hipSuccess ? 0 : -4;
 }
-template <int B, int MODE, bool NORM, bool XATTN, int CPL>
+template <int B, int MODE, bool NORM, bool XATTN, int CPL, bool PK = false>
 int ks_launch_t(const GemvParams& p, const ProjGeom& g, hipStream_t stream) {
     constexpr bool touches_h = NORM || MODE == GEMV_RESID;
     if (p.exact) {
-        if constexpr (MODE == GEMV_PLAIN) return -2;
+        if constexpr (MODE == GEMV_PLAIN || PK) return -2;
         else {
             if constexpr (MODE == GEMV_QKV) {
                 if (p.x_tok) return ks_launch_r<B, MODE, NORM, XS_EMBED, CPL, true, true>(p, g, stream);
@@ -468,20 +593,173 @@
         }
     }
     if constexpr (MODE == GEMV_QKV) {
-        if (p.x_tok) return p.h32 ? ks_launch_r<B, MODE, NORM, XS_EMBED, CPL, true>(p, g, stream) : ks_launch_r<B, MODE, NORM, XS_EMBED, CPL, false>(p, g, stream);
+        if (p.x_tok) return p.h32 ? ks_launch_r<B, MODE, NORM, XS_EMBED, CPL, true, false, PK>(p, g, stream) : ks_launch_r<B, MODE, NORM, XS_EMBED, CPL, false, false, PK>(p, g, stream);
     }
     if constexpr (touches_h) {
-        if (p.h32) return ks_launch_r<B, MODE, NORM, XATTN ? XS_ATTN : XS_GLOBAL, CPL, true>(p, g, stream);
-    }
-    return ks_launch_r<B, MODE, NORM, XATTN ? XS_ATTN : XS_GLOBAL, CPL, false>(p, g, stream);
+        if (p.h32) return ks_launch_r<B, MODE, NORM, XATTN ? XS_ATTN : XS_GLOBAL, CPL, true, false, PK>(p, g, stream);
+    }
+    return ks_launch_r<B, MODE, NORM, XATTN ? XS_ATTN : XS_GLOBAL, CPL, false, false, PK>(p, g, stream);
 }
 
 template <int MODE, bool NORM, bool XATTN>
 int ks_launch_mode(const GemvParams& p, int B, const ProjGeom& g, hipStream_t stream) {
+    if (g.pk) {
+        if constexpr (MODE != GEMV_PLAIN) {
+            if (B == 1 && g.cpl == 1) return ks_launch_t<1, MODE, NORM, XATTN, 1, true>(p, g, stream);
+        }
+        return -2;
+    }
 #define KS_CASE(BB, CC) if (B == BB && g.cpl == CC) return ks_launch_t<BB, MODE, NORM, XATTN, CC>(p, g, stream)
     KS_CASE(1, 1); KS_CASE(1, 2); KS_CASE(1, 3); KS_CASE(2, 1); KS_CASE(2, 2); KS_CASE(2, 3);
 #undef KS_CASE
     return -2;
+}
+
+struct Pk13Args {
+    const bf16_t* W;
+    bf16_t* W_out;
+    unsigned char *planes, *hdr, *ovf;
+    int ldw, n_rows, K, head_dim, shift, mode, n_groups, grid, regions, ovf_cap;
+    int *n_overflow, *n_bad;
+};
+__device__ __forceinline__ void pk13_locate(const Pk13Args& a, int t, int& g_lo, int& nrows, int& i0, int& wave, size_t* plane_off = nullptr, bool* half_out = nullptr) {
+    const int gb = t >> 3, r = a.n_groups % a.grid, q = a.n_groups / a.grid;
+    const int nb1 = ks_pk_batches(q + 1), nb0 = ks_pk_batches(q);
+    const int bid = gb < r * nb1 ? gb / nb1 : r + (gb - r * nb1) / nb0;
+    const int bb = gb - ks_pk_first_batch(a.n_groups, a.grid, bid);
+    int npairs;
+    ks_share_of(a.n_groups, a.grid, bid, g_lo, npairs);
+    nrows = 2 * npairs;
+    i0 = bb * PK13_ROWS;
+    wave = t & 7;
+    const bool half = nrows - i0 <= 8;
+    if (half_out) *half_out = half;
+    if (plane_off) *plane_off = (size_t)ks_pk_first_byte(a.n_groups, a.grid, bid) * KS_WAVES + (size_t)bb * (KS_WAVES * PK13_REGION) + (size_t)wave * (half ? PK13_HALF : PK13_REGION);
+}
+__device__ __forceinline__ u32x4_t pk13_raw_row(const Pk13Args& a, int g_lo, int nrows, int i, int coff, int* row_out = nullptr) {
+    int r0, r1;
+    ks_pair_rows_of(a.mode, a.head_dim, a.shift, a.n_rows, g_lo + (i >> 1), r0, r1);
+    const int r = (i & 1) ? r1 : r0;
+    if (row_out) *row_out = r;
+    if (i >= nrows) return u32x4_t{0u, 0u, 0u, 0u};
+    return *((const u32x4_t*)(a.W + (size_t)r * a.ldw) + coff);
+}
+__device__ __forceinline__ int pk13_coff(const Pk13Args& a, int wave, int lane) {
+    const int NCW = a.K >> 6;
+    return wave * NCW + min(lane, NCW - 1);
+}
+
+__global__ __launch_bounds__(64) void emmax_pk13_pack_kernel(Pk13Args a) {
+    const int t = blockIdx.x, lane = threadIdx.x;
+    int g_lo, nrows, i0, wave;
+    size_t poff;
+    bool half;
+    pk13_locate(a, t, g_lo, nrows, i0, wave, &poff, &half);
+    const int coff = pk13_coff(a, wave, lane);
+    u32x4_t out[PK13_SLOTS];
+#pragma unroll
+    for (int L = 0; L < PK13_SLOTS; ++L) out[L] = u32x4_t{0u, 0u, 0u, 0u};
+    uint32_t bases[4] = {0u, 0u, 0u, 0u};
+    bool ok = true;
+    KsUnroll<PK13_ROWS>::run([&](auto J) {
+        constexpr int jj = decltype(J)::value;
+        const u32x4_t v = pk13_raw_row(a, g_lo, nrows, i0 + jj, coff);
+        uint16_t h[8];
+        int emax = 0;
+#pragma unroll
+        for (int e = 0; e < 8; ++e) {
+            h[e] = (uint16_t)(v[e >> 1] >> (16 * (e & 1)));
+            emax = max(emax, (h[e] >> 7) & 0xff);
+        }
+#pragma unroll
+        for (int m = 32; m >= 1; m >>= 1) emax = max(emax, __shfl_xor(emax, m));
+        bases[jj >> 2] |= (uint32_t)emax << (8 * (jj & 3));
+        uint32_t sm[2];
+        uint64_t ex;
+        ok = pk13_encode(h, (unsigned)emax, sm, ex) && ok;
+        constexpr int T = jj >> 3, j = jj & 7, i = (40 * j) >> 5, sft = (40 * j) & 31;
+        out[pk13_sm_slot(jj)][(jj & 1) * 2] = sm[0];
+        out[pk13_sm_slot(jj)][(jj & 1) * 2 + 1] = sm[1];
+        const uint64_t sh = ex << sft;
+        out[pk13_ex_slot(T, i)][pk13_ex_word(T, i)] |= (uint32_t)sh;
+        out[pk13_ex_slot(T, i + 1)][pk13_ex_word(T, i + 1)] |= (uint32_t)(sh >> 32);
+    });
+    const bool bad = __any(!ok) != 0;
+    u32x4_t* dst = (u32x4_t*)(a.planes + poff) + lane;
+#pragma unroll
+    for (int L = 0; L < PK13_SLOTS; ++L)
+        if (L < PK13_HALF / 1024 || !half) dst[L * 64] = bad ? u32x4_t{0u, 0u, 0u, 0u} : out[L];
+    if (lane == 0) {
+        u32x4_t* hp = (u32x4_t*)(a.hdr + (size_t)t * PK13_HDR);
+        hp[0] = u32x4_t{bases[0], bases[1], bad ? 1u : 0u, 0u};
+        hp[1] = u32x4_t{0u, 0u, 0u, 0u};
+        hp[2] = u32x4_t{bases[2], bases[3], bad ? 1u : 0u, 0u};
+        hp[3] = u32x4_t{0u, 0u, 0u, 0u};
+    }
+}
+__global__ __launch_bounds__(1024) void emmax_pk13_index_kernel(Pk13Args a) {
+    __shared__ int cnt[1024];
+    const int tid = threadIdx.x, per = (a.regions + 1023) / 1024, t0 = tid * per, t1 = min(t0 + per, a.regions);
+    int n = 0;
+    for (int t = t0; t < t1; ++t) n += ((const int*)(a.hdr + (size_t)t * PK13_HDR))[2] != 0;
+    cnt[tid] = n;
+    __syncthreads();
+    for (int d = 1; d < 1024; d <<= 1) {
+        const int v = tid >= d ? cnt[tid - d] : 0;
+        __syncthreads();
+        cnt[tid] += v;
+        __syncthreads();
+    }
+    int idx = cnt[tid] - n;
+    for (int t = t0; t < t1; ++t) {
+        int* hp = (int*)(a.hdr + (size_t)t * PK13_HDR);
+        const int v = hp[2] != 0 ? idx++ : -1;
+        hp[2] = v;
+        hp[10] = v;
+    }
+    if (tid == 1023) *a.n_overflow = cnt[1023];
+}
+__global__ __launch_bounds__(64) void emmax_pk13_overflow_kernel(Pk13Args a) {
+    const int t = blockIdx.x, lane = threadIdx.x;
+    const int oi = ((const int*)(a.hdr + (size_t)t * PK13_HDR))[2];
+    if (oi < 0 || oi >= a.ovf_cap) return;
+    int g_lo, nrows, i0, wave;
+    pk13_locate(a, t, g_lo, nrows, i0, wave);
+    const int coff = pk13_coff(a, wave, lane);
+    u32x4_t* dst = (u32x4_t*)(a.ovf + (size_t)oi * PK13_OVF) + lane;
+    for (int jj = 0; jj < PK13_ROWS; ++jj) dst[jj * 64] = pk13_raw_row(a, g_lo, nrows, i0 + jj, coff);
+}
+__global__ __launch_bounds__(64) void emmax_pk13_unpack_kernel(Pk13Args a) {
+    const int t = blockIdx.x, lane = threadIdx.x;
+    int g_lo, nrows, i0, wave;
+    size_t poff;
+    bool half;
+    pk13_locate(a, t, g_lo, nrows, i0, wave, &poff, &half);
+    const int coff = pk13_coff(a, wave, lane);
+    const KsPkHdr hd = ks_pk_hdr(a.hdr, t);
+    const int oi = (int)hd.a[2];
+    if (oi >= a.ovf_cap) {
+        if (!a.W_out && lane == 0) atomicAdd(a.n_bad, 1);
+        return;
+    }
+    u32x4_t wr[16];
+    const u32x4_t* src = oi >= 0 ? (const u32x4_t*)(a.ovf + (size_t)oi * PK13_OVF) + lane : (const u32x4_t*)(a.planes + poff) + lane;
+#pragma unroll
+    for (int L = 0; L < 16; ++L) wr[L] = (oi >= 0 || L < (half ? PK13_HALF / 1024 : PK13_SLOTS)) ? src[L * 64] : u32x4_t{0u, 0u, 0u, 0u};
+    bool same = true;
+    KsUnroll<PK13_ROWS>::run([&](auto J) {
+        constexpr int jj = decltype(J)::value;
+        const u32x4_t w = oi >= 0 ? wr[jj] : pk13_expand<jj>(wr, ks_pk_bb<jj>(hd));
+        if (a.W_out) {
+            int r0, r1;
+            ks_pair_rows_of(a.mode, a.head_dim, a.shift, a.n_rows, g_lo + ((i0 + jj) >> 1), r0, r1);
+            if (i0 + jj < nrows && lane < (a.K >> 6)) *((u32x4_t*)(a.W_out + (size_t)(((i0 + jj) & 1) ? r1 : r0) * a.ldw) + coff) = w;
+        } else {
+            const u32x4_t v = pk13_raw_row(a, g_lo, nrows, i0 + jj, coff);
+            same = same && v[0] == w[0] && v[1] == w[1] && v[2] == w[2] && v[3] == w[3];
+        }
+    });
+    if (!a.W_out && __any(!same) != 0 && lane == 0) atomicAdd(a.n_bad, 1);
 }
 
 }
@@ -519,6 +797,54 @@
     g.smem = (size_t)(KS_WAVES * B * g.kc + KS_WAVES * B) * sizeof(float);
     if (out) *out = g;
     return true;
+}
+
+bool pk13_plan(int mode, int n_rows, int K, const ProjGeom& g, Pk13Plan* out) {
+    if (mode < GEMV_QKV || mode > GEMV_LMHEAD || g.cpl != 1 || g.grid < 1 || g.n_groups < g.grid || K % 64 || n_rows < 1) return false;
+    const int q = g.n_groups / g.grid, r = g.n_groups % g.grid;
+    const long long batches = (long long)r * ks_pk_batches(q + 1) + (long long)(g.grid - r) * ks_pk_batches(q);
+    const long long regions = batches * KS_WAVES;
+    const long long bytes = ((long long)r * ks_pk_block_bytes(q + 1) + (long long)(g.grid - r) * ks_pk_block_bytes(q)) * KS_WAVES;
+    if (bytes >= (1ll << 31) - (1 << 20)) return false;
+    if (out) *out = {(int)regions, bytes, regions * PK13_HDR};
+    return true;
+}
+static Pk13Args pk13_args(int mode, const void* W, int ldw, int n_rows, int K, int head_dim, const ProjGeom& g, const void* planes, const void* hdr, const void* ovf,
+                          int ovf_cap, int regions) {
+    Pk13Args a = {};
+    a.W = (const bf16_t*)W; a.planes = (unsigned char*)planes; a.hdr = (unsigned char*)hdr; a.ovf = (unsigned char*)ovf;
+    a.ldw = ldw; a.n_rows = n_rows; a.K = K; a.head_dim = head_dim; a.shift = g.shift; a.mode = mode; a.n_groups = g.n_groups; a.grid = g.grid;
+    a.regions = regions; a.ovf_cap = ovf_cap;
+    return a;
+}
+int launch_pk13_pack(int mode, const void* W, int ldw, int n_rows, int K, int head_dim, const ProjGeom& g, void* planes, void* hdr, void* ovf, int ovf_cap,
+                     int* n_overflow, hipStream_t stream) {
+    Pk13Plan pl;
+    if (!pk13_plan(mode, n_rows, K, g, &pl) || ldw % 8 || ldw < K || ovf_cap < 0) return -2;
+    Pk13Args a = pk13_args(mode, W, ldw, n_rows, K, head_dim, g, planes, hdr, ovf, ovf_cap, pl.regions);
+    a.n_overflow = n_overflow;
+    hipLaunchKernelGGL(emmax_pk13_pack_kernel, dim3(pl.regions), dim3(64), 0, stream, a);
+    hipLaunchKernelGGL(emmax_pk13_index_kernel, dim3(1), dim3(1024), 0, stream, a);
+    if (ovf_cap > 0) hipLaunchKernelGGL(emmax_pk13_overflow_kernel, dim3(pl.regions), dim3(64), 0, stream, a);
+    return hipGetLastError() == hipSuccess ? 0 : -4;
+}
+int launch_pk13_verify(int mode, const void* W, int ldw, int n_rows, int K, int head_dim, const ProjGeom& g, const void* planes, const void* hdr, const void* ovf,
+                       int ovf_cap, int* n_bad, hipStream_t stream) {
+    Pk13Plan pl;
+    if (!pk13_plan(mode, n_rows, K, g, &pl) || ldw % 8 || ldw < K) return -2;
+    Pk13Args a = pk13_args(mode, W, ldw, n_rows, K, head_dim, g, planes, hdr, ovf, ovf_cap, pl.regions);
+    a.n_bad = n_bad;
+    hipLaunchKernelGGL(emmax_pk13_unpack_kernel, dim3(pl.regions), dim3(64), 0, stream, a);
+    return hipGetLastError() == hipSuccess ? 0 : -4;
+}
+int launch_pk13_unpack(int mode, void* W, int ldw, int n_rows, int K, int head_dim, const ProjGeom& g, const void* planes, const void* hdr, const void* ovf,
+                       int ovf_cap, hipStream_t stream) {
+    Pk13Plan pl;
+    if (!pk13_plan(mode, n_rows, K, g, &pl) || ldw % 8 || ldw < K) return -2;
+    Pk13Args a = pk13_args(mode, W, ldw, n_rows, K, head_dim, g, planes, hdr, ovf, ovf_cap, pl.regions);
+    a.W_out = (bf16_t*)W;
+    hipLaunchKernelGGL(emmax_pk13_unpack_kernel, dim3(pl.regions), dim3(64), 0, stream, a);
+    return hipGetLastError() == hipSuccess ? 0 : -4;
 }
 
 int launch_decode_ks(int mode, const GemvParams& p_in, int B, hipStream_t stream, int* grid_out, const ProjGeom* geom) {
diff --git a/emma-x_amd/csrc/kernels.h b/emma-x_amd/csrc/kernels.h
--- a/emma-x_amd/csrc/kernels.h
+++ b/emma-x_amd/csrc/kernels.h
@@ -169,6 +169,7 @@
     int kv_fp8;
     int resid32;
     int mx4_wide;
+    int pk;
     int exact;
     int epoch;
 };
@@ -217,6 +218,9 @@
     int exact;
     long long kv24;
     const void* w4_scales;
+    const void* pk_hdr;
+    const void* pk_ovf;
+    unsigned pk_bytes, pk_ovf_bytes;
 };
 
 enum { PW_BF16 = 0, PW_FP8 = 1, PW_MX4 = 2 };
@@ -240,6 +244,7 @@
     int cpl, f8;
     int nb, phased, roll;
     int tmax, nph, nh;
+    int pk;
 };
 bool decode_ks_takes(const ProjShape& s, int B, ProjGeom* g = nullptr);
 bool decode_gemv_takes(const ProjShape& s, int B, ProjGeom* g = nullptr);
@@ -250,6 +255,14 @@
 int launch_decode_gemv_staged(int mode, const GemvParams& p, int B, const ProjGeom& g, hipStream_t stream, int* grid_out = nullptr);
 int launch_decode_ks(int mode, const GemvParams& p, int B, hipStream_t stream, int* grid_out = nullptr, const ProjGeom* geom = nullptr);
 bool decode_ks_enabled();
+struct Pk13Plan { int regions; long long plane_bytes, hdr_bytes; };
+bool pk13_plan(int mode, int n_rows, int K, const ProjGeom& g, Pk13Plan* out);
+int launch_pk13_pack(int mode, const void* W, int ldw, int n_rows, int K, int head_dim, const ProjGeom& g, void* planes, void* hdr, void* ovf, int ovf_cap,
+                     int* n_overflow, hipStream_t stream);
+int launch_pk13_verify(int mode, const void* W, int ldw, int n_rows, int K, int head_dim, const ProjGeom& g, const void* planes, const void* hdr, const void* ovf,
+                       int ovf_cap, int* n_bad, hipStream_t stream);
+int launch_pk13_unpack(int mode, void* W, int ldw, int n_rows, int K, int head_dim, const ProjGeom& g, const void* planes, const void* hdr, const void* ovf,
+                       int ovf_cap, hipStream_t stream);
 int decode_gemv_init();
 int launch_decode_embed(const int32_t* cur_tok, const void* E, void* h, int B, int hidden, int vocab, hipStream_t stream, float* h32 = nullptr);
 
diff --git a/emma-x_amd/csrc/model.hip b/emma-x_amd/csrc/model.hip
--- a/emma-x_amd/csrc/model.hip
+++ b/emma-x_amd/csrc/model.hip
@@ -5,6 +5,7 @@
 #include <mutex>
 
 #include "session.h"
+#include "pk13.h"
 
 thread_local std::string g_err;
 int fail(int code, const char* fmt, ...) {
@@ -36,7 +37,7 @@
     {"gemm_hybrid", &EmmaxTune::gemm_hybrid, 1}, {"gemm_normfuse", &EmmaxTune::gemm_normfuse, 1},
     {"resid32", &EmmaxTune::resid32, 1},       {"kv_fp8", &EmmaxTune::kv_fp8, 0},
     {"exact", &EmmaxTune::exact, 0},           {"attn_group", &EmmaxTune::attn_group, -1},
-    {"mx4_wide", &EmmaxTune::mx4_wide, 0},
+    {"mx4_wide", &EmmaxTune::mx4_wide, 0},      {"pk", &EmmaxTune::pk, 22},
 };
 EmmaxTune g_tune;
 std::once_flag g_tune_once;
@@ -139,6 +140,7 @@
     for (auto& L : m->layers)
         for (const ProjDim& d : layer_projs(m)) L.proj[d.stage].q4w = m->mx4_wide;
     m->lm_head_w.q4w = m->mx4_wide;
+    m->pk_mask = (m->fp8 || m->mx4) ? 0 : (emmax_tune().pk & 31);
 }
 
 static void plan_arena(emmax_model* m, Bump& b) {
@@ -386,6 +388,90 @@
     return 0;
 }
 
+struct PkItem { const ProjW* w; int layer, stage, mode, n_rows, K; ProjGeom g; Pk13Plan pl; int cap; void *pk, *hdr, *ovf; };
+static std::vector<PkItem> plan_pk(const emmax_model* m, Bump& b, int32_t** counters) {
+    std::vector<PkItem> items;
+    auto add = [&](const ProjW* w, int layer, int stage) {
+        PkItem it = {};
+        it.w = w; it.layer = layer; it.stage = stage;
+        if (!(m->pk_mask & w->f8bit) || !pk_stage_plan(m, stage, &it.g, &it.pl, &it.mode, &it.n_rows, &it.K)) return;
+        it.cap = (it.pl.regions + 999) / 1000;
+        it.pk = b.bytes(it.pl.plane_bytes);
+        it.hdr = b.bytes(it.pl.hdr_bytes);
+        it.ovf = b.bytes((int64_t)it.cap * PK13_OVF);
+        items.push_back(it);
+    };
+    for (size_t li = 0; li < m->layers.size(); ++li)
+        for (const ProjDim& d : layer_projs(m)) add(&m->layers[li].proj[d.stage], (int)li, d.stage);
+    add(&m->lm_head_w, -1, STAGE_LMHEAD);
+    int32_t* c = (int32_t*)b.bytes((int64_t)items.size() * 8 + 8);
+    if (counters) *counters = c;
+    return items;
+}
+
+int64_t emmax_model_pk_bytes(const emmax_model* m) {
+    if (!m) return -1;
+    if (!m->pk_mask) return 0;
+    Bump b{nullptr};
+    return plan_pk(m, b, nullptr).empty() ? 0 : b.off + 256;
+}
+
+int emmax_model_build_pk(emmax_model* m, void* buf, int64_t bytes, emmax_stream stream) {
+    if (!m) return fail(EMMAX_ERR_INVALID, "null argument");
+    if (!m->finalized) return fail(EMMAX_ERR_STATE, "emmax_model_build_pk before emmax_model_finalize");
+    if (m->pk_built) return fail(EMMAX_ERR_STATE, "emmax_model_build_pk: the packed copies exist already");
+    const int64_t need = emmax_model_pk_bytes(m);
+    if (need == 0) return 0;
+    if (!buf) return fail(EMMAX_ERR_INVALID, "null argument");
+    if (bytes < need) return fail(EMMAX_ERR_NOMEM, "pk arena too small: %lld < %lld", (long long)bytes, (long long)need);
+    if ((uintptr_t)buf % 256) return fail(EMMAX_ERR_INVALID, "pk arena must be 256-byte aligned");
+    hipStream_t st = (hipStream_t)stream;
+    Bump b{(char*)buf};
+    int32_t* cnt = nullptr;
+    const std::vector<PkItem> items = plan_pk(m, b, &cnt);
+    const int n = (int)items.size();
+    if (hipMemsetAsync(cnt, 0, (size_t)n * 8 + 8, st) != hipSuccess) return fail(EMMAX_ERR_HIP, "emmax_model_build_pk: memset failed");
+    for (int i = 0; i < n; ++i) {
+        const PkItem& it = items[i];
+        int r = launch_pk13_pack(it.mode, it.w->rm, it.K, it.n_rows, it.K, m->cfg.head_dim, it.g, it.pk, it.hdr, it.ovf, it.cap, cnt + 2 * i, st);
+        if (!r) r = launch_pk13_verify(it.mode, it.w->rm, it.K, it.n_rows, it.K, m->cfg.head_dim, it.g, it.pk, it.hdr, it.ovf, it.cap, cnt + 2 * i + 1, st);
+        if (r) return fail(r == -4 ? EMMAX_ERR_HIP : EMMAX_ERR_INVALID, "emmax_model_build_pk: packing the %s matrix failed (%d)", decode_stage_name(it.stage), r);
+    }
+    std::vector<int32_t> host((size_t)2 * n);
+    if (hipMemcpyAsync(host.data(), cnt, (size_t)n * 8, hipMemcpyDeviceToHost, st) != hipSuccess || hipStreamSynchronize(st) != hipSuccess)
+        return fail(EMMAX_ERR_HIP, "emmax_model_build_pk: reading the counters failed");
+    for (int i = 0; i < n; ++i)
+        if (host[2 * i] <= items[i].cap && host[2 * i + 1] != 0)
+            return fail(EMMAX_ERR_STATE, "emmax_model_build_pk: the packed copy of the %s matrix (layer %d) does not expand to its rows: %d of %d regions differ",
+                        decode_stage_name(items[i].stage), items[i].layer, host[2 * i + 1], items[i].pl.regions);
+    for (int st_ = 0; st_ <= STAGE_LMHEAD; ++st_) { m->pk_packed[st_] = m->pk_kept_raw[st_] = 0; m->pk_overflow[st_] = 0; }
+    for (int i = 0; i < n; ++i) {
+        const PkItem& it = items[i];
+        if (host[2 * i] > it.cap) {
+            m->pk_kept_raw[it.stage] += 1;
+            continue;
+        }
+        ProjW& w = it.layer < 0 ? m->lm_head_w : m->layers[it.layer].proj[it.stage];
+        w.pk = it.pk; w.pk_hdr = it.hdr; w.pk_ovf = it.ovf;
+        w.pk_bytes = (unsigned)it.pl.plane_bytes; w.pk_ovf_cap = it.cap; w.pk_grid = it.g.grid; w.pk_groups = it.g.n_groups;
+        m->pk_packed[it.stage] += 1;
+        m->pk_overflow[it.stage] += host[2 * i];
+    }
+    m->pk_built = true;
+    return 0;
+}
+int emmax_model_pk_info(const emmax_model* m, int stage, int* packed, int* kept_raw, int64_t* overflow_regions) {
+    if (!m || stage > STAGE_LMHEAD) return fail(EMMAX_ERR_INVALID, "emmax_model_pk_info: null model or stage above 5");
+    int np = 0, nr = 0;
+    int64_t no = 0;
+    for (int st = 0; st <= STAGE_LMHEAD; ++st)
+        if (stage < 0 || stage == st) { np += m->pk_packed[st]; nr += m->pk_kept_raw[st]; no += m->pk_overflow[st]; }
+    if (packed) *packed = np;
+    if (kept_raw) *kept_raw = nr;
+    if (overflow_regions) *overflow_regions = no;
+    return m->pk_mask;
+}
+
 int emmax_model_max_decode_batch(const emmax_model* m) { return m ? model_max_decode_batch(m) : -1; }
 int emmax_model_max_decode_batch_exact(const emmax_model* m) { return m ? model_max_decode_batch(m, true) : -1; }
 int emmax_model_mxfp4_wide(const emmax_model* m) { return m ? (m->mx4_wide ? 1 : 0) : -1; }
diff --git a/emma-x_amd/csrc/ops.hip b/emma-x_amd/csrc/ops.hip
--- a/emma-x_amd/csrc/ops.hip
+++ b/emma-x_amd/csrc/ops.hip
@@ -696,5 +696,42 @@
     return 0;
 }
 
-
-}
+static bool pk13_op_geom(int mode, int n_rows, int K, int head_dim, int max_grid, ProjGeom* g, Pk13Plan* pl) {
+    ProjShape s = {};
+    s.mode = mode; s.K = K; s.n_rows = n_rows; s.head_dim = head_dim; s.wfmt = PW_BF16; s.ld_ok = true; s.max_parts = EMMAX_LM_BLOCKS; s.max_grid = max_grid;
+    if (mode < GEMV_QKV || mode > GEMV_LMHEAD || n_rows < 2 || ((mode == GEMV_QKV || mode == GEMV_GATEUP) && n_rows % (mode == GEMV_QKV ? (head_dim > 0 ? head_dim : 1) : 32))) return false;
+    return decode_ks_takes(s, 1, g) && pk13_plan(mode, n_rows, K, *g, pl);
+}
+int emmax_op_last_proj_packed(void) { return last_proj_packed(); }
+int emmax_op_pk13_plan(int mode, int n_rows, int K, int head_dim, int max_grid, int* grid, int* n_groups, int* regions) {
+    ProjGeom g;
+    Pk13Plan pl;
+    if (!pk13_op_geom(mode, n_rows, K, head_dim, max_grid, &g, &pl))
+        return fail(EMMAX_ERR_INVALID, "emmax_op_pk13_plan: no packed form (modes 0-3; K %% 64 and K <= 4096; qkv: rows in whole heads, head_dim a power of two; gate/up: rows %% 32)");
+    if (grid) *grid = g.grid;
+    if (n_groups) *n_groups = g.n_groups;
+    if (regions) *regions = pl.regions;
+    return 0;
+}
+int emmax_op_pk13_pack(const void* W, int ld, int mode, int n_rows, int K, int head_dim, int max_grid, void* planes, void* hdr, void* ovf, int ovf_cap,
+                       int32_t* n_overflow, emmax_stream st) {
+    ProjGeom g;
+    Pk13Plan pl;
+    if (!W || !planes || !hdr || !n_overflow || (ovf_cap > 0 && !ovf)) return fail(EMMAX_ERR_INVALID, "emmax_op_pk13_pack: null argument");
+    if (!pk13_op_geom(mode, n_rows, K, head_dim, max_grid, &g, &pl)) return fail(EMMAX_ERR_INVALID, "emmax_op_pk13_pack: no packed form for this shape (emmax_op_pk13_plan)");
+    const int r = launch_pk13_pack(mode, W, ld, n_rows, K, head_dim, g, planes, hdr, ovf, ovf_cap, n_overflow, (hipStream_t)st);
+    if (r) return fail(r == -4 ? EMMAX_ERR_HIP : EMMAX_ERR_INVALID, "emmax_op_pk13_pack: ld %% 8, ld >= K, ovf_cap >= 0 required");
+    return 0;
+}
+int emmax_op_pk13_unpack(void* W, int ld, int mode, int n_rows, int K, int head_dim, int max_grid, const void* planes, const void* hdr, const void* ovf, int ovf_cap,
+                         emmax_stream st) {
+    ProjGeom g;
+    Pk13Plan pl;
+    if (!W || !planes || !hdr || (ovf_cap > 0 && !ovf)) return fail(EMMAX_ERR_INVALID, "emmax_op_pk13_unpack: null argument");
+    if (!pk13_op_geom(mode, n_rows, K, head_dim, max_grid, &g, &pl)) return fail(EMMAX_ERR_INVALID, "emmax_op_pk13_unpack: no packed form for this shape (emmax_op_pk13_plan)");
+    const int r = launch_pk13_unpack(mode, W, ld, n_rows, K, head_dim, g, planes, hdr, ovf, ovf_cap, (hipStream_t)st);
+    if (r) return fail(r == -4 ? EMMAX_ERR_HIP : EMMAX_ERR_INVALID, "emmax_op_pk13_unpack: ld %% 8, ld >= K required");
+    return 0;
+}
+
+}
diff --git a/emma-x_amd/csrc/pk13.h b/emma-x_amd/csrc/pk13.h
--- /dev/null
+++ b/emma-x_amd/csrc/pk13.h
@@ -0,0 +1,54 @@
+#pragma once
+#include <cstdint>
+
+#include "common.h"
+
+enum { PK13_ROWS = 16, PK13_SLOTS = 13, PK13_REGION = PK13_SLOTS * 1024, PK13_HALF = 7 * 1024, PK13_HDR = 64, PK13_OVF = PK13_ROWS * 1024 };
+
+__host__ __device__ constexpr int pk13_sm_slot(int jj) { return (jj >> 3) * 7 + ((((jj & 7) >> 1) == 0) ? 1 : 2 + ((jj & 7) >> 1)); }
+__host__ __device__ constexpr int pk13_ex_slot(int T, int i) { return i < 4 ? T * 7 : i < 8 ? T * 7 + 2 : 6; }
+__host__ __device__ constexpr int pk13_ex_word(int T, int i) { return i < 8 ? (i & 3) : 2 * T + (i - 8); }
+
+__host__ __device__ inline bool pk13_encode(const uint16_t (&h)[8], unsigned base, uint32_t (&sm)[2], uint64_t& ex) {
+    bool ok = true;
+    sm[0] = sm[1] = 0;
+    ex = 0;
+    for (int e = 0; e < 8; ++e) {
+        const unsigned v = h[e], ef = (v >> 7) & 0xffu;
+        unsigned o;
+        if (ef == 0) { o = base; ok = ok && base <= 31u; }
+        else { o = base - ef; ok = ok && o <= 30u; }
+        sm[e >> 2] |= (((v >> 8) & 0x80u) | (v & 0x7fu)) << (8 * (e & 3));
+        ex |= (uint64_t)(o & 31u) << (5 * e);
+    }
+    return ok;
+}
+
+#if defined(__HIPCC__)
+template <int S>
+__device__ __forceinline__ u32x4_t pk13_expand_words(uint32_t d0, uint32_t d1, uint32_t S0, uint32_t S1, uint32_t bb) {
+    const uint32_t lo = S ? __builtin_amdgcn_alignbit(d1, d0, S) : d0;
+    const uint32_t hi = S ? (d1 >> S) : d1;
+    u32x4_t w;
+#pragma unroll
+    for (int k = 0; k < 4; ++k) {
+        const uint32_t Sm = k < 2 ? S0 : S1;
+        const uint32_t a = (2 * k) & 3, b = a + 1;
+        const uint32_t dup = __builtin_amdgcn_perm(Sm, Sm, a | (a << 8) | (b << 16) | (b << 24));
+        const uint32_t v = k == 0 ? lo : k < 3 ? (lo >> (10 * k)) : __builtin_amdgcn_alignbit(hi, lo, 30);
+        const uint32_t O = (((v & 0x3ffu) * 0x801u) & 0x001f001fu);
+        w[k] = (dup & 0x807f807fu) | ((bb - O) << 7);
+    }
+    return w;
+}
+template <int JJ>
+__device__ __forceinline__ u32x4_t pk13_expand(const u32x4_t (&wr)[16], uint32_t bb, uint32_t s6a, uint32_t s6b) {
+    constexpr int T = JJ >> 3, j = JJ & 7, i = (40 * j) >> 5, s = (40 * j) & 31;
+    constexpr int sl = pk13_sm_slot(JJ), sw = (JJ & 1) * 2;
+    const uint32_t d0 = (T == 1 && i >= 8) ? (i == 8 ? s6a : s6b) : wr[pk13_ex_slot(T, i)][pk13_ex_word(T, i)];
+    const uint32_t d1 = (T == 1 && i + 1 >= 8) ? (i + 1 == 8 ? s6a : s6b) : wr[pk13_ex_slot(T, i + 1)][pk13_ex_word(T, i + 1)];
+    return pk13_expand_words<s>(d0, d1, wr[sl][sw], wr[sl][sw + 1], bb);
+}
+template <int JJ>
+__device__ __forceinline__ u32x4_t pk13_expand(const u32x4_t (&wr)[16], uint32_t bb) { return pk13_expand<JJ>(wr, bb, wr[6][2], wr[6][3]); }
+#endif
diff --git a/emma-x_amd/csrc/session.h b/emma-x_amd/csrc/session.h
--- a/emma-x_amd/csrc/session.h
+++ b/emma-x_amd/csrc/session.h
@@ -78,6 +78,9 @@
     void *q4, *q4s;
     int gemv_mode, f8bit;
     bool q4w;
+    void *pk, *pk_hdr, *pk_ovf;
+    unsigned pk_bytes;
+    int pk_ovf_cap, pk_grid, pk_groups;
 };
 struct LayerW {
     bf16 *ln1, *ln2;
@@ -96,6 +99,10 @@
     bool fp8 = false;
     bool mx4 = false;
     bool mx4_wide = false;
+    int pk_mask = 0;
+    bool pk_built = false;
+    int pk_packed[STAGE_LMHEAD + 1] = {}, pk_kept_raw[STAGE_LMHEAD + 1] = {};
+    long long pk_overflow[STAGE_LMHEAD + 1] = {};
     bool ln_folded = false;
     bool aux_built = false;
     bool aux_ab = false;
@@ -279,6 +286,8 @@
 int decode_stage_route(const emmax_model* m, int stage, int B, bool exact);
 bool decode_batch_served(const emmax_model* m, int B, bool exact);
 const char* decode_stage_name(int stage);
+int last_proj_packed();
+bool pk_stage_plan(const emmax_model* m, int stage, ProjGeom* g, Pk13Plan* pl, int* mode, int* n_rows, int* K);
 int stage_chunk(int stage, bool exact);
 bool beam_pages_fit(const emmax_session* s, int S, int max_new);
 int launch_beam_finish(emmax_session* s, bool is_prefill, hipStream_t st);
diff --git a/emma-x_amd/csrc/step.hip b/emma-x_amd/csrc/step.hip
--- a/emma-x_amd/csrc/step.hip
+++ b/emma-x_amd/csrc/step.hip
@@ -1,4 +1,5 @@
 #include "session.h"
+#include "pk13.h"
 
 static bool streamk_on() { return emmax_tune().streamk != 0; }
 
@@ -8,13 +9,16 @@
     return B == 1 ? (F8_OPROJ | F8_LMHEAD) : F8_OPROJ;
 }
 
-struct ProjCopies { bool rm, r8, sc, km, fm, q4; int f8bit; bool q4w; };
-static ProjCopies copies_of(const ProjW& w) { return {w.rm != nullptr, w.r8 != nullptr, w.sc != nullptr, w.km != nullptr, w.fm != nullptr, w.q4 != nullptr, w.f8bit, w.q4 != nullptr && w.q4w}; }
+struct ProjCopies { bool rm, r8, sc, km, fm, q4; int f8bit; bool q4w; bool pk; int pk_grid, pk_groups; };
+static ProjCopies copies_of(const ProjW& w) {
+    return {w.rm != nullptr, w.r8 != nullptr, w.sc != nullptr, w.km != nullptr, w.fm != nullptr, w.q4 != nullptr, w.f8bit, w.q4 != nullptr && w.q4w,
+            w.pk != nullptr, w.pk_grid, w.pk_groups};
+}
 static ProjCopies copies_planned(const emmax_model* m, int stage) {
     const bool pair = stage == STAGE_QKV || stage == STAGE_GATEUP;
     const bool fm = m->fp8 || (!m->mx4 && (!pair || (m->aux_built ? m->aux_ab : emmax_tune().km == 0)));
     const int bit = stage == STAGE_QKV ? F8_QKV : stage == STAGE_OPROJ ? F8_OPROJ : stage == STAGE_GATEUP ? F8_GATEUP : stage == STAGE_DOWN ? F8_DOWN : F8_LMHEAD;
-    return {true, m->fp8, m->fp8, !m->mx4, fm, m->mx4, bit, m->mx4 && m->mx4_wide};
+    return {true, m->fp8, m->fp8, !m->mx4, fm, m->mx4, bit, m->mx4 && m->mx4_wide, false, 0, 0};
 }
 
 enum { ROUTE_NO_FM = -1 };
@@ -39,18 +43,25 @@
         if (!c.fm) return ROUTE_NO_FM;
         return decode_mfma_takes(s, B, g) ? EMMAX_VIA_MFMA : EMMAX_VIA_NONE;
     }
-    if (decode_ks_enabled() && decode_ks_takes(s, B, g)) return EMMAX_VIA_KS;
+    if (decode_ks_enabled() && decode_ks_takes(s, B, g)) {
+        if (g && B == 1 && c.pk && (emmax_tune().pk & c.f8bit) && g->cpl == 1 && g->grid == c.pk_grid && g->n_groups == c.pk_groups) g->pk = 1;
+        return EMMAX_VIA_KS;
+    }
     return decode_gemv_takes(s, B, g) ? EMMAX_VIA_GEMV : EMMAX_VIA_NONE;
 }
 
+static int g_last_proj_packed = 0;
+int last_proj_packed() { return g_last_proj_packed; }
 static int launch_proj(const ProjW& w, GemvParams& p, int B, hipStream_t st, int* grid_out, int* via = nullptr) {
     const int mode = w.gemv_mode;
     ProjGeom g;
     const int route = proj_route(copies_of(w), proj_shape(mode, p), B, &g);
+    g_last_proj_packed = route == EMMAX_VIA_KS && g.pk ? 1 : 0;
     if (via) *via = route > 0 ? route : EMMAX_VIA_NONE;
     switch (route) {
         case EMMAX_VIA_KS:
             p.W = w.rm;
+            if (g.pk) { p.W = w.pk; p.pk_hdr = w.pk_hdr; p.pk_ovf = w.pk_ovf; p.pk_bytes = w.pk_bytes; p.pk_ovf_bytes = (unsigned)w.pk_ovf_cap * (unsigned)PK13_OVF; }
             return launch_decode_ks(mode, p, B, st, grid_out, &g);
         case EMMAX_VIA_GEMV:
             p.W = w.rm;
@@ -134,6 +145,18 @@
         n_prev = n;
     }
     return via;
+}
+
+bool pk_stage_plan(const emmax_model* m, int stage, ProjGeom* g, Pk13Plan* pl, int* mode, int* n_rows, int* K) {
+    if (m->fp8 || m->mx4) return false;
+    const ProjShape s = stage_shape(m, stage, 1, false);
+    ProjGeom gg;
+    if (!decode_ks_takes(s, 1, &gg) || !pk13_plan(s.mode, s.n_rows, s.K, gg, pl)) return false;
+    if (g) *g = gg;
+    if (mode) *mode = s.mode;
+    if (n_rows) *n_rows = s.n_rows;
+    if (K) *K = s.K;
+    return true;
 }
 
 static const int kProjStages[] = {STAGE_QKV, STAGE_OPROJ, STAGE_GATEUP, STAGE_DOWN, STAGE_LMHEAD};
diff --git a/emma-x_amd/emmax/_lib.py b/emma-x_amd/emmax/_lib.py
--- a/emma-x_amd/emmax/_lib.py
+++ b/emma-x_amd/emmax/_lib.py
@@ -57,6 +57,9 @@
     "emmax_model_finalize": (C.c_int, [_vp, _vp, C.c_int64, _vp]),
     "emmax_model_aux_bytes": (C.c_int64, [_vp]),
     "emmax_model_build_aux": (C.c_int, [_vp, _vp, C.c_int64, _vp]),
+    "emmax_model_pk_bytes": (C.c_int64, [_vp]),
+    "emmax_model_build_pk": (C.c_int, [_vp, _vp, C.c_int64, _vp]),
+    "emmax_model_pk_info": (C.c_int, [_vp, C.c_int, _vp, _vp, _vp]),
     "emmax_session_bytes": (C.c_int, [_vp, C.c_int, C.c_int, C.c_int, _c_i64p, _c_i64p]),
     "emmax_session_create": (C.c_int, [_vp, C.c_int, C.c_int, C.c_int, _vp, C.c_int64, _vp, C.c_int64, C.POINTER(_vp)]),
     "emmax_session_bytes_ex": (C.c_int, [_vp, C.c_int, C.c_int, C.c_int, C.c_int, _c_i64p, _c_i64p]),
@@ -110,6 +113,10 @@
     "emmax_op_quant_fm8": (C.c_int, [_vp, C.c_int, _vp, _vp, C.c_int, C.c_int, _vp]),
     "emmax_op_quant_mxfp4": (C.c_int, [_vp, C.c_int, _vp, _vp, C.c_int, C.c_int, C.c_int, C.c_int, _vp]),
     "emmax_op_dequant_mxfp4": (C.c_int, [_vp, _vp, _vp, C.c_int, C.c_int, C.c_int, C.c_int, C.c_int, _vp]),
+    "emmax_op_last_proj_packed": (C.c_int, []),
+    "emmax_op_pk13_plan": (C.c_int, [C.c_int, C.c_int, C.c_int, C.c_int, C.c_int, _vp, _vp, _vp]),
+    "emmax_op_pk13_pack": (C.c_int, [_vp, C.c_int, C.c_int, C.c_int, C.c_int, C.c_int, C.c_int, _vp, _vp, _vp, C.c_int, _vp, _vp]),
+    "emmax_op_pk13_unpack": (C.c_int, [_vp, C.c_int, C.c_int, C.c_int, C.c_int, C.c_int, C.c_int, _vp, _vp, _vp, C.c_int, _vp]),
     "emmax_op_gemm_small_mxfp4": (C.c_int, [_vp, _vp, _vp, _vp, C.c_int, C.c_int, C.c_int, _vp]),
     "emmax_op_gemm_wide_mxfp4": (C.c_int, [_vp, _vp, _vp, _vp, C.c_int, C.c_int, C.c_int, _vp]),
     "emmax_op_gemm_small_fp8": (C.c_int, [_vp, _vp, _vp, _vp, C.c_int, C.c_int, C.c_int, _vp]),
diff --git a/emma-x_amd/emmax/engine.py b/emma-x_amd/emmax/engine.py
--- a/emma-x_amd/emmax/engine.py
+++ b/emma-x_amd/emmax/engine.py
@@ -91,12 +91,16 @@
         self.finalize_s = time.perf_counter() - t0
         self.aux_build_s = 0.0
         del keep
+        self.pk_arena: Optional[torch.Tensor] = None
+        self.pk_s, self.pk_mask, self.pk_packed, self.pk_kept_raw, self.pk_overflow_regions = 0.0, 0, 0, 0, 0
         self.aux_arena: Optional[torch.Tensor] = None
         self.max_batch = self.max_prompt = self.max_ctx = 0
         self._resize_tables: Dict[Tuple[int, int, int], tuple] = {}
         self._adm_stream = None
         self._commit_event = None
         self.new_session(max_batch, max_prompt, max_ctx)
+        if max_batch == 1:
+            self.ensure_packed_weights()
 
     def new_session(self, max_batch: int, max_prompt: int, max_ctx: Optional[int] = None, stage_rows: int = 0) -> None:
         if self._session:
@@ -125,6 +129,8 @@
             self.new_session(max(self.max_batch, int(n)), self.max_prompt, self.max_ctx, stage_rows=int(n))
 
     def ensure_decode_batch(self, batch: int) -> None:
+        if batch == 1:
+            self.ensure_packed_weights()
         if batch < 3 or self.aux_arena is not None:
             return
         n = int(self.lib.emmax_model_aux_bytes(self._model))
@@ -144,8 +150,28 @@
             return int(self.lib.emmax_model_max_decode_batch_exact(self._model))
         return int(self.lib.emmax_model_max_decode_batch(self._model))
 
+    def ensure_packed_weights(self) -> None:
+        if self.pk_arena is not None or self.exact:
+            return
+        n_pk = int(self.lib.emmax_model_pk_bytes(self._model))
+        if n_pk <= 0:
+            return
+        import time
+
+        t0 = time.perf_counter()
+        self.pk_arena = _device_bytes(n_pk, self.device, "PK")
+        _lib.check(self.lib.emmax_model_build_pk(self._model, self.pk_arena.data_ptr(), n_pk, _lib.current_stream()), "emmax_model_build_pk")
+        self.pk_s = time.perf_counter() - t0
+        self.pk_mask, self.pk_packed, self.pk_kept_raw, self.pk_overflow_regions = self.pk_info()
+
+    def pk_info(self, stage: int = -1):
+        a, b, c = C.c_int(), C.c_int(), C.c_int64()
+        mask = int(self.lib.emmax_model_pk_info(self._model, int(stage), C.byref(a), C.byref(b), C.byref(c)))
+        return mask, a.value, b.value, c.value
+
     def weight_bytes(self) -> int:
-        return int(self.arena.numel()) + (int(self.aux_arena.numel()) if self.aux_arena is not None else 0)
+        return (int(self.arena.numel()) + (int(self.aux_arena.numel()) if self.aux_arena is not None else 0)
+                + (int(self.pk_arena.numel()) if self.pk_arena is not None else 0))
 
     def ensure_capacity(self, batch: int, prompt: int, max_new: int) -> None:
         need_ctx = self.cfg.n_patches + prompt + max_new + 1
diff --git a/include/emmax.h b/include/emmax.h
--- a/include/emmax.h
+++ b/include/emmax.h
@@ -61,6 +61,9 @@
 int emmax_model_finalize(emmax_model* m, void* arena_dev, int64_t arena_bytes, emmax_stream stream);
 int64_t emmax_model_aux_bytes(const emmax_model* m);
 int emmax_model_build_aux(emmax_model* m, void* aux_arena_dev, int64_t aux_bytes, emmax_stream stream);
+int64_t emmax_model_pk_bytes(const emmax_model* m);
+int emmax_model_build_pk(emmax_model* m, void* pk_arena_dev, int64_t pk_bytes, emmax_stream stream);
+int emmax_model_pk_info(const emmax_model* m, int stage, int* packed, int* kept_raw, int64_t* overflow_regions);
 
 int emmax_session_bytes(const emmax_model* m, int max_batch, int max_prompt, int max_ctx,
                         int64_t* workspace_bytes, int64_t* kv_bytes);
@@ -212,6 +215,12 @@
 int emmax_op_quant_fm8(const void* W_dev, int ld, void* W8_fm_out_dev, float* scales_out_dev, int N, int K, emmax_stream stream);
 int emmax_op_quant_mxfp4(const void* W_dev, int ld, void* tiles_out_dev, void* scales_out_dev, int N, int K, int perm, int perm_hd, emmax_stream stream);
 int emmax_op_dequant_mxfp4(const void* tiles_dev, const void* scales_dev, void* W_out_dev, int ld, int N, int K, int perm, int perm_hd, emmax_stream stream);
+int emmax_op_pk13_plan(int mode, int n_rows, int K, int head_dim, int max_grid, int* grid, int* n_groups, int* regions);
+int emmax_op_last_proj_packed(void);
+int emmax_op_pk13_pack(const void* W_dev, int ld, int mode, int n_rows, int K, int head_dim, int max_grid, void* planes_dev, void* hdr_dev, void* ovf_dev,
+                       int ovf_cap, int32_t* n_overflow_dev, emmax_stream stream);
+int emmax_op_pk13_unpack(void* W_out_dev, int ld, int mode, int n_rows, int K, int head_dim, int max_grid, const void* planes_dev, const void* hdr_dev,
+                         const void* ovf_dev, int ovf_cap, emmax_stream stream);
 int emmax_op_gemm_small_mxfp4(const void* x_dev, const void* tiles_dev, const void* scales_dev, void* y_dev, int B, int N, int K, emmax_stream stream);
 int emmax_op_gemm_wide_mxfp4(const void* x_dev, const void* tiles_dev, const void* scales_dev, void* y_dev, int B, int N, int K, emmax_stream stream);
 int emmax_op_gemm_small_fp8(const void* x_dev, const void* W8_fm_dev, const float* scales_dev, void* y_dev, int B, int N, int K,
```

After: 0.7660 actions/s (median of 6 runs). 1.02x the previous value.
